# microsoft/aurora

Hardware: AMD Instinct MI355X
Metric: forecast-steps/sec (6h step) 0.25deg ERA5 721x1440x13 (higher is better)
Workload: dtype bf16; 1 GPU; AuroraPretrained(autocast=True) 1.3B, 0.25deg ERA5 721x1440, 13 levels, T=2, batch 1 per GPU, one forward step (BASELINE.json configs[1]); parallelism=1 GPU

## Files before the change

aurora_amd/csrc/gemm.hip:

```cpp
#include <stdlib.h>

#include <algorithm>

#include "gemm_tile.h"

namespace aurora {

namespace {

constexpr int BM = 128;
constexpr int BN = 128;
constexpr int ROW_BYTES = 128;
constexpr int TILE_BYTES = 128 * ROW_BYTES;
constexpr int THREADS = 256;
constexpr int A4_DEFAULT_MIN_K = 0;

template <typename T>
__global__ __launch_bounds__(THREADS, 2) void linear_kernel(const LinearArgs p_in) {
  const LinearArgs p = batch_problem(p_in);
  extern __shared__ __attribute__((aligned(16))) char smem[];
  auto lds_x = [&](int buf) { return smem + buf * 2 * TILE_BYTES; };
  auto lds_w = [&](int buf) { return smem + buf * 2 * TILE_BYTES + TILE_BYTES; };

  const int tid = threadIdx.x;
// ... 409 lines not shown
    }
  }
  if (p.C2 == nullptr && p.res == nullptr && p.vec_store) {
    if (p.act == AURORA_ACT_GELU) epilogue_256_bf16_coalesced<4>(p, acc, m0, n0, wm, wn, wave, lane, smem, &bias_pre);
    else epilogue_256_bf16_coalesced<2>(p, acc, m0, n0, wm, wn, wave, lane, smem, &bias_pre);
    return;
  }
  epilogue_256<bf16_t>(p, acc, m0, n0, wm, wn, i16, g);
}

}

}

using namespace aurora;

namespace {
int default_f32_mode() {
  static const int mode = [] {
    const char* e = getenv("AURORA_F32_GEMM");
    return !e ? 1 : (e[0] == 'n' || e[0] == '0') ? 0 : (e[0] == 'f' || e[0] == '2') ? 2 : 1;
  }();
  return mode;
}

int a4_min_k() {
  static const int v = [] {
    const char* e = getenv("AURORA_GEMM_A4_MIN_K");
    const int k = e ? atoi(e) : A4_DEFAULT_MIN_K;
    return k <= 0 ? 0x7fffffff : k;
  }();
  return v;
}

struct SplitWs { float* slabs; int64_t slab_bytes; int32_t* tickets; int n_tickets; int split; };

int choose_split(int64_t M, int N, int K, int64_t cus) {
  if (N % BN2 != 0 || M < 1024 || K % 32 != 0) return 1;
  const int64_t tiles = ((M + BM2 - 1) / BM2) * (N / BN2);
  const int kt = K / 32;
  int s = (int)std::min<int64_t>(std::min<int64_t>(8, cus / tiles), kt / 64);
  return s < 1 ? 1 : s;
}

struct LinearCall {
  const void* A; int64_t lda; const void* W; int64_t ldw; const float* bias; void* C; int64_t ldc;
  int64_t M; int N; int K; int dtype; void* stream;
  int act = AURORA_ACT_NONE;
  void* C2 = nullptr; int64_t ldc2 = 0; const float* residual = nullptr; int64_t ldr = 0;
  int f32_gemm = -1; const float* guard = nullptr; float guard_limit = 0.f;
  int batch = 1; int64_t stride_a = 0, stride_w = 0, stride_bias = 0, stride_c = 0;
  const SplitWs* ws = nullptr;
  int64_t plane_stride = 0; int plane_heads = 0;
  int pre = 0, mode = 0;
  int es() const { return dtype == AURORA_F32 ? 4 : 2; }
};

enum { K_TILE_128 = F32_KERNELS, K_RING, K_RING_MID, K_PP, K_PP_SPLITK, K_A4 };
struct LinearPlan {
  int kernel; bool twin;
  int bm, bn, rowb;
  int ksplit;
};

int check_call(LinearCall& c) {
  AURORA_CHECK_ARG(c.dtype == AURORA_F32 || c.dtype == AURORA_BF16, "linear: bad dtype %d", c.dtype);
  AURORA_CHECK_ARG(c.plane_stride == 0 || (c.dtype == AURORA_BF16 && c.plane_heads > 0 && c.N % (64 * c.plane_heads) == 0 &&
                                           c.N <= 192 * c.plane_heads && c.plane_stride >= c.M * 192 &&
                                           c.plane_stride % 8 == 0 && c.C2 == nullptr && c.residual == nullptr && c.batch == 1),
                   "linear: head planes need bf16, N = 64 heads x (1, 2 or 3), planes of >= M rows, one output, no residual");
  c.pre = c.f32_gemm < 0 ? 0 : c.f32_gemm & (AURORA_F32_A_SPLIT | AURORA_F32_W_SPLIT | AURORA_F32_C_SPLIT);
  if (c.pre) c.f32_gemm &= ~c.pre;
  AURORA_CHECK_ARG(c.f32_gemm >= -1 && c.f32_gemm <= 2, "linear: bad fp32 GEMM mode %d", c.f32_gemm);
  c.mode = c.f32_gemm < 0 ? default_f32_mode() : c.f32_gemm;
  AURORA_CHECK_ARG(!c.pre || (c.dtype == AURORA_F32 && c.mode == 2 && c.N % 128 == 0 && c.K % 32 == 0 && c.K >= 96),
                   "linear: fp16-pair operands need fp32, mode 2, N %% 128 == 0, K %% 32 == 0, K >= 96 (N=%d K=%d)", c.N, c.K);
  AURORA_CHECK_ARG(!(c.pre & AURORA_F32_A_SPLIT) || (c.pre & AURORA_F32_W_SPLIT),
                   "linear: a pre-split activation operand needs pre-split weights");
  AURORA_CHECK_ARG(!(c.pre & AURORA_F32_C_SPLIT) || (c.C2 == nullptr && c.ldc % 32 == 0 && ((uintptr_t)c.C % 16) == 0),
                   "linear: fp16-pair output needs ldc %% 32 == 0, 16-byte alignment and no second output");
  if (!(c.mode == 2 || (c.mode == 1 && c.dtype == AURORA_F32))) c.guard = nullptr;
  AURORA_CHECK_ARG(c.M > 0 && c.N > 0 && c.K > 0, "linear: empty problem M=%lld N=%d K=%d", (long long)c.M, c.N, c.K);
  const int es = c.es();
  AURORA_CHECK_ARG(((int64_t)c.K * es) % ROW_BYTES == 0,
                   "linear: K=%d must be a multiple of %d elements", c.K, ROW_BYTES / es);
  AURORA_CHECK_ARG((c.lda * es) % 16 == 0 && (c.ldw * es) % 16 == 0 && c.lda >= c.K && c.ldw >= c.K,
                   "linear: operand strides must be 16-byte multiples >= K");
  AURORA_CHECK_ARG(((uintptr_t)c.A % 16) == 0 && ((uintptr_t)c.W % 16) == 0, "linear: unaligned operand");
  AURORA_CHECK_ARG(c.act >= AURORA_ACT_NONE && c.act <= AURORA_ACT_SILU, "linear: bad activation %d", c.act);
  AURORA_CHECK_ARG(c.C != nullptr && c.ldc >= c.N && (!c.C2 || c.ldc2 >= c.N) && (!c.residual || c.ldr >= c.N || c.ldr == 0),
                   "linear: bad output strides");
  return AURORA_OK;
}

LinearPlan plan_linear(const LinearCall& c, int64_t cus) {
  const int64_t M = c.M;
  const int N = c.N, K = c.K, dtype = c.dtype, pre = c.pre, mode = c.mode;
  const bool split = dtype == AURORA_F32 && mode >= 1;
  const bool tall = pre != 0 && N % VN != 0;
  bool big = (M >= 1024 || split) && (N % BN2 == 0 || tall);
  bool mid = false;
  int ksplit = 1;
  if (big && dtype == AURORA_BF16 && c.batch == 1 && c.ws != nullptr) {
    ksplit = c.ws->split > 0 ? std::min(c.ws->split, K / 128) : choose_split(M, N, K, cus);
    const int64_t tiles = ((M + BM2 - 1) / BM2) * (N / BN2);
    if (ksplit > 1 && (tiles > c.ws->n_tickets || tiles * ksplit * (int64_t)(BM2 * BN2 * 4) > c.ws->slab_bytes)) ksplit = 1;
  }
  if (big && !split && ksplit <= 1) {
    const int64_t nb_big = ((M + BM2 - 1) / BM2) * (N / BN2), nb_small = ((M + BM - 1) / BM) * ((N + BN - 1) / BN);
    const int64_t nb_mid = ((M + BM2 - 1) / BM2) * (N / 128);
    if (dtype == AURORA_BF16) {
      auto cost = [&](int64_t nb, int64_t slots, double a, double b) {
        const int64_t full = nb / slots, rem = nb % slots;
        const double part = rem == 0 ? 0.0 : (slots > cus && rem <= cus) ? 0.65 : 1.0;
        return ((double)full + part) * (a + b * (double)K);
      };
      const double t_big = cost(nb_big, cus, 10.1, 0.0266), t_mid = cost(nb_mid, 2 * cus, 7.7, 0.0317),
                   t_small = cost(nb_small, 2 * cus, 7.6, 0.0153);
      if (t_mid < 0.97 * t_big && t_mid <= t_small) mid = true;
      else if (t_small < 0.97 * t_big) big = false;
    } else {
      auto fill = [&](int64_t nb, int64_t slots) { return (double)nb / (double)(((nb + slots - 1) / slots) * slots); };
      if (0.8 * fill(nb_small, 2 * cus) > fill(nb_big, cus)) big = false;
    }
  }
  LinearPlan plan{K_TILE_128, false, big ? BM2 : BM, mid ? 128 : big ? BN2 : BN, big ? ROW2 : ROW_BYTES, ksplit};
  const int k_tiles = (int)(((int64_t)K * c.es()) / plan.rowb);
  const bool f32pp = big && split && mode == 2 && K % 32 == 0 && K >= 96;
  const int pp = tall ? ((pre & AURORA_F32_A_SPLIT) ? F32_PP_AW_TALL : F32_PP_W_TALL)
                      : (pre & AURORA_F32_A_SPLIT) ? F32_PP_AW : (pre & AURORA_F32_W_SPLIT) ? F32_PP_W : F32_PP;
  if (mid) plan.kernel = K_RING_MID;
  else if (!big) plan.kernel = K_TILE_128;
  else if (pre) plan.kernel = pp;
  else if (split && mode == 1 && c.guard != nullptr) plan.kernel = F32_THREE;
  else if (split && mode == 2 && c.guard != nullptr) {
    plan.kernel = f32pp ? pp : F32_TWO;
    plan.twin = true;
  } else if (f32pp) plan.kernel = pp;
  else if (split && mode == 2) plan.kernel = F32_TWO;
  else if (split) plan.kernel = F32_THREE;
  else if (dtype == AURORA_F32) plan.kernel = K_RING;
  else if (ksplit > 1) plan.kernel = K_PP_SPLITK;
  else if (k_tiles >= 8 && k_tiles % 2 == 0 && K >= a4_min_k()) plan.kernel = K_A4;
  else if (k_tiles >= 4) plan.kernel = K_PP;
  else plan.kernel = K_RING;
  return plan;
}

constexpr LinearKernel KERNELS[K_A4 - K_TILE_128][2] = {
     {{linear_kernel<bf16_t>, THREADS, 4 * TILE_BYTES}, {linear_kernel<float>, THREADS, 4 * TILE_BYTES}},
     {{linear_kernel_256<bf16_t, 4, 4>, THREADS2, RING_LDS}, {linear_kernel_256<float, 4, 4>, THREADS2, RING_LDS}},
     {{linear_kernel_256<bf16_t, 2, 3>, 256, MID_LDS}, {}},
     {{linear_kernel_256pp<false>, THREADS2, PP_LDS}, {}},
     {{linear_kernel_256pp<true>, THREADS2, PP_LDS}, {}},
};

int vec_store_of(const LinearCall& c) {
  const int es = c.es(), es2 = es == 4 ? 2 : 4;
  if (c.plane_stride) return ((uintptr_t)c.C % 16) == 0 ? 1 : 0;
  bool vec = ((uintptr_t)c.C % 16) == 0 && (c.ldc * es) % 16 == 0;
  if (c.C2) vec = vec && ((uintptr_t)c.C2 % 16) == 0 && (c.ldc2 * es2) % 16 == 0;
  if (c.residual) vec = vec && ((uintptr_t)c.residual % 16) == 0 && (c.ldr * 4) % 16 == 0;
  return vec ? 1 : 0;
}

int launch_linear(const LinearCall& c, const LinearPlan& plan) {
  const int64_t M = c.M;
  const int N = c.N, K = c.K, es = c.es();
  const bool split = c.dtype == AURORA_F32 && c.mode >= 1, big = plan.bm == BM2;
  LinearArgs p;
  p.A = (const char*)c.A; p.lda_b = c.lda * es;
  p.W = (const char*)c.W; p.ldw_b = c.ldw * es;
  p.bias = c.bias;
  p.C = (char*)c.C; p.ldc = c.ldc; p.C2 = (char*)c.C2; p.ldc2 = c.ldc2;
  p.res = c.residual; p.ldr = c.ldr;
  p.M = M; p.N = N; p.k_tiles = (int)(((int64_t)K * es) / plan.rowb); p.act = c.act;
  p.tiles_n = (N + plan.bn - 1) / plan.bn;
  p.n_blocks = ((M + plan.bm - 1) / plan.bm) * p.tiles_n;
  p.vec_store = vec_store_of(c);
  if (split && big && c.act == AURORA_ACT_GELU) p.act = ACT_GELU_FAST;
  p.guard = split ? c.guard : nullptr;
  p.guard_limit = c.guard_limit;
  p.out_split = (c.pre & AURORA_F32_C_SPLIT) ? 1 : 0;
  AURORA_CHECK_ARG(p.n_blocks < (int64_t)1 << 31, "linear: too many tiles");

  p.bs_a = c.stride_a * es; p.bs_w = c.stride_w * es; p.bs_c = c.stride_c * es; p.bs_bias = c.stride_bias;
  p.split = plan.ksplit; p.slabs = plan.ksplit > 1 ? c.ws->slabs : nullptr; p.tickets = plan.ksplit > 1 ? c.ws->tickets : nullptr;
  p.plane_stride = c.plane_stride; p.plane_heads = c.plane_heads;
  once_per_device([] {
    for (const auto& row : KERNELS)
      for (const LinearKernel& k : row)
        if (k.fn) (void)hipFuncSetAttribute((const void*)k.fn, hipFuncAttributeMaxDynamicSharedMemorySize, k.lds_bytes);
  });
  if (plan.kernel < F32_KERNELS) {
    if (plan.kernel >= F32_PP) {
      const bool tall = plan.kernel >= F32_PP_W_TALL;
      LinearArgs q = p;
      q.k_tiles = K / 32;
      q.tiles_n = tall ? N / 128 : N / VN;
      q.n_blocks = tall ? ((M + 255) / 256) * q.tiles_n : ((M + VM - 1) / VM) * q.tiles_n;
      if (const int err = aurora_f32_launch(plan.kernel, &q, (unsigned)q.n_blocks, (unsigned)c.batch, c.stream)) return err;
    } else {
      if (const int err = aurora_f32_launch(plan.kernel, &p, (unsigned)p.n_blocks, (unsigned)c.batch, c.stream)) return err;
    }
    if (plan.twin) (void)aurora_f32_launch(F32_THREE, &p, (unsigned)p.n_blocks, (unsigned)c.batch, c.stream);
  } else if (plan.kernel == K_A4) {
    (void)aurora_a4_launch(&p, (unsigned)p.n_blocks, (unsigned)c.batch, c.stream);
  } else {
    const LinearKernel& k = KERNELS[plan.kernel - K_TILE_128][c.dtype == AURORA_F32];
    const int64_t slices = plan.kernel == K_PP_SPLITK ? plan.ksplit : 1;
    const dim3 grid((unsigned)(p.n_blocks * slices), (unsigned)c.batch);
    hipLaunchKernelGGL(k.fn, grid, dim3(k.threads), k.lds_bytes, as_stream(c.stream), p);
  }
  return check_launch("linear");
}

int linear_impl(LinearCall c) {
  if (const int err = check_call(c)) return err;
  return launch_linear(c, plan_linear(c, device_cus()));
}

static_assert(F32_THREE == AURORA_PLAN_F32_THREE && F32_TWO == AURORA_PLAN_F32_TWO && F32_PP == AURORA_PLAN_F32_PP &&
              F32_PP_W == AURORA_PLAN_F32_PP_W && F32_PP_AW == AURORA_PLAN_F32_PP_AW &&
              F32_PP_W_TALL == AURORA_PLAN_F32_PP_W_TALL && F32_PP_AW_TALL == AURORA_PLAN_F32_PP_AW_TALL &&
              K_TILE_128 == AURORA_PLAN_TILE128 && K_RING == AURORA_PLAN_RING && K_RING_MID == AURORA_PLAN_RING_MID &&
              K_PP == AURORA_PLAN_PP && K_PP_SPLITK == AURORA_PLAN_PP_SPLITK && K_A4 == AURORA_PLAN_A4,
              "include/aurora_hip.h: AURORA_PLAN_* out of step with the dispatcher's kernel ids");

LinearCall plain_call(const void* A, int64_t lda, const void* W, int64_t ldw, const float* bias, void* C, int64_t ldc, void* C2,
                      int64_t ldc2, const float* residual, int64_t ldr, int64_t M, int N, int K, int dtype, int act, void* stream) {
  LinearCall c{A, lda, W, ldw, bias, C, ldc, M, N, K, dtype, stream, act};
  c.C2 = C2; c.ldc2 = ldc2; c.residual = residual; c.ldr = ldr;
  return c;
}
}

extern "C" int aurora_hip_default_f32_gemm(void) { return default_f32_mode(); }

extern "C" int64_t aurora_hip_linear_workspace(int64_t M, int N, int K, int dtype) {
  if (dtype != AURORA_BF16 || M <= 0 || N <= 0 || K <= 0) return 0;
  const int s = choose_split(M, N, K, device_cus());
  return s <= 1 ? 0 : ((M + BM2 - 1) / BM2) * (N / BN2) * s * (int64_t)(BM2 * BN2 * 4);
}

extern "C" int aurora_hip_linear(const void* A, int64_t lda, const void* W, int64_t ldw,
                                 const float* bias, void* C, int64_t ldc, void* C2, int64_t ldc2,
                                 const float* residual, int64_t ldr, int64_t M, int N, int K,
                                 int dtype, int act, void* stream) {
  return aurora_hip_linear_ex(A, lda, W, ldw, bias, C, ldc, C2, ldc2, residual, ldr, M, N, K, dtype, act, -1, nullptr,
                              0.f, stream);
}

extern "C" int aurora_hip_linear_ex(const void* A, int64_t lda, const void* W, int64_t ldw,
                                    const float* bias, void* C, int64_t ldc, void* C2, int64_t ldc2,
                                    const float* residual, int64_t ldr, int64_t M, int N, int K,
                                    int dtype, int act, int f32_gemm, const float* guard, float guard_limit,
                                    void* stream) {
  LinearCall c = plain_call(A, lda, W, ldw, bias, C, ldc, C2, ldc2, residual, ldr, M, N, K, dtype, act, stream);
  c.f32_gemm = f32_gemm; c.guard = guard; c.guard_limit = guard_limit;
  return linear_impl(c);
}

extern "C" int aurora_hip_linear_planes(const void* A, int64_t lda, const void* W, int64_t ldw, const float* bias, void* C,
                                        int64_t plane_stride, int heads, int64_t M, int N, int K, int dtype, void* stream) {
  AURORA_CHECK_ARG(plane_stride > 0 && heads > 0, "linear_planes: plane_stride=%lld heads=%d", (long long)plane_stride, heads);
  LinearCall c = plain_call(A, lda, W, ldw, bias, C, N, nullptr, 0, nullptr, 0, M, N, K, dtype, AURORA_ACT_NONE, stream);
  c.plane_stride = plane_stride; c.plane_heads = heads;
  return linear_impl(c);
}

extern "C" int aurora_hip_linear_ws(const void* A, int64_t lda, const void* W, int64_t ldw, const float* bias, void* C,
                                    int64_t ldc, void* C2, int64_t ldc2, const float* residual, int64_t ldr, int64_t M, int N,
                                    int K, int dtype, int act, void* workspace, int64_t workspace_bytes, int32_t* tickets,
                                    int n_tickets, int split, void* stream) {
  AURORA_CHECK_ARG(workspace_bytes >= 0 && n_tickets >= 0 && split >= 0 && ((uintptr_t)workspace % 16) == 0,
                   "linear_ws: bad workspace arguments");
  const SplitWs ws{(float*)workspace, workspace ? workspace_bytes : 0, tickets, tickets ? n_tickets : 0, split};
  LinearCall c = plain_call(A, lda, W, ldw, bias, C, ldc, C2, ldc2, residual, ldr, M, N, K, dtype, act, stream);
  c.ws = &ws;
  return linear_impl(c);
}

extern "C" int aurora_hip_linear_batched(const void* A, int64_t lda, const void* W, int64_t ldw, const float* bias, void* C,
                                         int64_t ldc, int64_t M, int N, int K, int dtype, int act, int f32_gemm,
                                         const float* guard, float guard_limit, int batch, int64_t stride_a,
                                         int64_t stride_w, int64_t stride_bias, int64_t stride_c, void* stream) {
  AURORA_CHECK_ARG(batch >= 1 && batch <= 65535, "linear_batched: 1 <= batch <= 65535 (got %d)", batch);
  const int es = dtype == AURORA_F32 ? 4 : 2;
  AURORA_CHECK_ARG((stride_a * es) % 16 == 0 && (stride_w * es) % 16 == 0 && (stride_c * es) % 16 == 0 && stride_bias % 4 == 0,
                   "linear_batched: batch strides must keep every problem 16-byte aligned");
  LinearCall c = plain_call(A, lda, W, ldw, bias, C, ldc, nullptr, 0, nullptr, 0, M, N, K, dtype, act, stream);
  c.f32_gemm = f32_gemm; c.guard = guard; c.guard_limit = guard_limit;
  c.batch = batch; c.stride_a = stride_a; c.stride_w = stride_w; c.stride_bias = stride_bias; c.stride_c = stride_c;
  return linear_impl(c);
}

extern "C" int aurora_hip_linear_plan(int64_t M, int N, int K, int dtype, int f32_gemm, int has_guard, int batch, int64_t ldc,
                                      int64_t c_addr, int64_t ldc2, int64_t c2_addr, int64_t ldr, int64_t residual_addr,
                                      int64_t workspace_bytes, int n_tickets, int split, int64_t plane_stride, int plane_heads,
                                      int cus, int32_t* plan_out) {
  AURORA_CHECK_ARG(plan_out != nullptr && c_addr != 0 && cus >= 0 && batch >= 1, "linear_plan: bad query");
  static const float guard_word = 0.f;
  LinearCall c = plain_call((const void*)16, K, (const void*)16, K, nullptr, (void*)(uintptr_t)c_addr, ldc,
                            (void*)(uintptr_t)c2_addr, ldc2, (const float*)(uintptr_t)residual_addr, ldr, M, N, K, dtype,
                            AURORA_ACT_NONE, nullptr);
  c.f32_gemm = f32_gemm; c.guard = has_guard ? &guard_word : nullptr;
  c.batch = batch;
  const SplitWs ws{nullptr, workspace_bytes, nullptr, n_tickets, split};
  if (workspace_bytes >= 0) c.ws = &ws;
  c.plane_stride = plane_stride; c.plane_heads = plane_heads;
  if (const int err = check_call(c)) return err;
  const LinearPlan plan = plan_linear(c, cus > 0 ? cus : device_cus());
  const bool pp = plan.kernel >= F32_PP && plan.kernel < F32_KERNELS, tall = pp && plan.kernel >= F32_PP_W_TALL;
  plan_out[0] = plan.kernel;
  plan_out[1] = plan.twin ? 1 : 0;
  plan_out[2] = pp ? (tall ? 256 : VM) : plan.bm;
  plan_out[3] = pp ? (tall ? 128 : VN) : plan.bn;
  plan_out[4] = plan.ksplit;
  plan_out[5] = vec_store_of(c);
  return AURORA_OK;
}
```

aurora_amd/csrc/gemm_f32.hip:

```cpp
#include "gemm_tile.h"

#ifndef F32PP_PARTS
#define F32PP_PARTS 4
#endif

namespace aurora {

namespace {

typedef __bf16 bf16x8_t __attribute__((ext_vector_type(8)));

struct Split3 { u32x4 h, m, l; };

__device__ __forceinline__ void split_pair(uint32_t a0, uint32_t a1, uint32_t& h, uint32_t& m, uint32_t& l) {
  constexpr uint32_t SEL = 0x07060302u;
  h = __builtin_amdgcn_perm(a1, a0, SEL);
  const float r0 = __uint_as_float(a0) - __uint_as_float(a0 & 0xffff0000u);
  const float r1 = __uint_as_float(a1) - __uint_as_float(a1 & 0xffff0000u);
  const uint32_t q0 = __float_as_uint(r0), q1 = __float_as_uint(r1);
  m = __builtin_amdgcn_perm(q1, q0, SEL);
  const float s0 = r0 - __uint_as_float(q0 & 0xffff0000u);
  const float s1 = r1 - __uint_as_float(q1 & 0xffff0000u);
  l = __builtin_amdgcn_perm(__float_as_uint(s1), __float_as_uint(s0), SEL);
}
// ... 133 lines not shown
      Split2 w[4];
#pragma unroll
      for (int f = 0; f < 4; ++f)
        w[f] = split8_f16<true>(*reinterpret_cast<const u32x4*>(bufa + off_w[f]),
                                *reinterpret_cast<const u32x4*>(bufb + off_w[f]));
      u32x4 ra = *reinterpret_cast<const u32x4*>(bufa + off_x[0]);
      u32x4 rb = *reinterpret_cast<const u32x4*>(bufb + off_x[0]);
#pragma unroll
      for (int fm = 0; fm < 8; ++fm) {
        const Split2 x = split8_f16<false>(ra, rb);
        if (fm + 1 < 8) {
          ra = *reinterpret_cast<const u32x4*>(bufa + off_x[fm + 1]);
          rb = *reinterpret_cast<const u32x4*>(bufb + off_x[fm + 1]);
        }
#pragma unroll
        for (int fn = 0; fn < 4; ++fn) acc[fn][fm] = mma_f16(w[fn].l, x.h, acc[fn][fm]);
#pragma unroll
        for (int fn = 0; fn < 4; ++fn) acc[fn][fm] = mma_f16(w[fn].h, x.l, acc[fn][fm]);
#pragma unroll
        for (int fn = 0; fn < 4; ++fn) acc[fn][fm] = mma_f16(w[fn].h, x.h, acc[fn][fm]);
      }
  };
  for (int j = 0; j < np; ++j) {
    const char* bufa = smem + ((2 * j) & (NSTAGE2 - 1)) * STAGE2;
    const char* bufb = smem + ((2 * j + 1) & (NSTAGE2 - 1)) * STAGE2;
    if constexpr (TERMS == 3) pair3(bufa, bufb);
    else pair2(bufa, bufb);
    if (j + 1 < np) {
      asm volatile("s_waitcnt vmcnt(0)" ::: "memory");
      __builtin_amdgcn_s_barrier();
      asm volatile("" ::: "memory");
      if (j + 2 < np) {
        stage(2 * j + 4);
        stage(2 * j + 5);
      }
    }
  }
  if constexpr (use_two) {
#pragma unroll
    for (int a = 0; a < 4; ++a)
#pragma unroll
      for (int b = 0; b < 8; ++b) acc[a][b] *= 0.015625f;
  }
  if (p.C2 == nullptr && p.vec_store) {
    __syncthreads();
    epilogue_256_f32_coalesced(p, acc, m0, n0, wm, wn, wave, lane, smem);
    return;
  }
  epilogue_256<float>(p, acc, m0, n0, wm, wn, i16, g);
}


constexpr int VROW = 128, VTHREADS = 512, VNST = 3;
constexpr int VOPER_X = VM * VROW, VOPER_W = VN * VROW, VSTAGE = VOPER_X + VOPER_W;

template <bool A_PRE, bool W_PRE, bool TALL = false>
__global__ __launch_bounds__(VTHREADS, 2) void linear_kernel_f32pp(const LinearArgs p_in) {
  constexpr int TM = TALL ? 256 : VM, TN = TALL ? 128 : VN, OPX = TM * VROW, XP = TM / 64, WP = TN / 64;
  static_assert(OPX + TN * VROW == VSTAGE && XP + WP == 6, "stage size / DMA count the waitcnt immediates assume");
  const LinearArgs p = batch_problem(p_in);
  extern __shared__ __attribute__((aligned(16))) char smem[];
  if (p.guard != nullptr && !(*p.guard < p.guard_limit)) return;
  const int tid = threadIdx.x;
  const int lane = tid & 63;
  const int wave = __builtin_amdgcn_readfirstlane(tid >> 6);
  const int late = wave >> 2;
  const int wm = TALL ? wave >> 1 : wave >> 2, wn = TALL ? wave & 1 : wave & 3;

  uint32_t tile_m, tile_n;
  tile_of_block<2>(blockIdx.x, (uint32_t)p.n_blocks, (uint32_t)(p.n_blocks / p.tiles_n), (uint32_t)p.tiles_n, tile_m, tile_n);
  const int64_t m0 = (int64_t)tile_m * TM;
  const int n0 = (int)tile_n * TN;

  const char* src_x[XP];
  const char* src_w[WP];
#pragma unroll
  for (int r = 0; r < XP; ++r) {
    const int id = r * VTHREADS + tid;
    const int row = id >> 3, c = id & 7;
    int64_t gm = m0 + row;
    gm = gm < p.M ? gm : p.M - 1;
    src_x[r] = p.A + gm * p.lda_b + ((c ^ swz_x(row)) << 4);
  }
#pragma unroll
  for (int r = 0; r < WP; ++r) {
    const int id = r * VTHREADS + tid;
    const int row = id >> 3, c = id & 7;
    src_w[r] = p.W + (int64_t)(n0 + row) * p.ldw_b + ((c ^ swz_w(row)) << 4);
  }
  auto stage = [&](int kt) {
    const int64_t koff = (int64_t)kt * VROW;
    char* base = smem + (kt % VNST) * VSTAGE;
#pragma unroll
    for (int r = 0; r < XP; ++r)
      dma16(src_x[r] + koff, base + (r * VTHREADS + wave * 64) * 16);
#pragma unroll
    for (int r = 0; r < WP; ++r)
      dma16(src_w[r] + koff, base + OPX + (r * VTHREADS + wave * 64) * 16);
  };
  const int i16 = lane & 15, g = lane >> 4;
  int off_x[4][2], off_w[4][2];
#pragma unroll
  for (int f = 0; f < 4; ++f) {
    const int row_x = wm * 64 + 16 * f + i16;
    const int row_w = wn * 64 + 16 * (i16 >> 2) + 4 * f + (i16 & 3);
#pragma unroll
    for (int ks = 0; ks < 2; ++ks) {
      const int cx = A_PRE ? g + 4 * ks : 2 * g + ks, cw = W_PRE ? g + 4 * ks : 2 * g + ks;
      off_x[f][ks] = row_x * VROW + ((cx ^ swz_x(row_x)) << 4);
      off_w[f][ks] = OPX + row_w * VROW + ((cw ^ swz_w(row_w)) << 4);
    }
  }
  f32x4 acc[4][4];
  zero_acc(acc);

  const int nt = p.k_tiles;
  stage(0);
  stage(1);
  stage(2);
  asm volatile("s_waitcnt vmcnt(12)" ::: "memory");
  __builtin_amdgcn_s_barrier();
  asm volatile("" ::: "memory");
  if (late == 1) __builtin_amdgcn_s_barrier();

  for (int s = 0; s < nt; ++s) {
    const char* buf = smem + (s % VNST) * VSTAGE;
    u32x4 xa[4], xb[4];
    Split2 w[4];
#pragma unroll
    for (int f = 0; f < 4; ++f) {
      xa[f] = *reinterpret_cast<const u32x4*>(buf + off_x[f][0]);
      xb[f] = *reinterpret_cast<const u32x4*>(buf + off_x[f][1]);
    }
#pragma unroll
    for (int f = 0; f < 4; ++f)
      if constexpr (W_PRE)
        w[f] = Split2{*reinterpret_cast<const u32x4*>(buf + off_w[f][0]), *reinterpret_cast<const u32x4*>(buf + off_w[f][1])};
      else
        w[f] = split8_f16<true>(*reinterpret_cast<const u32x4*>(buf + off_w[f][0]), *reinterpret_cast<const u32x4*>(buf + off_w[f][1]));
    if (s >= 1 && s + 2 < nt) stage(s + 2);
    if (s + 2 < nt) asm volatile("s_waitcnt vmcnt(6)" ::: "memory");
    else asm volatile("s_waitcnt vmcnt(0)" ::: "memory");
    asm volatile("s_waitcnt lgkmcnt(0)" ::: "memory");
    __builtin_amdgcn_sched_barrier(0);
    __builtin_amdgcn_s_barrier();
    __builtin_amdgcn_sched_barrier(0);
    asm volatile("" ::: "memory");
#pragma unroll
    for (int fm = 0; fm < 4; ++fm) {
      Split2 x;
      if constexpr (A_PRE) x = Split2{xa[fm], xb[fm]};
      else x = split8_f16<false>(xa[fm], xb[fm]);
#pragma unroll
      for (int fn = 0; fn < 4; ++fn) acc[fn][fm] = mma_f16(w[fn].l, x.h, acc[fn][fm]);
#pragma unroll
      for (int fn = 0; fn < 4; ++fn) acc[fn][fm] = mma_f16(w[fn].h, x.l, acc[fn][fm]);
#pragma unroll
      for (int fn = 0; fn < 4; ++fn) acc[fn][fm] = mma_f16(w[fn].h, x.h, acc[fn][fm]);
    }
    __builtin_amdgcn_sched_barrier(0);
    __builtin_amdgcn_s_barrier();
    __builtin_amdgcn_sched_barrier(0);
    asm volatile("" ::: "memory");
  }
  if (late == 0) __builtin_amdgcn_s_barrier();
  asm volatile("" ::: "memory");

  const int nbase = n0 + wn * 64 + 16 * g;
  float bias_v[16];
#pragma unroll
  for (int t = 0; t < 16; ++t) bias_v[t] = p.bias ? p.bias[nbase + t] : 0.f;
  const bool vec = p.vec_store != 0;
  if (vec && p.C2 == nullptr && p.res == nullptr) {
    char* mine = smem + wave * 16384;
    const int rr = lane >> 4, cc = lane & 15;
    float* cbase = reinterpret_cast<float*>(p.C) + n0 + wn * 64 + cc * 4;
#pragma unroll
    for (int part = 0; part < F32PP_PARTS; ++part) {
#pragma unroll
    for (int fm = part * (4 / F32PP_PARTS); fm < (part + 1) * (4 / F32PP_PARTS); ++fm) {
      float v[16];
#pragma unroll
      for (int fn = 0; fn < 4; ++fn) {
        v[4 * fn + 0] = fmaf(acc[fn][fm].x, 0.015625f, bias_v[4 * fn + 0]);
        v[4 * fn + 1] = fmaf(acc[fn][fm].y, 0.015625f, bias_v[4 * fn + 1]);
        v[4 * fn + 2] = fmaf(acc[fn][fm].z, 0.015625f, bias_v[4 * fn + 2]);
        v[4 * fn + 3] = fmaf(acc[fn][fm].w, 0.015625f, bias_v[4 * fn + 3]);
      }
      if (p.act == AURORA_ACT_GELU || p.act == ACT_GELU_FAST) gelu_fast16x2(v);
      else if (p.act == AURORA_ACT_SILU) silu16(v);
      const int row = 16 * fm + i16, sw = row & 7;
      char* lrow = mine + row * 256;
      if (p.out_split) {
        uint32_t h[8], l[8];
#pragma unroll
        for (int t = 0; t < 8; ++t) split_pair_f16(v[2 * t], v[2 * t + 1], h[t], l[t]);
        const int pc = 8 * (g >> 1) + 2 * (g & 1);
        *reinterpret_cast<u32x4*>(lrow + (((pc + 0) ^ sw) << 4)) = u32x4{h[0], h[1], h[2], h[3]};
        *reinterpret_cast<u32x4*>(lrow + (((pc + 1) ^ sw) << 4)) = u32x4{h[4], h[5], h[6], h[7]};
        *reinterpret_cast<u32x4*>(lrow + (((pc + 4) ^ sw) << 4)) = u32x4{l[0], l[1], l[2], l[3]};
        *reinterpret_cast<u32x4*>(lrow + (((pc + 5) ^ sw) << 4)) = u32x4{l[4], l[5], l[6], l[7]};
      } else {
#pragma unroll
        for (int q = 0; q < 4; ++q)
// ... 29 lines not shown
      if (vec) {
#pragma unroll
        for (int q = 0; q < 4; ++q) {
          const f32x4 rv = reinterpret_cast<const f32x4*>(rp)[q];
          v[4 * q] += rv.x; v[4 * q + 1] += rv.y; v[4 * q + 2] += rv.z; v[4 * q + 3] += rv.w;
        }
      } else {
#pragma unroll
        for (int t = 0; t < 16; ++t) v[t] += rp[t];
      }
    }
    if (p.out_split) {
      uint32_t h[8], l[8];
#pragma unroll
      for (int t = 0; t < 8; ++t) split_pair_f16(v[2 * t], v[2 * t + 1], h[t], l[t]);
      char* dst = p.C + (m * p.ldc + (nbase & ~31)) * 4 + (nbase & 31) * 2;
      reinterpret_cast<u32x4*>(dst)[0] = u32x4{h[0], h[1], h[2], h[3]};
      reinterpret_cast<u32x4*>(dst)[1] = u32x4{h[4], h[5], h[6], h[7]};
      reinterpret_cast<u32x4*>(dst + 64)[0] = u32x4{l[0], l[1], l[2], l[3]};
      reinterpret_cast<u32x4*>(dst + 64)[1] = u32x4{l[4], l[5], l[6], l[7]};
      continue;
    }
    store16<float>(reinterpret_cast<float*>(p.C) + m * p.ldc + nbase, v, vec, 16);
    if (p.C2) store16<bf16_t>(reinterpret_cast<bf16_t*>(p.C2) + m * p.ldc2 + nbase, v, vec, 16);
  }
}

__global__ __launch_bounds__(256) void split_f16_kernel(const float* __restrict__ src, int64_t ld_src, char* __restrict__ dst,
                                                        int64_t ld_dst, int64_t rows, int K, float scale) {
  const int per_row = K >> 3;
  const int64_t id = (int64_t)blockIdx.x * 256 + threadIdx.x;
  if (id >= rows * per_row) return;
  const int64_t r = id / per_row;
  const int c = (int)(id - r * per_row) * 8;
  const f32x4 a = *reinterpret_cast<const f32x4*>(src + r * ld_src + c);
  const f32x4 b = *reinterpret_cast<const f32x4*>(src + r * ld_src + c + 4);
  uint32_t h[4], l[4];
  split_pair_f16(a.x * scale, a.y * scale, h[0], l[0]);
  split_pair_f16(a.z * scale, a.w * scale, h[1], l[1]);
  split_pair_f16(b.x * scale, b.y * scale, h[2], l[2]);
  split_pair_f16(b.z * scale, b.w * scale, h[3], l[3]);
  char* d = dst + (r * ld_dst + (c & ~31)) * 4 + (c & 31) * 2;
  *reinterpret_cast<u32x4*>(d) = u32x4{h[0], h[1], h[2], h[3]};
  *reinterpret_cast<u32x4*>(d + 64) = u32x4{l[0], l[1], l[2], l[3]};
}

}

}

using namespace aurora;

namespace {
constexpr LinearKernel F32_TABLE[F32_KERNELS] = {
     {linear_kernel_256_f32x3<3>, THREADS2, NSTAGE2 * STAGE2},
     {linear_kernel_256_f32x3<2>, THREADS2, NSTAGE2 * STAGE2},
     {linear_kernel_f32pp<false, false>, VTHREADS, VNST * VSTAGE},
     {linear_kernel_f32pp<false, true>, VTHREADS, VNST * VSTAGE},
     {linear_kernel_f32pp<true, true>, VTHREADS, VNST * VSTAGE},
     {linear_kernel_f32pp<false, true, true>, VTHREADS, VNST * VSTAGE},
     {linear_kernel_f32pp<true, true, true>, VTHREADS, VNST * VSTAGE},
};
}

extern "C" __attribute__((visibility("hidden"))) int aurora_f32_launch(int kernel, const void* linear_args, unsigned n_blocks,
                                                                      unsigned batch, void* stream) {
  const LinearArgs& p = *static_cast<const LinearArgs*>(linear_args);
  AURORA_CHECK_ARG(kernel >= 0 && kernel < F32_KERNELS, "linear: no fp32 kernel %d", kernel);
  once_per_device([] {
    for (const LinearKernel& k : F32_TABLE) (void)hipFuncSetAttribute((const void*)k.fn, hipFuncAttributeMaxDynamicSharedMemorySize, k.lds_bytes);
  });
  const LinearKernel& k = F32_TABLE[kernel];
  hipLaunchKernelGGL(k.fn, dim3(n_blocks, batch), dim3(k.threads), k.lds_bytes, as_stream(stream), p);
  return 0;
}

extern "C" int aurora_hip_split_f16(const float* src, int64_t ld_src, void* dst, int64_t ld_dst, int64_t rows, int K,
                                    float scale, void* stream) {
  AURORA_CHECK_ARG(src != nullptr && dst != nullptr && rows > 0 && K > 0 && K % 32 == 0, "split_f16: K=%d must be a positive multiple of 32", K);
  AURORA_CHECK_ARG(ld_src >= K && ld_dst >= K && ld_src % 4 == 0 && ld_dst % 32 == 0 && ((uintptr_t)src % 16) == 0 &&
                   ((uintptr_t)dst % 16) == 0, "split_f16: strides / alignment");
  const int64_t n = rows * (K >> 3);
  hipLaunchKernelGGL(split_f16_kernel, dim3((unsigned)((n + 255) / 256)), dim3(256), 0, as_stream(stream), src, ld_src,
                     (char*)dst, ld_dst, rows, K, scale);
  return check_launch("split_f16");
}
```

aurora_amd/csrc/gemm_tile.h:

```cpp
#pragma once

#include "common.h"

namespace aurora {

namespace {

constexpr int ACT_GELU_FAST = 4;

struct LinearArgs {
  const char* A; int64_t lda_b;
  const char* W; int64_t ldw_b;
  const float* bias;
  char* C; int64_t ldc;
  char* C2; int64_t ldc2;
  const float* res; int64_t ldr;
  int64_t M; int N; int k_tiles; int act;
  int tiles_n; int64_t n_blocks;
  int vec_store;
  const float* guard; float guard_limit;
  int out_split;
  int64_t bs_a, bs_w, bs_c, bs_bias;
  int split; float* slabs; int32_t* tickets;
  int64_t plane_stride; int plane_heads;
};

template <typename T>
__device__ __forceinline__ T* out_piece(const LinearArgs& p, int64_t m, int n) {
  T* const c = reinterpret_cast<T*>(p.C);
  if (!p.plane_stride) return c + m * p.ldc + n;
  const int blk = n >> 6, sel = blk / p.plane_heads, h = blk - sel * p.plane_heads;
  return c + (int64_t)h * p.plane_stride + m * 192 + sel * 64 + (n & 63);
}

__device__ __forceinline__ LinearArgs batch_problem(const LinearArgs& in) {
  LinearArgs p = in;
  const int64_t g = blockIdx.y;
  p.A += g * in.bs_a;
  p.W += g * in.bs_w;
  p.C += g * in.bs_c;
  if (in.bias) p.bias += g * in.bs_bias;
  return p;
}

typedef __attribute__((address_space(3))) void* lds_ptr_t;

__device__ __forceinline__ int swz_x(int row) { return row & 7; }
__device__ __forceinline__ int swz_w(int row) { return (((row >> 4) & 3) << 1) | ((row >> 1) & 1); }

template <typename T> struct Mma;
template <> struct Mma<bf16_t> {
  typedef __bf16 bf16x8 __attribute__((ext_vector_type(8)));
  __device__ static __forceinline__ f32x4 run(u32x4 a, u32x4 b, f32x4 c) {
    return __builtin_amdgcn_mfma_f32_16x16x32_bf16(__builtin_bit_cast(bf16x8, a),
                                                   __builtin_bit_cast(bf16x8, b), c, 0, 0, 0);
  }
};
template <> struct Mma<float> {
  __device__ static __forceinline__ f32x4 run(u32x4 a, u32x4 b, f32x4 c) {
    c = __builtin_amdgcn_mfma_f32_16x16x4f32(__uint_as_float(a.x), __uint_as_float(b.x), c, 0, 0, 0);
    c = __builtin_amdgcn_mfma_f32_16x16x4f32(__uint_as_float(a.y), __uint_as_float(b.y), c, 0, 0, 0);
    c = __builtin_amdgcn_mfma_f32_16x16x4f32(__uint_as_float(a.z), __uint_as_float(b.z), c, 0, 0, 0);
    c = __builtin_amdgcn_mfma_f32_16x16x4f32(__uint_as_float(a.w), __uint_as_float(b.w), c, 0, 0, 0);
    return c;
  }
};

template <typename T>
__device__ __forceinline__ void store16(T* dst, const float (&v)[16], bool vec, int n_left);

template <>
__device__ __forceinline__ void store16<float>(float* dst, const float (&v)[16], bool vec, int n_left) {
  if (vec && n_left >= 16) {
#pragma unroll
    for (int q = 0; q < 4; ++q)
      reinterpret_cast<f32x4*>(dst)[q] = f32x4{v[4 * q], v[4 * q + 1], v[4 * q + 2], v[4 * q + 3]};
  } else {
// ... 191 lines not shown
  float bias_v[16];
#pragma unroll
  for (int t = 0; t < 16; ++t) bias_v[t] = p.bias ? p.bias[nbase + t] : 0.f;
  const int rr = lane >> 4, cc = lane & 15;
  float* cbase = reinterpret_cast<float*>(p.C) + n0 + wn * 64 + cc * 4;
#pragma unroll
  for (int half = 0; half < 2; ++half) {
#pragma unroll
    for (int f = 0; f < 4; ++f) {
      const int fm = 4 * half + f;
      float v[16];
      biased16(acc, fm, bias_v, v);
      if (p.act == AURORA_ACT_GELU) {
#pragma unroll
        for (int t = 0; t < 16; ++t) v[t] = gelu_for<float>(v[t]);
      } else if (p.act == ACT_GELU_FAST) {
#pragma unroll
        for (int t = 0; t < 16; t += 2) {
          const f32x2_hw r = gelu_erf_fast2(f32x2_hw{v[t], v[t + 1]});
          v[t] = r.x;
          v[t + 1] = r.y;
        }
      } else if (p.act == AURORA_ACT_SILU) {
        silu16(v);
      }
      if (p.res) {
        const int64_t m = m0 + wm * 128 + 16 * fm + i16;
        const float* rp = p.res + (m < p.M ? m : p.M - 1) * p.ldr + nbase;
#pragma unroll
        for (int q = 0; q < 4; ++q) {
          const f32x4 rv = reinterpret_cast<const f32x4*>(rp)[q];
          v[4 * q] += rv.x; v[4 * q + 1] += rv.y; v[4 * q + 2] += rv.z; v[4 * q + 3] += rv.w;
        }
      }
      const int row = 16 * f + i16, sw = row & 7;
#pragma unroll
      for (int q = 0; q < 4; ++q)
        *reinterpret_cast<f32x4*>(mine + row * 256 + (((4 * g + q) ^ sw) << 4)) =
            f32x4{v[4 * q], v[4 * q + 1], v[4 * q + 2], v[4 * q + 3]};
    }
#pragma unroll
    for (int it = 0; it < 16; ++it) {
      const int row = it * 4 + rr;
      const f32x4 d = *reinterpret_cast<const f32x4*>(mine + row * 256 + ((cc ^ (row & 7)) << 4));
      const int64_t m = m0 + wm * 128 + 64 * half + row;
      if (m < p.M) __builtin_nontemporal_store(d, reinterpret_cast<f32x4*>(cbase + m * p.ldc));
    }
  }
}

struct LinearKernel { void (*fn)(LinearArgs); unsigned threads; int lds_bytes; };

enum F32Kernel { F32_THREE, F32_TWO, F32_PP, F32_PP_W, F32_PP_AW, F32_PP_W_TALL, F32_PP_AW_TALL, F32_KERNELS };

}

}

extern "C" __attribute__((visibility("hidden"))) int aurora_a4_launch(const void* linear_args, unsigned n_blocks, unsigned batch,
                                                                     void* stream);
extern "C" __attribute__((visibility("hidden"))) int aurora_f32_launch(int kernel, const void* linear_args, unsigned n_blocks,
                                                                      unsigned batch, void* stream);
```

aurora_amd/csrc/model.h:

```cpp
#pragma once

#include <math.h>
#include <stdlib.h>
#include <string.h>

#include <algorithm>
#include <array>
#include <exception>
#include <map>
#include <memory>
#include <stdexcept>
#include <string>
#include <vector>

#include "band.h"
#include "common.h"

namespace aurora {

struct Fail {
  int code;
};
#define REQUIRE(cond, ...)               \
  do {                                   \
// ... 137 lines not shown
  std::vector<std::string> sep_perceiver, mod_heads, pos_surf, pos_atmos, surf_inputs, density_vars, angle_vars;
  std::map<std::string, int> diff_index;
  std::vector<aurora::Channel> surf_channels, atmos_channels;
  std::vector<std::string> surf_heads, surf_out;
  std::vector<std::string> atmos_heads;

  std::map<std::string, aurora::Tensor> w;
  std::map<std::string, aurora::Tensor> w16;
  bool finalized = false;
  std::vector<aurora::Block> blocks;
  aurora::DevBuf mod, lead_emb, enc_q0;
  std::vector<aurora::DevBuf> keep;
  std::map<int, aurora::AttnSet> attn_sets;
  struct Merge { const void* w; const float *ln_w, *ln_b; };
  struct Split { const void *w1, *w2; const float *ln_w, *ln_b; };
  std::vector<Merge> merges;
  std::vector<Split> splits;
  aurora::Resampler enc_rs, dec_rs, dec_rs_alt;
  bool has_alt = false;

  bool have_grid = false;
  int n_lat = 0, n_lon = 0, Hp = 0, Wp = 0, n_levels = 0;
  int full_Hp = 0;
  std::vector<double> levels;
  aurora::DevBuf pos_scale, enc_bias, dec_queries, dec_q, dec_q_alt, stats;
  std::vector<size_t> surf_stat_off, static_stat_off, atmos_stat_off;
  size_t one_stat_off = 0;
  std::vector<size_t> static_lvl_stat_off;
  std::vector<double> static_loc;
  std::map<std::array<int64_t, 3>, aurora::EmbedPack> embed_packs;
  float enc_bias_max = 0.f;
  aurora::DevBuf surf_w0_s, surf_w2_s;
  float surf_l1_0 = 0.f, surf_b0 = 0.f, surf_c = 0.f;
  bool surf_chain = false;
  aurora::HeadGroup head_surf, head_main, head_alt;
  float dec_out_bound = 0.f, dec_out_bound_alt = 0.f;
  std::map<std::pair<int, int>, aurora::DevTables> tables;
  std::vector<aurora::Res> stage_res;
  std::vector<std::array<int, 2>> merge_pad;

  aurora_hip_band band{0, 1, nullptr, nullptr, nullptr};
  std::vector<std::vector<std::array<int, 2>>> rows;
  std::map<std::pair<int, int>, aurora::DevPlan> plans;
  void* stage_send = nullptr;
  void* stage_recv = nullptr;
  int64_t staging_bytes = 0, staging_need = 0;
  bool sharded() const { return band.world > 1; }
  int fuse_ln = 1;
  bool split_attention = false;
  bool qkv_planes = true;
  bool reassoc_out = true;
  bool compose_front = true;
  bool front_composed = false;
  bool score_weights = true;

  aurora::DevBuf abs_enc, dyn_planes, ctx_max;
  float guard_limit_min[4] = {INFINITY, INFINITY, INFINITY, INFINITY};
  int guard_launches[4] = {0, 0, 0, 0};
  void note_guard(const float* word, float limit) {
    const ptrdiff_t i = word - ctx_max.f();
    if (dry || word == nullptr || i < 0 || i >= 4) return;
    guard_limit_min[i] = std::min(guard_limit_min[i], limit);
    ++guard_launches[i];
  }
  aurora::DevBuf tickets;
  bool split_k = true;
  int abs_B = 0;
  struct Pinned { float* host = nullptr; size_t bytes = 0; hipEvent_t done = nullptr; };
  Pinned pinned[4];
  int pinned_next = 0;
  ~aurora_hip_model() {
    for (auto& t : timed) { (void)hipEventDestroy(t.e0); (void)hipEventDestroy(t.e1); }
    for (auto& e : event_pool) (void)hipEventDestroy(e);
    for (auto& s : pinned) {
      if (s.host) (void)hipHostFree(s.host);
      if (s.done) (void)hipEventDestroy(s.done);
    }
  }
  aurora::Arena arena;
  bool dry = false;
  int64_t generation = 0;

  struct Timed { int kind; double work; hipEvent_t e0, e1; };
  uint32_t profile_mask = 0;
  std::vector<Timed> timed;
  std::vector<hipEvent_t> event_pool;

  const float* W(const std::string& name) const {
    auto it = w.find(name);
    REQUIRE(it != w.end(), "missing weight '%s'", name.c_str());
    return it->second.f();
  }
  const aurora::Tensor& T_(const std::string& name) const {
    auto it = w.find(name);
    REQUIRE(it != w.end(), "missing weight '%s'", name.c_str());
    return it->second;
  }
  bool has(const std::string& name) const { return w.count(name) != 0; }
  int bb() const { return autocast ? AURORA_BF16 : AURORA_F32; }
  size_t bbs() const { return autocast ? 2 : 4; }
  int stage_dim(int s) const { return D << s; }
};

namespace aurora {

typedef aurora_hip_model Model;

enum Kind { K_LINEAR_BF16, K_LINEAR_F32, K_WINDOW_ATTENTION, K_LAYERNORM, K_MERGE_LN, K_SPLIT_LN, K_PATCHIFY,
            K_PERCEIVER_ATTENTION, K_ASSEMBLE, K_UNPATCHIFY, K_COPY2D, K_ABSMAX, K_LINEAR_LN, K_GATHER, K_PERCEIVER_OUT, K_COUNT };

hipEvent_t take_event(Model& m);

template <typename F>
void timed(Model& m, void* stream, int kind, double work, F&& fn) {
  if (m.dry) return;
  const bool on = (m.profile_mask >> kind) & 1u;
  hipEvent_t e0 = nullptr, e1 = nullptr;
  if (on) {
    e0 = take_event(m);
    e1 = take_event(m);
    hip_ok(hipEventRecord(e0, (hipStream_t)stream), "hipEventRecord");
  }
  ok(fn());
  if (on) {
    hip_ok(hipEventRecord(e1, (hipStream_t)stream), "hipEventRecord");
    m.timed.push_back({kind, work, e0, e1});
  }
}

constexpr int SPLIT_TICKETS = 4096;

struct LinearOp {
  const void *A, *W;
  const float* bias;
  void* C;
  int64_t lda, ldw, ldc, M;
  int N, K, dtype, act = AURORA_ACT_NONE, f32_gemm = -1, batch = 1;
  void* C2 = nullptr;
  const float *res = nullptr, *guard = nullptr;
  int64_t ldc2 = 0, ldr = 0, sa = 0, sw = 0, sbias = 0, sc = 0;
  float limit = 0.f;
  LinearOp(const void* A_, int64_t lda_, const void* W_, int64_t ldw_, const float* bias_, void* C_, int64_t ldc_, int64_t M_, int N_,
           int K_, int dtype_)
      : A(A_), W(W_), bias(bias_), C(C_), lda(lda_), ldw(ldw_), ldc(ldc_), M(M_), N(N_), K(K_), dtype(dtype_) {}
  LinearOp& activation(int a) { act = a; return *this; }
  LinearOp& second_output(void* c2, int64_t ld) { C2 = c2; ldc2 = ld; return *this; }
  LinearOp& residual(const float* r, int64_t ld) { res = r; ldr = ld; return *this; }
  LinearOp& f32_mode(int mode) { f32_gemm = mode; return *this; }
  LinearOp& guarded_by(const float* word, float lim) { guard = word; limit = lim; return *this; }
  LinearOp& batched(int n, int64_t a, int64_t w, int64_t b, int64_t c) { batch = n; sa = a; sw = w; sbias = b; sc = c; return *this; }
};

struct PerceiverCols {
  int B;
  int64_t cols, kv_bstride, kv_lstride;
  int Lq, Lk, heads;
  int64_t n_cols() const { return (int64_t)B * cols; }
  int64_t n_rows() const { return n_cols() * Lq; }
};

struct Launcher {
  Model& m;
  void* stream;
  void linear(const LinearOp& o) {
    void* ws = nullptr;
    int64_t ws_bytes = 0;
    const size_t mark = m.arena.top;
    m.note_guard(o.guard, o.limit);
    if (m.split_k && o.dtype == AURORA_BF16 && o.batch == 1 && o.f32_gemm == -1 &&
        (ws_bytes = aurora_hip_linear_workspace(o.M, o.N, o.K, o.dtype)) > 0)
      ws = m.arena.take((size_t)ws_bytes);
    timed(m, stream, o.dtype == AURORA_BF16 ? K_LINEAR_BF16 : K_LINEAR_F32, 2.0 * (double)o.M * o.N * o.K * o.batch, [&] {
      if (ws)
        return aurora_hip_linear_ws(o.A, o.lda, o.W, o.ldw, o.bias, o.C, o.ldc, o.C2, o.ldc2, o.res, o.ldr, o.M, o.N, o.K, o.dtype,
                                    o.act, ws, ws_bytes, (int32_t*)m.tickets.p, SPLIT_TICKETS, 0, stream);
      if (o.batch > 1)
        return aurora_hip_linear_batched(o.A, o.lda, o.W, o.ldw, o.bias, o.C, o.ldc, o.M, o.N, o.K, o.dtype, o.act, o.f32_gemm,
                                         o.guard, o.limit, o.batch, o.sa, o.sw, o.sbias, o.sc, stream);
      return aurora_hip_linear_ex(o.A, o.lda, o.W, o.ldw, o.bias, o.C, o.ldc, o.C2, o.ldc2, o.res, o.ldr, o.M, o.N, o.K, o.dtype,
                                  o.act, o.f32_gemm, o.guard, o.limit, stream);
    });
    m.arena.top = mark;
  }
  void guarded_pair(LinearOp op, const void* Ws, int splits, const float* word, float limit) {
    const void* Wf = op.W;
    op.W = Ws;
    linear(op.f32_mode(2 | AURORA_F32_W_SPLIT | splits).guarded_by(word, limit));
    op.W = Wf;
    linear(op.f32_mode(1));
  }
  void guarded_linear(LinearOp op, const void* Ws, int splits, int mode, const float* word, float limit) {
    if (Ws) guarded_pair(op, Ws, splits, word, limit);
    else if (mode == 2) linear(op.f32_mode(2).guarded_by(word, limit));
    else linear(op.f32_mode(mode));
  }
  void linear_planes(const void* A, int64_t lda, const void* Wt, int64_t ldw, const float* bias, void* C, int64_t plane_stride,
                     int heads, int64_t M, int N, int K) {
    timed(m, stream, K_LINEAR_BF16, 2.0 * (double)M * N * K, [&] {
      return aurora_hip_linear_planes(A, lda, Wt, ldw, bias, C, plane_stride, heads, M, N, K, AURORA_BF16, stream);
    });
  }
  void layernorm(const void* y, int64_t ldy, const float* gain, const float* shift, const float* res, int64_t ldr,
                 int64_t res_mod, float* out_f32, int64_t ldo, void* out_t, int64_t ldt, int64_t M, int D, float eps,
                 int dtype) {
    timed(m, stream, K_LAYERNORM, 0.0, [&] {
      return aurora_hip_layernorm(y, ldy, gain, shift, res, ldr, res_mod, out_f32, ldo, out_t, ldt, M, D, eps, dtype, stream);
    });
  }
  void layernorm_split(const float* y, int64_t ldy, const float* gain, const float* shift, const void* res, int64_t ldr,
                       int64_t res_mod, int res_is_split, float* out_f32, int64_t ldo, void* out_split, int64_t ld_split,
                       int64_t M, int D, float eps) {
    timed(m, stream, K_LAYERNORM, 0.0, [&] {
      return aurora_hip_layernorm_split(y, ldy, gain, shift, res, ldr, res_mod, res_is_split, out_f32, ldo, out_split, ld_split, M, D,
                                        eps, stream);
    });
  }
  void perceiver_attention(const PerceiverCols& g, int head_dim, const float* q, int64_t q_stride, const float* kv, float* att,
                           const float* pair_word, float pair_limit, const float* skip_word, float skip_limit) {
    timed(m, stream, K_PERCEIVER_ATTENTION, 0.0, [&] {
      if (skip_word)
        return aurora_hip_perceiver_attention_unless(q, q_stride, kv, att, g.B, g.cols, g.kv_bstride, g.kv_lstride, g.Lq, g.Lk, g.heads,
                                                     head_dim, AURORA_F32, pair_word, pair_limit, skip_word, skip_limit, stream);
      return aurora_hip_perceiver_attention_ex(q, q_stride, kv, att, g.B, g.cols, g.kv_bstride, g.kv_lstride, g.Lq, g.Lk, g.heads,
                                               head_dim, AURORA_F32, pair_word, pair_limit, stream);
    });
  }
  void perceiver_attention_scores(const PerceiverCols& g, int head_dim, const float* vs, int64_t ld_vs, int s_off, float* att,
                                  const float* pair_word, float pair_limit, const float* skip_word, float skip_limit) {
    timed(m, stream, K_PERCEIVER_ATTENTION, 0.0, [&] {
      return aurora_hip_perceiver_attention_scores(vs, ld_vs, s_off, att, g.B, g.cols, g.kv_bstride, g.kv_lstride, g.Lq, g.Lk, g.heads,
                                                   head_dim, pair_word, pair_limit, skip_word, skip_limit, stream);
    });
  }
  void perceiver_probs(const PerceiverCols& g, int head_dim, const float* q, const float* kv, int64_t ld_vs, int s_off, float* P,
                       void* Vp, const float* word, float limit) {
    timed(m, stream, K_PERCEIVER_ATTENTION, 0.0, [&] {
      if (q)
        return aurora_hip_perceiver_probs(q, kv, P, Vp, g.B, g.cols, g.kv_bstride, g.kv_lstride, g.Lq, g.Lk, g.heads, head_dim, word,
                                          limit, stream);
      return aurora_hip_perceiver_probs_scores(kv, ld_vs, s_off, P, Vp, g.B, g.cols, g.kv_bstride, g.kv_lstride, g.Lq, g.Lk, g.heads,
                                               head_dim, word, limit, stream);
    });
  }
  void perceiver_out(const PerceiverCols& g, int head_dim, const void* Vp, const void* W_pairs, int inner, const float* P, float* out,
                     int N, const float* word, float limit) {
    timed(m, stream, K_PERCEIVER_OUT, 2.0 * (double)g.n_cols() * g.Lk * N * inner + 2.0 * (double)g.n_rows() * N * g.heads * g.Lk, [&] {
      return aurora_hip_perceiver_out(Vp, W_pairs, inner, P, nullptr, out, N, g.n_cols(), g.Lq, g.Lk, g.heads, head_dim, N, word, limit,
                                      stream);
    });
  }
};

inline void upload(void* dst, const void* src, size_t bytes) {
  hip_ok(hipMemcpy(dst, src, bytes, hipMemcpyHostToDevice), "upload");
}
inline DevBuf to_device(const std::vector<float>& v) {
  DevBuf b(v.size() * sizeof(float));
  upload(b.p, v.data(), v.size() * sizeof(float));
  return b;
}
inline std::vector<float> to_host(const float* dev, size_t n) {
  std::vector<float> h(n);
  hip_ok(hipMemcpy(h.data(), dev, n * 4, hipMemcpyDeviceToHost), "download");
  return h;
}
inline std::vector<float> to_host(const Tensor& t) { return to_host(t.f(), (size_t)t.numel); }
inline bool contains(const std::vector<std::string>& v, const std::string& s) { return std::find(v.begin(), v.end(), s) != v.end(); }

// ... 36 lines not shown
```

aurora_amd/csrc/model.hip:

```cpp
#include "model.h"

namespace aurora {

hipEvent_t take_event(Model& m) {
  if (!m.event_pool.empty()) {
    hipEvent_t e = m.event_pool.back();
    m.event_pool.pop_back();
    return e;
  }
  hipEvent_t e;
  hip_ok(hipEventCreate(&e), "hipEventCreate");
  return e;
}

int bounded_mode() {
  static const int mode = getenv("AURORA_F32_GEMM") ? -1 : 2;
  return mode;
}

std::string level_to_str(double level) {
  const double value = round(level * 1000.0) / 1000.0;
  char buf[64];
  if (value == (double)(long long)value) snprintf(buf, sizeof buf, "%lld", (long long)value);
  else {
// ... 124 lines not shown
      m->enc_heads[i] = c->encoder_heads[i]; m->dec_heads[i] = c->decoder_heads[i];
      se += c->encoder_depths[i]; sd += c->decoder_depths[i];
    }
    REQUIRE(se == sd, "Encoder and decoder must have the same total depth.");
    for (int a = 0; a < 3; ++a) m->window[a] = c->window[a];
    REQUIRE(m->window[0] * m->window[1] * m->window[2] <= 144, "windows of more than 144 tokens are not supported");
    REQUIRE(m->Cl % m->window[0] == 0, "latent levels must be divisible by the window's level extent");
    m->enc_depth = c->enc_depth; m->dec_depth = c->dec_depth; m->max_history = c->max_history;
    m->ln_eps = c->perceiver_ln_eps; m->timestep_hours = c->timestep_hours;
    m->stabilise = c->stabilise_level_agg != 0; m->use_lora = c->use_lora != 0;
    m->lora_steps = c->lora_steps; m->lora_mode = c->lora_mode; m->autocast = c->autocast != 0;
    REQUIRE(m->lora_mode >= 0 && m->lora_mode <= 2, "create: lora_mode must be 0 (single), 1 (from_second) or 2 (all)");
    auto names = [](const char* const* p, int n, std::vector<std::string>& dst) {
      for (int i = 0; i < n; ++i) dst.push_back(p[i]);
    };
    names(c->surf_vars, c->n_surf, m->surf_vars);
    names(c->static_vars, c->n_static, m->static_vars);
    names(c->atmos_vars, c->n_atmos, m->atmos_vars);
    REQUIRE(!m->surf_vars.empty() && !m->atmos_vars.empty(), "create: variable lists must not be empty");
    m->variant = c->variant;
    REQUIRE(m->variant >= 0 && m->variant <= 2, "create: variant must be 0 (base), 1 (air pollution) or 2 (ocean wave)");
    for (int i = 0; i < c->n_level_condition; ++i) m->level_condition.push_back(c->level_condition[i]);
    m->dynamic_vars = c->dynamic_vars != 0; m->atmos_static_vars = c->atmos_static_vars != 0;
    m->clamp_first = c->clamp_at_first_step != 0; m->index_bug = c->simulate_indexing_bug != 0;
    names(c->separate_perceiver, c->n_separate_perceiver, m->sep_perceiver);
    names(c->modulation_heads, c->n_modulation_heads, m->mod_heads);
    names(c->positive_surf_vars, c->n_positive_surf, m->pos_surf);
    names(c->positive_atmos_vars, c->n_positive_atmos, m->pos_atmos);
    names(c->surf_inputs, c->n_surf_inputs, m->surf_inputs);
    names(c->density_channel_surf_vars, c->n_density, m->density_vars);
    names(c->angle_surf_vars, c->n_angle, m->angle_vars);
    if (m->surf_inputs.empty()) m->surf_inputs = m->surf_vars;
    REQUIRE(m->variant == 2 || m->surf_inputs == m->surf_vars, "create: surf_inputs are for the ocean-wave variant");
    if (c->difference_history)
      for (int i = 0; i < c->n_modulation_heads; ++i)
        if (c->difference_history[i] >= 0) m->diff_index[m->mod_heads[i]] = c->difference_history[i];
    REQUIRE(m->static_vars.size() <= 60 && m->surf_inputs.size() <= 60 && m->atmos_vars.size() <= 60, "create: too many variables");
    build_blocks(*m);
    build_channels(*m);
    m->ctx_max = DevBuf(16);
    const auto& tu = c->tuning;
    REQUIRE(tu.fuse_ln >= 0 && tu.fuse_ln <= 3, "create: tuning.fuse_ln = %d (0 default, 1 never, 2 by the fill rule, 3 always)", tu.fuse_ln);
    auto sw = [](int32_t v, bool dflt, const char* what) {
      REQUIRE(v >= 0 && v <= 2, "create: tuning.%s = %d (0 default, 1 off, 2 on)", what, v);
      return v == 0 ? dflt : v == 2;
    };
    m->fuse_ln = tu.fuse_ln == 0 ? 1 : tu.fuse_ln - 1;
    m->split_attention = sw(tu.band_split_attention, false, "band_split_attention");
    m->qkv_planes = sw(tu.qkv_planes, true, "qkv_planes");
    m->split_k = sw(tu.split_k, true, "split_k");
    m->reassoc_out = sw(tu.perceiver_reassoc, true, "perceiver_reassoc");
    m->score_weights = sw(tu.score_weights, true, "score_weights");
    m->compose_front = sw(tu.compose_front, true, "compose_front");
    m->tickets = DevBuf(SPLIT_TICKETS * sizeof(int32_t));
    hip_ok(hipMemset(m->tickets.p, 0, SPLIT_TICKETS * sizeof(int32_t)), "hipMemset");
    *out = m.release();
  })
}

extern "C" void aurora_hip_destroy(aurora_hip_model* m) { delete m; }

extern "C" int aurora_hip_set_band(aurora_hip_model* mp, const aurora_hip_band* band) {
  GUARDED({
    REQUIRE(mp != nullptr, "set_band: null model");
    Model& m = *mp;
    if (band == nullptr || band->world <= 1) {
      m.band = aurora_hip_band{0, 1, nullptr, nullptr, nullptr};
    } else {
      REQUIRE(band->rank >= 0 && band->rank < band->world, "set_band: rank %d of %d", band->rank, band->world);
      REQUIRE(band->post && band->wait, "set_band: the halo transport callbacks are required");
      m.band = *band;
    }
    m.have_grid = false;
    m.plans.clear(); m.rows.clear();
    m.stage_send = m.stage_recv = nullptr;
    m.staging_bytes = m.staging_need = 0;
  })
}

extern "C" int aurora_hip_band_rows(const aurora_hip_model* m, int32_t* row0, int32_t* row1) {
  GUARDED({
    REQUIRE(m && row0 && row1 && m->have_grid, "band_rows: precompute the grid first");
    const int h0 = m->sharded() ? m->rows[0][m->band.rank][0] : 0;
    *row0 = h0 * m->P;
    *row1 = (h0 + m->Hp) * m->P;
  })
}

extern "C" int64_t aurora_hip_band_staging_bytes(const aurora_hip_model* m) { return m ? m->staging_need : 0; }

extern "C" int aurora_hip_set_band_staging(aurora_hip_model* m, void* send, void* recv, int64_t staging_bytes) {
  GUARDED({
    REQUIRE(m != nullptr, "set_band_staging: null model");
    REQUIRE(staging_bytes >= m->staging_need, "set_band_staging: %lld bytes per buffer, %lld needed", (long long)staging_bytes,
            (long long)m->staging_need);
    REQUIRE(m->staging_need == 0 || (send && recv && (uintptr_t)send % 16 == 0 && (uintptr_t)recv % 16 == 0),
            "set_band_staging: two 16-byte aligned device buffers are required");
    m->stage_send = send;
    m->stage_recv = recv;
    m->staging_bytes = staging_bytes;
  })
}

extern "C" int aurora_hip_output_vars(const aurora_hip_model* m, const char** names, int capacity) {
  if (!m) return 0;
  if (names)
// ... 130 lines not shown
```

aurora_amd/csrc/model_weights.hip:

```cpp
#include "model.h"

namespace aurora {

constexpr int LORA_RANK = 8;

float absmax(const std::vector<float>& h) {
  float mx = 0.f;
  for (float v : h) mx = std::max(mx, fabsf(v));
  return mx;
}
float absmax(const float* dev, size_t n) { return absmax(to_host(dev, n)); }
float max_row_l1(const std::vector<float>& h, int64_t rows, int64_t K, float floor) {
  float best = floor;
  for (int64_t r = 0; r < rows; ++r) {
    float sum = 0.f;
    for (int64_t k = 0; k < K; ++k) sum += fabsf(h[(size_t)r * K + k]);
    best = std::max(best, sum);
  }
  return best;
}

bool presplit_shape(int64_t rows, int64_t K, int row_multiple) { return rows % row_multiple == 0 && K % 32 == 0 && K >= 96; }
DevBuf presplit(const float* w, int64_t rows, int64_t K, int64_t ld, int row_multiple, int groups) {
  if (!presplit_shape(rows, K, row_multiple)) return DevBuf();
// ... 393 lines not shown
}

}

using namespace aurora;

extern "C" int aurora_hip_compose_weight(const float* w_ctx, int N, int D, const float* w_e, int K, int groups, float* out) {
  GUARDED({
    REQUIRE(w_ctx && w_e && out && N > 0 && D > 0 && K > 0 && groups > 0, "compose_weight: bad argument");
    std::vector<double> acc((size_t)K);
    for (int g = 0; g < groups; ++g)
      for (int n = 0; n < N; ++n) {
        std::fill(acc.begin(), acc.end(), 0.0);
        for (int d = 0; d < D; ++d) {
          const double a = w_ctx[(size_t)n * D + d];
          const float* row = w_e + ((size_t)g * D + d) * K;
          for (int k = 0; k < K; ++k) acc[k] += a * row[k];
        }
        float* dst = out + ((size_t)g * N + n) * K;
        for (int k = 0; k < K; ++k) dst[k] = (float)acc[k];
      }
  })
}

extern "C" int aurora_hip_compose_bias(const float* w_ctx, int N, int D, const float* bias, int C, float* out) {
  GUARDED({
    REQUIRE(w_ctx && bias && out && N > 0 && D > 0 && C > 0, "compose_bias: bad argument");
    for (int c = 0; c < C; ++c)
      for (int n = 0; n < N; ++n) {
        double acc = 0.0;
        for (int d = 0; d < D; ++d) acc += (double)w_ctx[(size_t)n * D + d] * bias[(size_t)c * D + d];
        out[(size_t)c * N + n] = (float)acc;
      }
  })
}

extern "C" int aurora_hip_compose_front_rule(int Kpad, int D, const int32_t* N, int n_layers) {
  return compose_front_rule(Kpad, D, N, n_layers) ? 1 : 0;
}

extern "C" int aurora_hip_composed_value_bound(float v_l1, float embed_l1, float embed_bias_max, float composed_v_l1,
                                               float composed_vb_max, float out[6]) {
  GUARDED({
    REQUIRE(out && v_l1 > 0.f && embed_l1 > 0.f && composed_v_l1 > 0.f && embed_bias_max >= 0.f && composed_vb_max >= 0.f,
            "composed_value_bound: bad argument");
    const ValueBound staged{v_l1 * embed_l1, v_l1 * embed_bias_max}, folded = composed_value_bound(v_l1, embed_l1, embed_bias_max,
                                                                                              composed_v_l1, composed_vb_max);
    out[0] = staged.a; out[1] = staged.c; out[2] = (F16_SAFE / v_l1 - embed_bias_max) / embed_l1;
    out[3] = folded.a; out[4] = folded.c; out[5] = folded.word_limit();
  })
}

extern "C" int aurora_hip_front_composed(const aurora_hip_model* m) { return m != nullptr && m->front_composed ? 1 : 0; }

extern "C" int aurora_hip_pack_weights(aurora_hip_model* m, const char* name, const void* data, const int64_t* shape, int ndim,
                                       int dtype, int on_device) {
  GUARDED({
    REQUIRE(m && name && data && ndim >= 0 && ndim <= 8, "pack_weights: bad argument");
    REQUIRE(dtype == AURORA_F32, "pack_weights: parameters must be float32 (the engine keeps fp32 masters)");
    Tensor t;
    t.numel = 1;
    for (int i = 0; i < ndim; ++i) { t.shape.push_back(shape[i]); t.numel *= shape[i]; }
    t.buf = DevBuf((size_t)t.numel * 4);
    hip_ok(hipMemcpy(t.buf.p, data, (size_t)t.numel * 4, on_device ? hipMemcpyDeviceToDevice : hipMemcpyHostToDevice),
           "pack_weights copy");
    m->w[name] = std::move(t);
    m->finalized = false;
  })
}

namespace {
const char PACK_MAGIC[] = "AURORAHIP1";

bool backbone_matrix(const Model& m, const std::string& name) {
  if (name.rfind("backbone.", 0) != 0 || name.size() < 7 || name.compare(name.size() - 7, 7, ".weight") != 0) return false;
  for (const char* tag : {".mlp.fc1.", ".mlp.fc2.", ".downsample.reduction.", ".upsample.lin1.", ".upsample.lin2."})
    if (name.find(tag) != std::string::npos) return true;
  if (!m.use_lora && (name.find(".attn.qkv.") != std::string::npos || name.find(".attn.proj.") != std::string::npos)) return true;
  return false;
}
}

extern "C" int aurora_hip_save_packed(aurora_hip_model* mp, const char* path, void* stream) {
  GUARDED({
    REQUIRE(mp && path, "save_packed: null argument");
    Model& m = *mp;
    FILE* f = fopen(path, "wb");
    REQUIRE(f != nullptr, "save_packed: cannot open '%s' for writing", path);
    struct Closer { FILE* f; ~Closer() { fclose(f); } } closer{f};
    auto put = [&](const void* p, size_t n) { REQUIRE(fwrite(p, 1, n, f) == n, "save_packed: short write"); };
    put(PACK_MAGIC, sizeof(PACK_MAGIC));
    const uint32_t n_entries = (uint32_t)(m.w.size() + m.w16.size());
    put(&n_entries, 4);
    std::vector<char> host;
    auto entry = [&](const std::string& name, const Tensor& t, uint32_t dtype, const void* dev, size_t bytes) {
      const uint32_t len = (uint32_t)name.size(), nd = (uint32_t)t.shape.size();
      put(&len, 4); put(name.data(), len); put(&dtype, 4); put(&nd, 4);
      for (int64_t d : t.shape) put(&d, 8);
      const uint64_t nb = bytes;
      put(&nb, 8);
      host.resize(bytes);
      hip_ok(hipMemcpy(host.data(), dev, bytes, hipMemcpyDeviceToHost), "save_packed download");
      put(host.data(), bytes);
    };
    for (const auto& kv : m.w) {
      if (m.autocast && backbone_matrix(m, kv.first)) {
// ... 73 lines not shown
```

aurora_amd/csrc/norm.hip:

```cpp
#include <stdlib.h>

#include "common.h"

namespace aurora {
namespace {

constexpr int ROWS_PER_BLOCK = 4;

template <int MAXC>
__device__ __forceinline__ void row_stats(const float (&v)[MAXC][8], int lane, int n_pieces, float inv_d, float eps,
                                          float& mean, float& rstd) {
  float s = 0.f;
#pragma unroll
  for (int i = 0; i < MAXC; ++i)
    if (lane + 64 * i < n_pieces) {
#pragma unroll
      for (int j = 0; j < 8; ++j) s += v[i][j];
    }
  mean = wave_sum(s) * inv_d;
  float q = 0.f;
#pragma unroll
  for (int i = 0; i < MAXC; ++i)
    if (lane + 64 * i < n_pieces) {
#pragma unroll
      for (int j = 0; j < 8; ++j) {
        const float d = v[i][j] - mean;
        q = fmaf(d, d, q);
      }
    }
  rstd = rsqrtf(wave_sum(q) * inv_d + eps);
}

struct LnArgs {
  const void* y; int64_t ldy; const float* gain; const float* shift;
  const float* res; int64_t ldr; int64_t res_mod;
  float* out_f32; int64_t ldo; void* out_t; int64_t ldt;
  int64_t M; int D; float eps;
  int split_t;
  int split_res;
};

template <typename T, int NC, bool PRE = false>
__global__ __launch_bounds__(256) void layernorm_f32_kernel(const LnArgs p) {
  const int lane = threadIdx.x & 63;
  const int64_t row = (int64_t)blockIdx.x * ROWS_PER_BLOCK + (threadIdx.x >> 6);
  if (row >= p.M) return;
  const int n_pieces = p.D >> 2;
  const T* yr = reinterpret_cast<const T*>(p.y) + row * p.ldy;
  const float* rr = nullptr;
  if (p.res) rr = p.res + (p.res_mod > 0 ? (int64_t)(((p.M | p.res_mod) >> 32) == 0 ? (uint32_t)row % (uint32_t)p.res_mod : row % p.res_mod) : row) * p.ldr;
  const bool res_plain = PRE && rr != nullptr && !p.split_res;
  float v[NC][4], r4[PRE ? NC : 1][4];
#pragma unroll
  for (int i = 0; i < NC; ++i)
    if (lane + 64 * i < n_pieces) {
      load4(yr + (lane + 64 * i) * 4, v[i]);
      if constexpr (PRE) {
        if (res_plain) load4(rr + (lane + 64 * i) * 4, r4[i]);
      }
    }
  float s = 0.f;
#pragma unroll
  for (int i = 0; i < NC; ++i)
    if (lane + 64 * i < n_pieces) s += (v[i][0] + v[i][1]) + (v[i][2] + v[i][3]);
  const float inv_d = 1.0f / p.D;
  const float mean = wave_sum(s) * inv_d;
  float q = 0.f;
#pragma unroll
  for (int i = 0; i < NC; ++i)
    if (lane + 64 * i < n_pieces) {
#pragma unroll
      for (int j = 0; j < 4; ++j) {
        const float d = v[i][j] - mean;
        q = fmaf(d, d, q);
      }
    }
  const float rstd = rsqrtf(wave_sum(q) * inv_d + p.eps);
#pragma unroll
  for (int i = 0; i < NC; ++i) {
    const int e = (lane + 64 * i) * 4;
    if (lane + 64 * i < n_pieces) {
      float gn[4], sh[4], o[4];
      if (p.gain) load4(p.gain + e, gn);
      if (p.shift) load4(p.shift + e, sh);
#pragma unroll
      for (int j = 0; j < 4; ++j) {
        float t = (v[i][j] - mean) * rstd;
        if (p.gain) t *= gn[j];
        if (p.shift) t += sh[j];
        o[j] = t;
      }
      if (rr && p.split_res) {
        const char* s = reinterpret_cast<const char*>(rr) + (e & ~31) * 4 + (e & 31) * 2;
        const u32x2 h = *reinterpret_cast<const u32x2*>(s);
        const u32x2 l = *reinterpret_cast<const u32x2*>(s + 64);
        auto half = [](uint32_t w, int hi) { return (float)__builtin_bit_cast(_Float16, (uint16_t)(hi ? w >> 16 : w & 0xffffu)); };
        const uint32_t hw[2] = {h.x, h.y}, lw[2] = {l.x, l.y};
#pragma unroll
        for (int j = 0; j < 4; ++j) o[j] += half(hw[j >> 1], j & 1) + half(lw[j >> 1], j & 1);
      } else if (rr) {
        if constexpr (PRE) {
#pragma unroll
          for (int j = 0; j < 4; ++j) o[j] += r4[i][j];
        } else {
          float r[4];
          load4(rr + e, r);
#pragma unroll
          for (int j = 0; j < 4; ++j) o[j] += r[j];
        }
      }
      if (p.out_f32) store4(p.out_f32 + row * p.ldo + e, o);
      if (p.out_t && p.split_t) {
        uint32_t h0, h1, l0, l1;
        split_pair_f16(o[0], o[1], h0, l0);
        split_pair_f16(o[2], o[3], h1, l1);
        const bool odd = (lane & 1) != 0;
        auto swap1 = [](uint32_t x) { return (uint32_t)__builtin_amdgcn_update_dpp(0, (int)x, 0xB1, 0xf, 0xf, true); };
        const uint32_t r0 = swap1(odd ? h0 : l0), r1 = swap1(odd ? h1 : l1);
        const int e8 = e & ~7;
        char* d = reinterpret_cast<char*>(p.out_t) + (row * p.ldt + (e8 & ~31)) * 4 + (e8 & 31) * 2 + (odd ? 64 : 0);
        *reinterpret_cast<u32x4*>(d) = odd ? u32x4{r0, r1, l0, l1} : u32x4{h0, h1, r0, r1};
      } else if (p.out_t) {
        store4(reinterpret_cast<T*>(p.out_t) + row * p.ldt + e, o);
      }
    }
  }
}

struct MergeArgs {
  const float* x; const float* w; const float* b; void* out;
  int B, C, H, W, D, H2, W2; float eps;
};

template <typename T, int MAXC>
__global__ __launch_bounds__(256) void merge_ln_kernel(const MergeArgs p) {
  const int lane = threadIdx.x & 63;
  const int64_t row = (int64_t)blockIdx.x * ROWS_PER_BLOCK + (threadIdx.x >> 6);
  const int64_t rows = (int64_t)p.B * p.C * p.H2 * p.W2;
  if (row >= rows) return;
  const int w2 = (int)(row % p.W2);
  const int h2 = (int)((row / p.W2) % p.H2);
  const int64_t bc = row / ((int64_t)p.W2 * p.H2);
  const int D4 = 4 * p.D, n_pieces = D4 >> 3;
  float v[MAXC][8];
#pragma unroll
  for (int i = 0; i < MAXC; ++i) {
    const int e = (lane + 64 * i) * 8;
    if (lane + 64 * i < n_pieces) {
      const int seg = e / p.D, d = e - seg * p.D;
      const int hh = 2 * h2 + (seg >> 1), ww = 2 * w2 + (seg & 1);
      if (hh < p.H && ww < p.W) {
        load8(p.x + ((bc * p.H + hh) * p.W + ww) * p.D + d, v[i]);
      } else {
#pragma unroll
        for (int j = 0; j < 8; ++j) v[i][j] = 0.f;
      }
    }
  }
  float mean, rstd;
  row_stats<MAXC>(v, lane, n_pieces, 1.0f / D4, p.eps, mean, rstd);
  T* orow = reinterpret_cast<T*>(p.out) + row * D4;
#pragma unroll
  for (int i = 0; i < MAXC; ++i) {
    const int e = (lane + 64 * i) * 8;
    if (lane + 64 * i < n_pieces) {
      float gn[8], sh[8], o[8];
      load8(p.w + e, gn);
      load8(p.b + e, sh);
#pragma unroll
      for (int j = 0; j < 8; ++j) o[j] = (v[i][j] - mean) * rstd * gn[j] + sh[j];
      store8(orow + e, o);
    }
  }
}

struct SplitArgs {
  const void* y; const float* w; const float* b; void* out;
  int B, C, H, W, Dq, Ho, Wo; float eps;
};
// ... 62 lines not shown
                                          const void* res, int64_t ldr, int64_t res_mod, int res_is_split, float* out_f32,
                                          int64_t ldo, void* out_split, int64_t ld_split, int64_t M, int D, float eps,
                                          void* stream) {
  AURORA_CHECK_ARG(D % 32 == 0, "layernorm_split: D=%d must be a multiple of 32", D);
  AURORA_CHECK_ARG(out_split == nullptr || (ld_split % 32 == 0 && ld_split >= D),
                   "layernorm_split: the pair-layout output stride must be a multiple of 32, >= D");
  AURORA_CHECK_ARG(!res_is_split || (res != nullptr && ldr % 32 == 0 && ldr >= D),
                   "layernorm_split: the pair-layout residual stride must be a multiple of 32, >= D");
  return layernorm_impl(y, ldy, gain, shift, static_cast<const float*>(res), ldr, res_mod, out_f32, ldo, out_split, ld_split,
                        M, D, eps, AURORA_F32, out_split ? 1 : 0, res_is_split ? 1 : 0, stream);
}

static int layernorm_impl(const void* y, int64_t ldy, const float* gain, const float* shift, const float* res, int64_t ldr,
                          int64_t res_mod, float* out_f32, int64_t ldo, void* out_t, int64_t ldt, int64_t M, int D,
                          float eps, int dtype, int split_t, int split_res, void* stream) {
  AURORA_CHECK_ARG(dtype == AURORA_F32 || dtype == AURORA_BF16, "layernorm: bad dtype");
  AURORA_CHECK_ARG(D % 8 == 0 && D > 0 && D <= 4096, "layernorm: D=%d must be a multiple of 8, <= 4096", D);
  const int es = dtype == AURORA_F32 ? 4 : 2;
  AURORA_CHECK_ARG((ldy * es) % 16 == 0 && (uintptr_t)y % 16 == 0, "layernorm: unaligned input rows");
  AURORA_CHECK_ARG((!res || ((ldr * 4) % 16 == 0 && (uintptr_t)res % 16 == 0)) &&
                       (!out_f32 || ((ldo * 4) % 16 == 0 && (uintptr_t)out_f32 % 16 == 0)) &&
                       (!out_t || ((ldt * es) % 16 == 0 && (uintptr_t)out_t % 16 == 0)),
                   "layernorm: unaligned residual/output rows");
  AURORA_CHECK_ARG(out_f32 || out_t, "layernorm: no output");
  if (M <= 0) return AURORA_OK;
  LnArgs p{y, ldy, gain, shift, res, ldr, res_mod, out_f32, ldo, out_t, ldt, M, D, eps, split_t, split_res};
  if (dtype == AURORA_F32) {
    const dim3 grid(row_blocks(M)), block(256);
    if (D <= 256) hipLaunchKernelGGL((layernorm_f32_kernel<float, 1>), grid, block, 0, as_stream(stream), p);
    else if (D <= 512) hipLaunchKernelGGL((layernorm_f32_kernel<float, 2>), grid, block, 0, as_stream(stream), p);
    else if (D <= 1024) hipLaunchKernelGGL((layernorm_f32_kernel<float, 4>), grid, block, 0, as_stream(stream), p);
    else if (D <= 2048) hipLaunchKernelGGL((layernorm_f32_kernel<float, 8>), grid, block, 0, as_stream(stream), p);
    else hipLaunchKernelGGL((layernorm_f32_kernel<float, 16>), grid, block, 0, as_stream(stream), p);
  } else {
    const dim3 grid(row_blocks(M)), block(256);
    const bool pre = res != nullptr && M <= (int64_t)40 * device_cus();
    if (pre) {
      if (D <= 256) hipLaunchKernelGGL((layernorm_f32_kernel<bf16_t, 1, true>), grid, block, 0, as_stream(stream), p);
      else if (D <= 512) hipLaunchKernelGGL((layernorm_f32_kernel<bf16_t, 2, true>), grid, block, 0, as_stream(stream), p);
      else if (D <= 1024) hipLaunchKernelGGL((layernorm_f32_kernel<bf16_t, 4, true>), grid, block, 0, as_stream(stream), p);
      else if (D <= 2048) hipLaunchKernelGGL((layernorm_f32_kernel<bf16_t, 8, true>), grid, block, 0, as_stream(stream), p);
      else hipLaunchKernelGGL((layernorm_f32_kernel<bf16_t, 16>), grid, block, 0, as_stream(stream), p);
    } else {
      if (D <= 256) hipLaunchKernelGGL((layernorm_f32_kernel<bf16_t, 1>), grid, block, 0, as_stream(stream), p);
      else if (D <= 512) hipLaunchKernelGGL((layernorm_f32_kernel<bf16_t, 2>), grid, block, 0, as_stream(stream), p);
      else if (D <= 1024) hipLaunchKernelGGL((layernorm_f32_kernel<bf16_t, 4>), grid, block, 0, as_stream(stream), p);
      else if (D <= 2048) hipLaunchKernelGGL((layernorm_f32_kernel<bf16_t, 8>), grid, block, 0, as_stream(stream), p);
      else hipLaunchKernelGGL((layernorm_f32_kernel<bf16_t, 16>), grid, block, 0, as_stream(stream), p);
    }
  }
  return check_launch("layernorm");
}

extern "C" int aurora_hip_merge_ln(const float* x, const float* ln_w, const float* ln_b, void* out, int B, int C,
                                   int H, int W, int D, float eps, int dtype, void* stream) {
  AURORA_CHECK_ARG(dtype == AURORA_F32 || dtype == AURORA_BF16, "merge_ln: bad dtype");
  AURORA_CHECK_ARG(D % 8 == 0 && 4 * D <= 4096, "merge_ln: D=%d must be a multiple of 8 with 4D <= 4096", D);
  AURORA_CHECK_ARG(H >= 1 && W >= 1, "merge_ln: empty grid %dx%d", H, W);
  MergeArgs p{x, ln_w, ln_b, out, B, C, H, W, D, (H + 1) / 2, (W + 1) / 2, eps};
  const int64_t rows = (int64_t)B * C * p.H2 * p.W2;
  if (dtype == AURORA_F32)
    AURORA_DISPATCH_ROW(merge_ln_kernel, float, 4 * D, dim3(row_blocks(rows)), dim3(256), 0, as_stream(stream), p);
  else
    AURORA_DISPATCH_ROW(merge_ln_kernel, bf16_t, 4 * D, dim3(row_blocks(rows)), dim3(256), 0, as_stream(stream), p);
  return check_launch("merge_ln");
}

extern "C" int aurora_hip_split_ln(const void* y, const float* ln_w, const float* ln_b, void* out, int B, int C,
                                   int H, int W, int Dq, int crop_h, int crop_w, float eps, int dtype,
                                   void* stream) {
  AURORA_CHECK_ARG(dtype == AURORA_F32 || dtype == AURORA_BF16, "split_ln: bad dtype");
  AURORA_CHECK_ARG(Dq % 8 == 0 && Dq <= 4096, "split_ln: Dq=%d must be a multiple of 8, <= 4096", Dq);
  AURORA_CHECK_ARG(crop_h >= 0 && crop_h <= 1 && crop_w >= 0 && crop_w <= 1, "split_ln: crop must be 0 or 1");
  SplitArgs p{y, ln_w, ln_b, out, B, C, H, W, Dq, 2 * H - crop_h, 2 * W - crop_w, eps};
  const int64_t rows = (int64_t)B * C * p.Ho * p.Wo;
  if (dtype == AURORA_F32)
    AURORA_DISPATCH_ROW(split_ln_kernel, float, Dq, dim3(row_blocks(rows)), dim3(256), 0, as_stream(stream), p);
  else
    AURORA_DISPATCH_ROW(split_ln_kernel, bf16_t, Dq, dim3(row_blocks(rows)), dim3(256), 0, as_stream(stream), p);
  return check_launch("split_ln");
}
```

aurora_amd/csrc/step.hip:

```cpp
#include <algorithm>

#include "model.h"
#include "resampler_space.h"

namespace aurora {

namespace {

struct CtxGuard { float* word; float a, c, limit_kv; bool pairs, scan; };
struct ComposedFront { const ComposedCtx* layers; int levels, groups; int64_t rows; float embed_l1, embed_bias_max; };

struct ResamplerCall {
  const Resampler* rs;
  const float* ctx;
  int64_t ctx_rows;
  int ctx_dim;
  const float *q0, *latents0;
  PerceiverCols g;
  float eps;
  bool out_pairs;
  const ComposedFront* front;
  CtxGuard guard;
};

struct ResamplerLayer {
  const ResamplerCall& call;
  size_t i;
  const Resampler::Layer& ly;
  LayerSpace sp;
  const float* lat;
  const float* word;
  float lim_out;
  float *y, *lat1;
  char* S;
  size_t after_y;
  float *kv, *qb, *att, *P, *o;
  void* Vp;
  const float* q;
  int64_t q_stride;
};

ResamplerLayer resampler_layer(Model& m, const ResamplerCall& c, size_t i, const float* lat) {
  const Resampler& rs = *c.rs;
  const auto& ly = rs.layers[i];
  LayerShape sh{};
  sh.layer = i;
  sh.dim = ly.dim; sh.inner = ly.inner; sh.hidden = ly.hidden; sh.head_dim = ly.head_dim; sh.heads = c.g.heads;
  sh.n_vs = rs.n_vs; sh.vs_lq = rs.vs_lq;
  sh.ln_k = ly.ln_k_w != nullptr; sh.to_out_s = ly.to_out_s != nullptr; sh.fc1_s = ly.fc1_s != nullptr; sh.fc2_s = ly.fc2_s != nullptr;
  sh.f16_mode = ly.f16_mode;
  sh.reassoc_out = m.reassoc_out;
  sh.out_supported = aurora_hip_perceiver_out_supported(c.g.Lq, c.g.Lk, c.g.heads, ly.head_dim, ly.dim) != 0;
  sh.B = c.g.B; sh.cols = c.g.cols; sh.ctx_rows = c.ctx_rows; sh.Lq = c.g.Lq; sh.Lk = c.g.Lk;
  const LayerSpace sp = layer_space(sh);
  const CtxGuard& gd = c.guard;
  const float lim_out = c.front ? composed_value_bound(ly.v_l1, c.front->embed_l1, c.front->embed_bias_max, c.front->layers[i].v_l1,
                                                       c.front->layers[i].vb_max).word_limit()
                                : (F16_SAFE / ly.v_l1 - gd.c) / gd.a;
  ResamplerLayer r{c, i, ly, sp, lat, gd.word, lim_out};
  r.y = (float*)m.arena.take(sp.unit);
  r.after_y = m.arena.top;
  r.Vp = r.y;
  r.lat1 = (float*)m.arena.take(sp.unit);
  r.S = (char*)m.arena.take(sp.s_bytes);
  r.kv = r.o = (float*)r.S;
  r.qb = (float*)(r.S + round256(sp.kv_bytes));
  r.P = (float*)(r.S + sp.p_off);
  r.att = sp.att_in_y ? r.y : (float*)(r.S + sp.att_off);
  r.q = i > 0 ? r.qb : c.q0;
  r.q_stride = i > 0 ? c.g.Lq : 0;
  return r;
}

void project_context(Launcher& L, const ResamplerLayer& r) {
  const ResamplerCall& c = r.call;
// ... 34 lines not shown
}

void attend_plain(Launcher& L, const ResamplerLayer& r, bool skip) {
  const PerceiverCols& g = r.call.g;
  const auto& ly = r.ly;
  const int inner = ly.inner;
  const bool pairs = !skip && r.sp.att_pairs;
  const float* pair_word = pairs ? r.word : nullptr;
  const float pair_limit = skip ? 0.f : r.lim_out, skip_limit = skip ? r.lim_out : 0.f;
  const float* skip_word = skip ? r.word : nullptr;
  if (pairs) L.m.note_guard(r.word, r.lim_out);
  if (r.sp.scores) L.perceiver_attention_scores(g, ly.head_dim, r.kv, r.sp.kv_ld, inner, r.att, pair_word, pair_limit, skip_word, skip_limit);
  else L.perceiver_attention(g, ly.head_dim, r.q, r.q_stride, r.kv, r.att, pair_word, pair_limit, skip_word, skip_limit);
  LinearOp to_out(r.att, inner, ly.to_out, inner, nullptr, r.o, ly.dim, g.n_rows(), ly.dim, inner, AURORA_F32);
  if (skip) L.linear(to_out.f32_mode(1).guarded_by(r.word, r.lim_out));
  else L.guarded_linear(to_out, ly.to_out_s, pairs ? AURORA_F32_A_SPLIT : 0, ly.f16_mode, r.word, r.lim_out);
}

void attend_reassociated(Launcher& L, const ResamplerLayer& r) {
  const PerceiverCols& g = r.call.g;
  const auto& ly = r.ly;
  const LayerSpace& sp = r.sp;
  REQUIRE(sp.p_off >= sp.kv_bytes && sp.p_off >= sp.unit && sp.p_off + sp.p_bytes <= sp.s_bytes,
          "resampler: the softmax weights overlap k | v or to_out's result in the scratch region");
  for (int k = 0; k < 3; ++k) L.m.note_guard(r.word, r.lim_out);
  L.perceiver_probs(g, ly.head_dim, sp.scores ? nullptr : r.q, r.kv, sp.kv_ld, ly.inner, r.P, r.Vp, r.word, r.lim_out);
  L.perceiver_out(g, ly.head_dim, r.Vp, ly.to_out_s, ly.inner, r.P, r.o, ly.dim, r.word, r.lim_out);
  attend_plain(L, r, true);
}

void resampler_mlp(Launcher& L, const ResamplerLayer& r) {
  const ResamplerCall& c = r.call;
  const auto& ly = r.ly;
  const LayerSpace& sp = r.sp;
  const int Dd = ly.dim;
  const int64_t n_rows = c.g.n_rows();
  const float* res = r.i == 0 ? c.latents0 : r.lat;
  const int64_t res_mod = r.i == 0 ? c.g.Lq : 0;
  float *lat1 = r.lat1, *y = r.y;
  if (sp.pairs) L.layernorm_split(r.o, Dd, ly.ln1_w, ly.ln1_b, res, Dd, res_mod, 0, nullptr, 0, lat1, Dd, n_rows, Dd, c.eps);
  else L.layernorm(r.o, Dd, ly.ln1_w, ly.ln1_b, res, Dd, res_mod, lat1, Dd, nullptr, 0, n_rows, Dd, c.eps, AURORA_F32);
  float* hid = (float*)r.S;
  const int64_t chunk_rows = sp.chunk_rows;
  REQUIRE(chunk_rows >= 1 && (size_t)chunk_rows * sp.hid_row <= sp.s_bytes, "resampler: scratch region too small for the MLP");
  const int all = 2 | AURORA_F32_A_SPLIT | AURORA_F32_W_SPLIT;
  for (int64_t r0 = 0; r0 < n_rows; r0 += chunk_rows) {
    const int64_t nr = std::min(chunk_rows, n_rows - r0);
    LinearOp fc1(lat1 + (size_t)r0 * Dd, Dd, sp.pairs ? ly.fc1_s : ly.fc1_w, Dd, ly.fc1_b, hid, ly.hidden, nr, ly.hidden, Dd, AURORA_F32);
    LinearOp fc2(hid, ly.hidden, sp.pairs ? ly.fc2_s : ly.fc2_w, ly.hidden, ly.fc2_b, y + (size_t)r0 * Dd, Dd, nr, Dd, ly.hidden, AURORA_F32);
    L.linear(fc1.activation(AURORA_ACT_GELU).f32_mode(sp.pairs ? all | AURORA_F32_C_SPLIT : ly.f16_mode));
    L.linear(fc2.f32_mode(sp.pairs ? all : ly.f16_mode));
  }
  const bool y_pairs = c.out_pairs && sp.pairs && r.i + 1 == c.rs->layers.size();
  if (sp.pairs) L.layernorm_split(y, Dd, ly.ln2_w, ly.ln2_b, lat1, Dd, 0, 1, y_pairs ? nullptr : y, Dd, y_pairs ? y : nullptr, Dd, n_rows, Dd, c.eps);
  else L.layernorm(y, Dd, ly.ln2_w, ly.ln2_b, lat1, Dd, 0, y, Dd, nullptr, 0, n_rows, Dd, c.eps, AURORA_F32);
}

float* resampler(Model& m, Launcher& L, const ResamplerCall& c) {
  if (c.guard.scan)
    timed(m, L.stream, K_ABSMAX, 0.0, [&] { return aurora_hip_absmax_fold(c.ctx, c.ctx_rows * c.ctx_dim, c.guard.word, L.stream); });
  float* lat = nullptr;
  for (size_t i = 0; i < c.rs->layers.size(); ++i) {
    const ResamplerLayer r = resampler_layer(m, c, i, lat);
    project_context(L, r);
    norm_keys(L, r);
    project_queries(L, r);
    if (r.sp.reassoc) attend_reassociated(L, r);
    else attend_plain(L, r, false);
    resampler_mlp(L, r);
    m.arena.top = r.after_y;
    lat = r.y;
  }
  return lat;
}

inline int index_of(const std::vector<std::string>& v, const std::string& s) {
  const auto it = std::find(v.begin(), v.end(), s);
  return it == v.end() ? -1 : (int)(it - v.begin());
}

aurora_patch_var channel_desc(const Model& m, const aurora_hip_step_io& io, const Channel& ch, bool atmos_level, int C) {
  const float* st = m.stats.f();
  aurora_patch_var d{};
  d.transform = ch.transform; d.tw0 = ch.tw0; d.tw1 = ch.tw1; d.tb = ch.tb;
  switch (ch.kind) {
    case SRC_SURF:
      d.src = io.surf[ch.src];
      d.stride_b = io.surf_strides[0]; d.stride_t = io.surf_strides[1]; d.stride_h = io.surf_strides[2]; d.stride_w = io.surf_strides[3];
      d.loc = st + m.surf_stat_off[ch.src]; d.inv_scale = d.loc + 2;
      break;
    case SRC_STATIC:
      d.src = io.stat[ch.src];
      d.stride_h = io.static_strides[0]; d.stride_w = io.static_strides[1];
      if (atmos_level) { d.loc = st + m.static_lvl_stat_off[ch.src]; d.inv_scale = d.loc + 2 * C; }
      else { d.loc = st + m.static_stat_off[ch.src]; d.inv_scale = d.loc + 2; }
      break;
    case SRC_DYN:
      d.src = m.dyn_planes.f() + (size_t)ch.src * m.abs_B;
      d.stride_b = 1;
      d.loc = st + m.one_stat_off; d.inv_scale = d.loc + 2 * C;
      break;
    case SRC_ATMOS:
      d.src = io.atmos[ch.src];
      d.stride_b = io.atmos_strides[0]; d.stride_t = io.atmos_strides[1]; d.stride_c = io.atmos_strides[2];
      d.stride_h = io.atmos_strides[3]; d.stride_w = io.atmos_strides[4];
      d.loc = st + m.atmos_stat_off[ch.src]; d.inv_scale = d.loc + 2 * C;
      break;
  }
  return d;
}

bool channel_present(const aurora_hip_step_io& io, const Channel& ch) {
  switch (ch.kind) {
    case SRC_SURF: return io.surf[ch.src] != nullptr;
    case SRC_STATIC: return io.stat != nullptr && io.stat[ch.src] != nullptr;
    case SRC_ATMOS: return io.atmos[ch.src] != nullptr;
    default: return true;
  }
}

struct Step {
  Model& m;
  Launcher L;
// ... 399 lines not shown
  const std::string& name = hg.names[hi];
  aurora_unpatch_var d = plain_unpatch(s.io.out_atmos[v], m.stats.f() + m.atmos_stat_off[v], s.C,
                                       s.clamp_now && index_of(m.pos_atmos, name) >= 0, (int)hi * s.PP);
  diff_fields(s, d, name, hg.names, true, v, s.C);
  if (m.variant == 1 && m.use_lora && name == "so2")
    for (int c = 0; c < s.C; ++c)
      if (m.levels[c] >= 850) d.clamp_max1_levels |= 1u << c;
  return d;
}

void decode_surface(Step& s, const float* x_cat) {
  Model& m = s.m;
  const int B = s.B, D2 = 2 * s.D;
  const int64_t Lp = s.Lp;
  const HeadGroup& hs = m.head_surf;
  const int n_s = (int)hs.names.size() * s.PP, ld_s = round_up(n_s, 4);
  float* y_s = (float*)m.arena.take((size_t)B * Lp * ld_s * 4);
  for (int b = 0; b < B; ++b)
    s.L.linear(LinearOp(x_cat + (size_t)b * s.Cl * Lp * D2, D2, hs.w.f(), D2, hs.b.f(), y_s + (size_t)b * Lp * ld_s, ld_s, Lp, n_s, D2,
                        AURORA_F32));
  std::vector<aurora_unpatch_var> ud;
  for (size_t v = 0; v < m.surf_out.size(); ++v) {
    const int src = index_of(m.surf_inputs, m.surf_out[v]);
    REQUIRE(src >= 0, "surface output '%s' is not a surface input", m.surf_out[v].c_str());
    if (s.io.out_surf[v] == nullptr || s.io.surf[src] == nullptr) continue;
    ud.push_back(surf_unpatch(s, hs, v, src));
  }
  in_launches_of_32(s, K_UNPATCHIFY, ud, [&](const aurora_unpatch_var* d, int n, int) {
    return aurora_hip_unpatchify(y_s, ld_s, d, n, B, 1, s.Hp, s.Wp, s.P, s.L.stream);
  });
}

void decode_group(Step& s, const HeadGroup& hg, const Resampler& rs, const float* q, float out_bound, bool scan_ctx, const float* ctx) {
  Model& m = s.m;
  const int B = s.B, C = s.C, Cl = s.Cl, D2 = 2 * s.D;
  const int64_t Lp = s.Lp;
  const size_t gmark = m.arena.top;
  const auto& last_ly = rs.layers.back();
  const bool last_pairs = last_ly.fc1_s && last_ly.fc2_s && last_ly.dim % 32 == 0;
  const bool two_term = hg.n_pad > 0 && last_pairs && out_bound < F16_SAFE;
  ResamplerCall call{};
  call.rs = &rs;
  call.ctx = ctx;
  call.ctx_rows = (int64_t)B * (Cl - 1) * Lp;
  call.ctx_dim = D2;
  call.q0 = q;
  call.latents0 = m.dec_queries.f();
  call.g.B = B; call.g.cols = Lp; call.g.kv_bstride = (int64_t)(Cl - 1) * Lp; call.g.kv_lstride = Lp;
  call.g.Lq = C; call.g.Lk = Cl - 1; call.g.heads = m.perceiver_heads;
  call.eps = m.ln_eps;
  call.out_pairs = two_term;
  call.front = nullptr;
  call.guard = CtxGuard{m.ctx_max.f() + 3, 1.0f, 0.0f, F16_SAFE, false, scan_ctx};
  float* lat = resampler(m, s.L, call);
  const int n_a = two_term ? hg.n_pad : (int)hg.names.size() * s.PP, ld_a = round_up(n_a, 4);
  const float* hw = two_term ? (const float*)hg.ws.p : hg.w.f();
  const float* hb = two_term ? hg.bs.f() : hg.b.f();
  const int mode = two_term ? (2 | AURORA_F32_A_SPLIT | AURORA_F32_W_SPLIT) : -1;
  float* y_a = (float*)m.arena.take((size_t)B * Lp * C * ld_a * 4);
  if (hg.groups > 1)
    s.L.linear(LinearOp(lat, (int64_t)C * D2, hw, D2, hb, y_a, (int64_t)C * ld_a, (int64_t)B * Lp, n_a, D2, AURORA_F32)
                   .f32_mode(mode).batched(C, D2, (int64_t)n_a * D2, ld_a, ld_a));
  else
    s.L.linear(LinearOp(lat, D2, hw, D2, hb, y_a, ld_a, (int64_t)B * Lp * C, n_a, D2, AURORA_F32).f32_mode(mode));
  std::vector<aurora_unpatch_var> ad;
  for (size_t hi = 0; hi < hg.names.size(); ++hi) {
    const int v = index_of(m.atmos_vars, hg.names[hi]);
    if (v < 0) continue;
    if (s.io.out_atmos[v] == nullptr || s.io.atmos[v] == nullptr) continue;
    ad.push_back(atmos_unpatch(s, hg, hi, v));
  }
  in_launches_of_32(s, K_UNPATCHIFY, ad, [&](const aurora_unpatch_var* d, int n, int) {
    return aurora_hip_unpatchify(y_a, ld_a, d, n, B, C, s.Hp, s.Wp, s.P, s.L.stream);
  });
  m.arena.top = gmark;
}

void decode_levels(Step& s, const float* x_cat) {
  Model& m = s.m;
  const int B = s.B, Cl = s.Cl, D2 = 2 * s.D;
  const int64_t Lp = s.Lp;
  const float* ctx = x_cat + (size_t)Lp * D2;
  if (B > 1) {
    float* ctx_copy = (float*)m.arena.take((size_t)B * (Cl - 1) * Lp * D2 * 4);
    for (int b = 0; b < B; ++b)
      timed(m, s.L.stream, K_COPY2D, 0.0, [&] {
        return aurora_hip_copy2d(x_cat + ((size_t)b * Cl * Lp + Lp) * D2, D2, ctx_copy + (size_t)b * (Cl - 1) * Lp * D2, D2,
                                 (int64_t)(Cl - 1) * Lp, D2, AURORA_F32, s.L.stream);
      });
    ctx = ctx_copy;
  }
  if (!m.head_main.names.empty()) decode_group(s, m.head_main, m.dec_rs, m.dec_q.f(), m.dec_out_bound, true, ctx);
  if (m.has_alt && !m.head_alt.names.empty())
    decode_group(s, m.head_alt, m.dec_rs_alt, m.dec_q_alt.f(), m.dec_out_bound_alt, m.head_main.names.empty(), ctx);
}

}

void run_step(Model& m, const StepIO& sio, void* stream) {
  const aurora_hip_step_io& io = *sio.io;
  const int new_step = io.rollout_step + 1;
  Step s{m, Launcher{m, stream}, io, sio.B, sio.T, m.P, m.D, m.Hp, m.Wp, m.Cl, m.n_levels, m.P * m.P, (int64_t)m.Hp * m.Wp,
         m.sharded(), m.band.rank, m.band.world,
         m.clamp_first ? new_step >= 1 : new_step > 1,
         m.autocast, m.bb(), m.bbs()};
  Arena& A = m.arena;
  A.top = 0;
  const int B = s.B, D = s.D, n = m.n_stages;
  const int64_t L0 = (int64_t)s.Cl * s.Lp;
  if (!m.dry) ok(aurora_hip_zero_words(m.ctx_max.f(), 4, stream));
  if (!m.dry)
    for (int i = 0; i < 4; ++i) { m.guard_limit_min[i] = INFINITY; m.guard_launches[i] = 0; }

  float* xf = (float*)A.take((size_t)B * L0 * D * 4);
  void* xb = s.bf ? A.take((size_t)B * L0 * D * 2) : nullptr;
  const size_t after_x = A.top;
  const float* xs1 = encode_surface(s);
  const float* lat = encode_levels(s);
  assemble(s, xs1, lat, xf, xb);
  A.top = after_x;

  const AttnSet& aw = attn_weights(m, lora_key(m, io.rollout_step), stream);
  float* x_cat = (float*)A.take((size_t)B * L0 * 2 * D * 4);
  std::vector<float*> skips;
  size_t bi = 0;
  for (int i = 0; i < n; ++i) {
    for (int k = 0; k < m.enc_depths[i]; ++k, ++bi) block(s, m.blocks[bi], aw.qkv[bi], aw.proj[bi], i, xf, xb, nullptr, 0);
    skips.push_back(xf);
    if (i < n - 1) merge_stage(s, i, xf, xb);
  }
  for (int i = 0; i < n; ++i) {
    const bool last_layer = i == n - 1;
    for (int k = 0; k < m.dec_depths[i]; ++k, ++bi)
      block(s, m.blocks[bi], aw.qkv[bi], aw.proj[bi], n - 1 - i, xf, xb, last_layer && k == m.dec_depths[i] - 1 ? x_cat : nullptr, 2 * D);
    if (last_layer && m.dec_depths[i] == 0 && !m.dry) ok(aurora_hip_copy2d(xf, D, x_cat, 2 * D, (int64_t)B * L0, D, AURORA_F32, stream));
    if (i < n - 1) split_stage(s, i, skips, xf, xb);
  }
  timed(m, stream, K_COPY2D, 0.0, [&] { return aurora_hip_copy2d(skips[0], D, x_cat + D, 2 * D, (int64_t)B * L0, D, AURORA_F32, stream); });

  const size_t mark = A.top;
  decode_surface(s, x_cat);
  decode_levels(s, x_cat);
  A.top = mark;
}
// ... 3 lines not shown
```

aurora_amd/engine/lib.py:

```python

from __future__ import annotations

import ctypes
import os
import threading
from collections import namedtuple
from ctypes import c_float, c_int, c_int32, c_int64, c_void_p
from pathlib import Path
from typing import Optional

import numpy as np
import torch

from aurora_amd.engine.tables import DeviceTables, _upload

F32, BF16, F64 = 0, 1, 2
ACT_NONE, ACT_GELU, ACT_SILU = 0, 1, 2

_LIB_PATH = Path(__file__).resolve().parents[1] / "_lib" / "libaurora_hip.so"


class PatchVar(ctypes.Structure):
    _fields_ = [
        ("src", c_void_p), ("stride_b", c_int64), ("stride_t", c_int64), ("stride_c", c_int64),
        ("stride_h", c_int64), ("stride_w", c_int64), ("loc", c_void_p), ("inv_scale", c_void_p),
        ("transform", c_int32), ("tw0", c_float), ("tw1", c_float), ("tb", c_float),
    ]


class UnpatchVar(ctypes.Structure):
    _fields_ = [("dst", c_void_p), ("loc", c_void_p), ("scale", c_void_p),
                ("clamp_min0", c_int32), ("col0", c_int32), ("lvl_stride", c_int32), ("mod_col0", c_int32),
                ("prev", c_void_p), ("prev_sb", c_int64), ("prev_sc", c_int64), ("prev_sh", c_int64),
                ("inv_scale", c_void_p), ("clamp_max1_levels", ctypes.c_uint32),
                ("angle_col0", c_int32), ("dens_col0", c_int32), ("mask", c_void_p), ("mask_sh", c_int64),
                ("mask_thresh", c_float)]


def unpatch_var(dst: int, loc: int, scale: int, clamp_min0: int, col0: int) -> UnpatchVar:
    d = UnpatchVar(dst, loc, scale, clamp_min0, col0)
    d.mod_col0 = d.angle_col0 = d.dens_col0 = -1
    return d


_SIGNATURES = {
    "aurora_hip_version": (c_int, []),
    "aurora_hip_last_error": (ctypes.c_char_p, []),
    "aurora_hip_default_f32_gemm": (c_int, []),
    "aurora_hip_linear_ex": (c_int, [c_void_p, c_int64, c_void_p, c_int64, c_void_p, c_void_p, c_int64,
                                     c_void_p, c_int64, c_void_p, c_int64, c_int64, c_int, c_int, c_int,
                                     c_int, c_int, c_void_p, c_float, c_void_p]),
    "aurora_hip_linear_workspace": (c_int64, [c_int64, c_int, c_int, c_int]),
    "aurora_hip_linear_ws": (c_int, [c_void_p, c_int64, c_void_p, c_int64, c_void_p, c_void_p, c_int64, c_void_p, c_int64,
                                     c_void_p, c_int64, c_int64, c_int, c_int, c_int, c_int, c_void_p, c_int64, c_void_p,
                                     c_int, c_int, c_void_p]),
    "aurora_hip_linear_batched": (c_int, [c_void_p, c_int64, c_void_p, c_int64, c_void_p, c_void_p, c_int64, c_int64, c_int,
                                          c_int, c_int, c_int, c_int, c_void_p, c_float, c_int, c_int64, c_int64, c_int64,
                                          c_int64, c_void_p]),
    "aurora_hip_linear_plan": (c_int, [c_int64, c_int, c_int, c_int, c_int, c_int, c_int, c_int64, c_int64, c_int64, c_int64,
                                       c_int64, c_int64, c_int64, c_int, c_int, c_int64, c_int, c_int,
                                       ctypes.POINTER(c_int32)]),
    "aurora_hip_absmax": (c_int, [c_void_p, c_int64, c_void_p, c_void_p]),
    "aurora_hip_absmax_fold": (c_int, [c_void_p, c_int64, c_void_p, c_void_p]),
    "aurora_hip_zero_words": (c_int, [c_void_p, c_int, c_void_p]),
    "aurora_hip_linear_layernorm": (c_int, [c_void_p, c_int64, c_void_p, c_int64, c_void_p, c_void_p, c_void_p, c_void_p,
                                            c_int64, c_void_p, c_int64, c_void_p, c_int64, c_int64, c_int, c_int, c_float,
                                            c_void_p]),
    "aurora_hip_split_f16": (c_int, [c_void_p, c_int64, c_void_p, c_int64, c_int64, c_int, c_float, c_void_p]),
    "aurora_hip_layernorm_split": (c_int, [c_void_p, c_int64, c_void_p, c_void_p, c_void_p, c_int64, c_int64, c_int,
                                           c_void_p, c_int64, c_void_p, c_int64, c_int64, c_int, c_float, c_void_p]),
    "aurora_hip_linear": (c_int, [c_void_p, c_int64, c_void_p, c_int64, c_void_p, c_void_p, c_int64,
                                  c_void_p, c_int64, c_void_p, c_int64, c_int64, c_int, c_int, c_int,
                                  c_int, c_void_p]),
    "aurora_hip_window_attention": (c_int, [c_void_p, c_void_p, c_void_p, c_void_p, c_void_p, c_int,
                                            c_int64, c_int64, c_int, c_int, c_int, c_int, c_int, c_void_p]),
    "aurora_hip_window_attention_planes": (c_int, [c_void_p, c_int64, c_void_p, c_void_p, c_void_p, c_void_p, c_int,
                                                   c_int64, c_int64, c_int, c_int, c_int, c_int, c_int, c_void_p]),
    "aurora_hip_linear_planes": (c_int, [c_void_p, c_int64, c_void_p, c_int64, c_void_p, c_void_p, c_int64, c_int, c_int64,
                                         c_int, c_int, c_int, c_void_p]),
    "aurora_hip_gather_rows": (c_int, [c_void_p, c_int64, c_void_p, c_void_p, c_int64, c_int64, c_int64,
                                       c_void_p]),
    "aurora_hip_layernorm": (c_int, [c_void_p, c_int64, c_void_p, c_void_p, c_void_p, c_int64, c_int64,
                                     c_void_p, c_int64, c_void_p, c_int64, c_int64, c_int, c_float,
                                     c_int, c_void_p]),
    "aurora_hip_merge_ln": (c_int, [c_void_p, c_void_p, c_void_p, c_void_p, c_int, c_int, c_int, c_int,
                                    c_int, c_float, c_int, c_void_p]),
    "aurora_hip_split_ln": (c_int, [c_void_p, c_void_p, c_void_p, c_void_p, c_int, c_int, c_int, c_int,
                                    c_int, c_int, c_int, c_float, c_int, c_void_p]),
    "aurora_hip_patchify": (c_int, [ctypes.POINTER(PatchVar), c_int, c_void_p, c_int64, c_int, c_int,
                                    c_int, c_int, c_int, c_int, c_int, c_int, c_int, c_void_p]),
    "aurora_hip_patchify_absmax": (c_int, [ctypes.POINTER(PatchVar), c_int, c_void_p, c_int64, c_int, c_int,
                                           c_int, c_int, c_int, c_int, c_int, c_int, c_int, c_void_p, c_void_p]),
    "aurora_hip_perceiver_attention": (c_int, [c_void_p, c_int64, c_void_p, c_void_p, c_int, c_int64,
                                               c_int64, c_int64, c_int, c_int, c_int, c_int, c_int,
                                               c_void_p]),
    "aurora_hip_perceiver_attention_ex": (c_int, [c_void_p, c_int64, c_void_p, c_void_p, c_int, c_int64,
                                                  c_int64, c_int64, c_int, c_int, c_int, c_int, c_int,
                                                  c_void_p, c_float, c_void_p]),
    "aurora_hip_perceiver_attention_unless": (c_int, [c_void_p, c_int64, c_void_p, c_void_p, c_int, c_int64,
                                                      c_int64, c_int64, c_int, c_int, c_int, c_int, c_int,
                                                      c_void_p, c_float, c_void_p, c_float, c_void_p]),
    "aurora_hip_perceiver_out_supported": (c_int, [c_int, c_int, c_int, c_int, c_int]),
    "aurora_hip_perceiver_probs": (c_int, [c_void_p, c_void_p, c_void_p, c_void_p, c_int, c_int64, c_int64, c_int64,
                                           c_int, c_int, c_int, c_int, c_void_p, c_float, c_void_p]),
    "aurora_hip_perceiver_attention_scores": (c_int, [c_void_p, c_int64, c_int, c_void_p, c_int, c_int64, c_int64, c_int64,
                                                      c_int, c_int, c_int, c_int, c_void_p, c_float, c_void_p, c_float,
                                                      c_void_p]),
    "aurora_hip_perceiver_probs_scores": (c_int, [c_void_p, c_int64, c_int, c_void_p, c_void_p, c_int, c_int64, c_int64,
                                                  c_int64, c_int, c_int, c_int, c_int, c_void_p, c_float, c_void_p]),
    "aurora_hip_perceiver_out": (c_int, [c_void_p, c_void_p, c_int64, c_void_p, c_void_p, c_void_p, c_int64, c_int64,
                                         c_int, c_int, c_int, c_int, c_int, c_void_p, c_float, c_void_p]),
    "aurora_hip_assemble_tokens": (c_int, [c_void_p, c_void_p, c_void_p, c_void_p, c_void_p, c_void_p,
                                           c_int, c_int, c_int64, c_int, c_int, c_void_p]),
    "aurora_hip_unpatchify": (c_int, [c_void_p, c_int64, ctypes.POINTER(UnpatchVar), c_int, c_int,
                                      c_int, c_int, c_int, c_int, c_void_p]),
    "aurora_hip_copy2d": (c_int, [c_void_p, c_int64, c_void_p, c_int64, c_int64, c_int64, c_int,
                                  c_void_p]),
    "aurora_hip_convert": (c_int, [c_void_p, c_void_p, c_int64, c_int, c_void_p]),
    "aurora_hip_regrid_plan": (c_int, [c_void_p, c_int, c_void_p, c_int, c_void_p, c_int, c_void_p, c_int, c_void_p,
                                       c_void_p, c_void_p, c_void_p]),
    "aurora_hip_regrid": (c_int, [c_void_p, c_int, c_void_p, c_int, c_int, c_int, c_void_p, c_void_p, c_int, c_void_p,
                                  c_void_p, c_int, c_void_p]),
    "aurora_hip_conservative_regrid": (c_int, [c_void_p, c_int, c_void_p, c_int, c_int, c_int, c_int, c_int, c_void_p, c_void_p,
# ... 358 lines not shown
        with _Timed("window_attention_bf16", 4.0 * B * n_windows * n_tok * D * 2):
            _check(load().aurora_hip_window_attention_planes(_ptr(qkv), plane_stride, _ptr(qkv_bias), _ptr(out), _ptr(tok), _ptr(grp),
                                                             B, L, L_out, D, heads, n_windows, n_tok, dtype_code(qkv.dtype),
                                                             _stream()))
        return out
    assert qkv.is_contiguous() and out.is_contiguous() and qkv.numel() == B * L * 3 * D
    assert out.numel() == B * L_out * D and out.dtype == qkv.dtype
    assert tok.dtype == torch.int32 and tok.is_contiguous() and tok.dim() == 2
    assert grp is None or (grp.dtype == torch.uint8 and grp.shape == tok.shape and grp.is_contiguous())
    assert qkv_bias is None or (qkv_bias.dtype == torch.float32 and qkv_bias.numel() == 3 * D)
    n_windows, n_tok = tok.shape
    name = "window_attention_bf16" if qkv.dtype == torch.bfloat16 else "window_attention_f32"
    with _Timed(name, 4.0 * B * n_windows * n_tok * D * qkv.element_size()):
        _check(load().aurora_hip_window_attention(_ptr(qkv), _ptr(qkv_bias), _ptr(out), _ptr(tok), _ptr(grp),
                                                  B, L, L_out, D, heads, n_windows, n_tok,
                                                  dtype_code(qkv.dtype), _stream()))
    return out


def layernorm(y: torch.Tensor, gain: Optional[torch.Tensor], shift: Optional[torch.Tensor], *,
              res: Optional[torch.Tensor] = None, res_mod: int = 0,
              out_f32: Optional[torch.Tensor] = None, out_t: Optional[torch.Tensor] = None,
              eps: float = 1e-5, d: Optional[int] = None, split_t: bool = False, split_res: bool = False) -> None:
    ldy, dy = _rows(y)
    D = d if d is not None else dy
    M = y.shape[0]
    for v in (gain, shift):
        assert v is None or (v.dtype == torch.float32 and v.numel() >= D and v.is_contiguous())
    ldr = ldo = ldt = 0
    if res is not None:
        assert res.dtype == torch.float32
        ldr, _ = _rows(res)
    if out_f32 is not None:
        assert out_f32.dtype == torch.float32 and out_f32.shape[0] == M
        ldo, _ = _rows(out_f32)
    if out_t is not None:
        assert out_t.dtype == y.dtype and out_t.shape[0] == M
        ldt, _ = _rows(out_t)
    nbytes = M * D * (y.element_size() + (4 if res is not None else 0) + (4 if out_f32 is not None else 0)
                      + (y.element_size() if out_t is not None else 0))
    if split_t or split_res:
        assert y.dtype == torch.float32 and (out_t is not None) == split_t and (res is not None or not split_res)
        with _Timed("layernorm", float(nbytes)):
            _check(load().aurora_hip_layernorm_split(_ptr(y), ldy, _ptr(gain), _ptr(shift), _ptr(res), ldr, res_mod,
                                                     1 if split_res else 0, _ptr(out_f32), ldo, _ptr(out_t), ldt, M, D,
                                                     eps, _stream()))
        return
    with _Timed("layernorm", float(nbytes)):
        _check(load().aurora_hip_layernorm(_ptr(y), ldy, _ptr(gain), _ptr(shift), _ptr(res), ldr, res_mod,
                                           _ptr(out_f32), ldo, _ptr(out_t), ldt, M, D, eps,
                                           dtype_code(y.dtype), _stream()))


def merge_ln(x: torch.Tensor, ln_w: torch.Tensor, ln_b: torch.Tensor, out: torch.Tensor,
             B: int, C: int, H: int, W: int, D: int, eps: float = 1e-5) -> torch.Tensor:
    assert x.dtype == torch.float32 and x.is_contiguous() and x.numel() == B * C * H * W * D
    assert out.is_contiguous() and out.numel() == B * C * ((H + 1) // 2) * ((W + 1) // 2) * 4 * D
    with _Timed("merge_ln", 0.0):
        _check(load().aurora_hip_merge_ln(_ptr(x), _ptr(ln_w), _ptr(ln_b), _ptr(out), B, C, H, W, D, eps,
                                          dtype_code(out.dtype), _stream()))
    return out


def split_ln(y: torch.Tensor, ln_w: torch.Tensor, ln_b: torch.Tensor, out: torch.Tensor,
             B: int, C: int, H: int, W: int, Dq: int, crop_h: int, crop_w: int,
             eps: float = 1e-5) -> torch.Tensor:
    assert y.is_contiguous() and y.numel() == B * C * H * W * 4 * Dq and y.dtype == out.dtype
    assert out.is_contiguous() and out.numel() == B * C * (2 * H - crop_h) * (2 * W - crop_w) * Dq
    with _Timed("split_ln", 0.0):
        _check(load().aurora_hip_split_ln(_ptr(y), _ptr(ln_w), _ptr(ln_b), _ptr(out), B, C, H, W, Dq,
                                          crop_h, crop_w, eps, dtype_code(y.dtype), _stream()))
    return out


def patchify(desc: list[PatchVar], out: torch.Tensor, k_offset: int, k_total: int, B: int, T: int,
             n_lvl: int, Hp: int, Wp: int, P: int, absmax: Optional[torch.Tensor] = None) -> None:
    Kpad = out.shape[1]
    assert out.is_contiguous() and out.shape[0] == n_lvl * B * Hp * Wp
    assert absmax is None or (absmax.dtype == torch.float32 and absmax.numel() >= 1)
    arr = (PatchVar * len(desc))(*desc)
    with _Timed("patchify", 0.0):
        _check(load().aurora_hip_patchify_absmax(arr, len(desc), _ptr(out), Kpad, k_offset, k_total, B, T, n_lvl,
                                                 Hp, Wp, P, dtype_code(out.dtype), _ptr(absmax), _stream()))


def perceiver_attention(q: torch.Tensor, q_col_stride: int, kv: torch.Tensor, out: torch.Tensor,
                        B: int, cols_per_b: int, kv_bstride: int, kv_lstride: int, Lq: int, Lk: int,
                        heads: int, head_dim: int, pair_guard=None, skip_guard=None) -> torch.Tensor:
    assert q.is_contiguous() and kv.is_contiguous() and out.is_contiguous()
    assert q.dtype == kv.dtype == out.dtype
    word, limit = pair_guard if pair_guard is not None else (None, 0.0)
    sword, slimit = skip_guard if skip_guard is not None else (None, 0.0)
    with _Timed("perceiver_attention", 0.0):
        _check(load().aurora_hip_perceiver_attention_unless(_ptr(q), q_col_stride, _ptr(kv), _ptr(out), B,
                                                            cols_per_b, kv_bstride, kv_lstride, Lq, Lk, heads,
                                                            head_dim, dtype_code(q.dtype), _ptr(word), float(limit),
                                                            _ptr(sword), float(slimit), _stream()))
    return out


def perceiver_probs(q: torch.Tensor, kv: torch.Tensor, B: int, cols_per_b: int, kv_bstride: int, kv_lstride: int,
                    Lq: int, Lk: int, heads: int, head_dim: int, guard=None):
    assert q.is_contiguous() and kv.is_contiguous() and q.dtype == kv.dtype == torch.float32
    n_cols, inner = B * cols_per_b, heads * head_dim
    P = torch.zeros((n_cols, heads, 64), device=kv.device, dtype=torch.float32)
    Vp = torch.zeros((n_cols * Lk, inner), device=kv.device, dtype=torch.float32)
# ... 810 lines not shown
              ("tcwv", tcwv), ("ivtu", ivtu), ("ivtv", ivtv), ("ivt", ivt))
    tensors = [t for _, fs in groups if fs is not None for t in fs if t is not None]
    if not tensors:
        return
    dev = tensors[0].device
    assert all(t.device == dev for t in tensors), "diagnostics: every tensor must be on one device"
    if row_table is not None:
        _operand("diagnostics", "row_table", row_table, torch.float64, f"fp64 {(n_lat, 4)}", dev=dev, anchor="the fields", shape=(n_lat, 4))
    if level_w is not None:
        _operand("diagnostics", "level_w", level_w, torch.float64, "fp64 vector", dev=dev, anchor="the fields", dim=1)
    addr = {}
    for what, fs in groups:
        if fs is None:
            continue
        if what in ("vo", "div", "ws") and any(t is None for t in fs):
            assert u is not None and len(fs) == len(u), f"diagnostics: {what} with None entries must have an entry per u entry"
            addr[what] = [a for t, like in zip(fs, u) for a in
                          ([0] * (like.numel() // (n_lat * n_lon)) if t is None else _plane_addresses("diagnostics", [t], n_lat, n_lon, what))]
        else:
            addr[what] = _plane_addresses("diagnostics", fs, n_lat, n_lon, what)
    n_wind, n_cols = len(addr.get("u", ())), 0
    C = 0 if level_w is None else level_w.shape[0]
    for what in ("v", "vo", "div", "ws"):
        assert what not in addr or len(addr[what]) == n_wind, f"diagnostics: {what} holds {len(addr[what])} planes, u {n_wind}"
    if q is not None:
        assert C >= 1 and len(addr["q"]) % C == 0, f"diagnostics: q holds {len(addr['q'])} planes, which is no multiple of the {C} level weights"
        n_cols = len(addr["q"]) // C
        for what in ("col_u", "col_v"):
            assert what not in addr or len(addr[what]) == n_cols * C, f"diagnostics: {what} holds {len(addr[what])} planes, q {n_cols * C}"
        for what in ("tcwv", "ivtu", "ivtv", "ivt"):
            assert what not in addr or len(addr[what]) == n_cols, f"diagnostics: {what} holds {len(addr[what])} planes for {n_cols} columns"
    if n_wind == 0 and n_cols == 0:
        return
    planes = _planes("diagnostics", [], dev)
    for what, addresses in addr.items():
        planes.add(what, addresses)
    at = planes.upload()
    moved = 4.0 * n_lat * n_lon * (n_wind * (2 + sum(k in addr for k in ("vo", "div", "ws"))) +
                                   n_cols * (C * (1 + sum(k in addr for k in ("col_u", "col_v"))) +
                                             sum(k in addr for k in ("tcwv", "ivtu", "ivtv", "ivt"))))
    _launch(dev, "diagnostics", moved, "aurora_hip_diagnostics", at.get("u"), at.get("v"), at.get("vo"), at.get("div"), at.get("ws"), n_wind,
            _ptr(row_table), float(L), 1 if wrap else 0, at.get("q"), at.get("col_u"), at.get("col_v"), at.get("tcwv"), at.get("ivtu"),
            at.get("ivtv"), at.get("ivt"), n_cols, C, _ptr(level_w), n_lat, n_lon)


_PD = ctypes.POINTER(ctypes.c_double)
_PF = ctypes.POINTER(ctypes.c_float)
_PS = ctypes.POINTER(ctypes.c_char_p)


class HipTuning(ctypes.Structure):
    _fields_ = [("fuse_ln", c_int32), ("band_split_attention", c_int32), ("qkv_planes", c_int32), ("split_k", c_int32),
                ("perceiver_reassoc", c_int32), ("score_weights", c_int32), ("compose_front", c_int32),
                ("reserved", c_int32 * 1)]


def tuning_from_env() -> HipTuning:
    t = HipTuning()

    def value(var: str, allowed: tuple[int, ...]):
        raw = os.environ.get(var)
        if raw is None:
            return None
        try:
            v = int(raw.strip())
        except ValueError:
            v = None
        if v not in allowed:
            raise ValueError(f"{var}={raw!r}: expected one of {', '.join(map(str, allowed))}")
        return v

    v = value("AURORA_FUSE_LN", (0, 1, 2))
    if v is not None:
        t.fuse_ln = v + 1
    for field, var in (("band_split_attention", "AURORA_BAND_SPLIT_ATTENTION"), ("qkv_planes", "AURORA_QKV_PLANES"),
                       ("split_k", "AURORA_SPLIT_K"), ("perceiver_reassoc", "AURORA_PERCEIVER_REASSOC"),
                       ("score_weights", "AURORA_SCORE_WEIGHTS"), ("compose_front", "AURORA_COMPOSE_FRONT")):
        v = value(var, (0, 1))
        if v is not None:
            setattr(t, field, 2 if v else 1)
    return t


class HipConfig(ctypes.Structure):
    _fields_ = [("embed_dim", c_int32), ("patch_size", c_int32), ("latent_levels", c_int32), ("num_heads", c_int32),
                ("n_stages", c_int32), ("encoder_depths", c_int32 * 4), ("encoder_heads", c_int32 * 4),
                ("decoder_depths", c_int32 * 4), ("decoder_heads", c_int32 * 4), ("window", c_int32 * 3),
                ("enc_depth", c_int32), ("dec_depth", c_int32), ("perceiver_ln_eps", c_float),
                ("max_history", c_int32), ("timestep_hours", ctypes.c_double), ("stabilise_level_agg", c_int32),
                ("use_lora", c_int32), ("lora_steps", c_int32), ("lora_mode", c_int32), ("autocast", c_int32),
                ("n_surf", c_int32), ("n_static", c_int32), ("n_atmos", c_int32),
                ("surf_vars", _PS), ("static_vars", _PS), ("atmos_vars", _PS),
                ("variant", c_int32), ("n_level_condition", c_int32), ("level_condition", _PD),
                ("dynamic_vars", c_int32), ("atmos_static_vars", c_int32), ("clamp_at_first_step", c_int32),
                ("simulate_indexing_bug", c_int32),
                ("n_separate_perceiver", c_int32), ("separate_perceiver", _PS),
                ("n_modulation_heads", c_int32), ("modulation_heads", _PS),
                ("difference_history", ctypes.POINTER(c_int32)),
                ("n_positive_surf", c_int32), ("positive_surf_vars", _PS),
                ("n_positive_atmos", c_int32), ("positive_atmos_vars", _PS),
                ("n_surf_inputs", c_int32), ("surf_inputs", _PS),
                ("n_density", c_int32), ("density_channel_surf_vars", _PS),
                ("n_angle", c_int32), ("angle_surf_vars", _PS), ("tuning", HipTuning)]


class HipHaloMsg(ctypes.Structure):
    _fields_ = [("peer", c_int32), ("reserved", c_int32), ("offset", c_int64), ("bytes", c_int64)]


HALO_POST_FN = ctypes.CFUNCTYPE(c_int, c_void_p, ctypes.POINTER(HipHaloMsg), c_int32, ctypes.POINTER(HipHaloMsg), c_int32,
                                c_void_p)
HALO_WAIT_FN = ctypes.CFUNCTYPE(c_int, c_void_p, c_void_p)


class HipBand(ctypes.Structure):
    _fields_ = [("rank", c_int32), ("world", c_int32), ("post", HALO_POST_FN), ("wait", HALO_WAIT_FN), ("user", c_void_p)]


class HipGrid(ctypes.Structure):
    _fields_ = [("n_lat", c_int32), ("n_lon", c_int32), ("lat", _PD), ("lon", _PD), ("n_levels", c_int32),
                ("levels", _PD), ("levels_float32", c_int32), ("surf_loc", _PD), ("surf_scale", _PD),
                ("static_loc", _PD), ("static_scale", _PD), ("atmos_loc", _PD), ("atmos_scale", _PD),
                ("pos_encoding", _PF), ("scale_encoding", _PF)]


class HipStepIO(ctypes.Structure):
    _fields_ = [("B", c_int32), ("T", c_int32), ("surf", ctypes.POINTER(c_void_p)), ("surf_strides", c_int64 * 4),
                ("stat", ctypes.POINTER(c_void_p)), ("static_strides", c_int64 * 2),
                ("atmos", ctypes.POINTER(c_void_p)), ("atmos_strides", c_int64 * 5),
                ("out_surf", ctypes.POINTER(c_void_p)), ("out_atmos", ctypes.POINTER(c_void_p)),
                ("rollout_step", c_int32)]


class HipProfileEntry(ctypes.Structure):
    _fields_ = [("kernel", ctypes.c_char_p), ("launches", c_int64), ("ms", ctypes.c_double), ("work", ctypes.c_double)]


class HipPlanInfo(ctypes.Structure):
    _fields_ = [("n_windows", c_int32), ("win_tokens", c_int32), ("n_own", c_int32), ("n_halo", c_int32),
                ("n_interior", c_int32), ("recv_offset", c_int32 * 2), ("recv_count", c_int32 * 2),
                ("send_count", c_int32 * 2), ("has_groups", c_int32)]


PROFILE_KINDS = ("linear_bf16", "linear_f32", "window_attention_bf16", "layernorm", "merge_ln", "split_ln", "patchify",
                 "perceiver_attention", "assemble_tokens", "unpatchify", "copy2d", "absmax", "linear_layernorm_bf16",
                 "gather_rows", "perceiver_out")

_SIGNATURES.update({
    "aurora_hip_profile_begin": (c_int, [c_void_p, ctypes.c_uint32]),
    "aurora_hip_profile_end": (c_int, [c_void_p, ctypes.POINTER(HipProfileEntry), c_int, ctypes.POINTER(c_int)]),
    "aurora_hip_profile_end_list": (c_int, [c_void_p, ctypes.POINTER(HipProfileEntry), c_int, ctypes.POINTER(c_int)]),
    "aurora_hip_create": (c_int, [ctypes.POINTER(HipConfig), ctypes.POINTER(c_void_p)]),
    "aurora_hip_destroy": (None, [c_void_p]),
    "aurora_hip_pack_weights": (c_int, [c_void_p, ctypes.c_char_p, c_void_p, ctypes.POINTER(c_int64), c_int, c_int, c_int]),
    "aurora_hip_finalize": (c_int, [c_void_p, c_void_p]),
    "aurora_hip_save_packed": (c_int, [c_void_p, ctypes.c_char_p, c_void_p]),
    "aurora_hip_load_packed": (c_int, [c_void_p, ctypes.c_char_p]),
    "aurora_hip_precompute": (c_int, [c_void_p, ctypes.POINTER(HipGrid), c_void_p]),
    "aurora_hip_set_time": (c_int, [c_void_p, _PD, c_int, c_void_p]),
    "aurora_hip_step": (c_int, [c_void_p, ctypes.POINTER(HipStepIO), c_void_p]),
    "aurora_hip_workspace_bytes": (c_int64, [c_void_p]),
    "aurora_hip_guard_words": (c_int, [c_void_p, ctypes.POINTER(c_float), c_void_p]),
    "aurora_hip_guard_limits": (c_int, [c_void_p, ctypes.POINTER(c_float)]),
    "aurora_hip_abi_sizes": (c_int, [ctypes.POINTER(c_int32), c_int]),
    "aurora_hip_generation": (c_int64, [c_void_p]),
    "aurora_hip_compose_weight": (c_int, [_PF, c_int, c_int, _PF, c_int, c_int, _PF]),
    "aurora_hip_compose_bias": (c_int, [_PF, c_int, c_int, _PF, c_int, _PF]),
    "aurora_hip_compose_front_rule": (c_int, [c_int, c_int, ctypes.POINTER(c_int32), c_int]),
    "aurora_hip_composed_value_bound": (c_int, [c_float, c_float, c_float, c_float, c_float, _PF]),
    "aurora_hip_front_composed": (c_int, [c_void_p]),
    "aurora_hip_output_vars": (c_int, [c_void_p, _PS, c_int]),
    "aurora_hip_set_time_ex": (c_int, [c_void_p, _PD, ctypes.POINTER(c_int32), c_int, c_void_p]),
    "aurora_hip_set_band": (c_int, [c_void_p, ctypes.POINTER(HipBand)]),
    "aurora_hip_band_rows": (c_int, [c_void_p, ctypes.POINTER(c_int32), ctypes.POINTER(c_int32)]),
    "aurora_hip_band_staging_bytes": (c_int64, [c_void_p]),
    "aurora_hip_set_band_staging": (c_int, [c_void_p, c_void_p, c_void_p, c_int64]),
    "aurora_hip_pos_scale_encoding": (c_int, [_PD, _PD, c_int, c_int, c_int, c_int, _PF, _PF]),
    "aurora_hip_band_partition": (c_int, [c_int, ctypes.POINTER(c_int32), ctypes.POINTER(c_int32), c_int, c_int, c_int,
                                          ctypes.POINTER(c_int32), ctypes.POINTER(c_int32)]),
    "aurora_hip_band_plan": (c_int, [ctypes.POINTER(c_int32), ctypes.POINTER(c_int32), c_int, c_int, c_int,
                                     ctypes.POINTER(c_int32), ctypes.POINTER(HipPlanInfo), c_void_p, c_void_p, c_void_p,
                                     c_void_p]),
})
EXPORTED_SYMBOLS = tuple(_SIGNATURES)
```

aurora_amd/engine/native.py:

```python
from __future__ import annotations

import ctypes
from datetime import timedelta

import numpy as np
import torch

from aurora_amd import normalisation
from aurora_amd.batch import BandBatch, Batch, derive_metadata
from aurora_amd.engine import encodings, lib

_LORA_MODES = {"single": 0, "from_second": 1, "all": 2}
_VARIANTS = {"base": 0, "air_pollution": 1, "wave": 2}


def _version(t: torch.Tensor) -> int:
    try:
        return t._version
    except RuntimeError:
        return -1


def _strs(names):
    return (ctypes.c_char_p * max(len(names), 1))(*[n.encode() for n in names])
# ... 253 lines not shown
                need = L.aurora_hip_band_staging_bytes(self._h)
                if self.transport.send is None or self.transport.send.numel() < need:
                    self.transport.allocate(need)
                lib._check(L.aurora_hip_set_band_staging(self._h, self.transport.send.data_ptr(), self.transport.recv.data_ptr(),
                                                         self.transport.send.numel()))
            self._grid_key = key
        self._grid_ident = ident
        self._keep_coords = (lat, lon)

    def full_lat(self):
        return self._keep_coords[0] if getattr(self, "_keep_coords", None) is not None else None

    def profile_begin(self, only=None) -> None:
        mask = 0
        for i, k in enumerate(lib.PROFILE_KINDS):
            if only is None or k in only:
                mask |= 1 << i
        lib._check(lib.load().aurora_hip_profile_begin(self._h, mask))

    def profile_end(self) -> dict:
        out = (lib.HipProfileEntry * len(lib.PROFILE_KINDS))()
        n = ctypes.c_int(0)
        lib._check(lib.load().aurora_hip_profile_end(self._h, out, len(out), ctypes.byref(n)))
        return {e.kernel.decode(): {"launches": e.launches, "ms": e.ms, "work": e.work} for e in out[:n.value] if e.launches}

    def profile_end_list(self) -> list:
        n = ctypes.c_int(0)
        lib._check(lib.load().aurora_hip_profile_end_list(self._h, None, 0, ctypes.byref(n)))
        out = (lib.HipProfileEntry * max(n.value, 1))()
        lib._check(lib.load().aurora_hip_profile_end_list(self._h, out, n.value, ctypes.byref(n)))
        return [(e.kernel.decode(), e.ms, e.work) for e in out[:n.value]]

    def set_time(self, times) -> None:
        stamps = _dbl([t.timestamp() / 3600 for t in times])
        cal = _i32([x for t in times for x in (t.hour, t.weekday(), t.day)])
        lib._check(lib.load().aurora_hip_set_time_ex(self._h, stamps, cal, len(times), lib._stream()))

    def workspace_bytes(self) -> int:
        return int(lib.load().aurora_hip_workspace_bytes(self._h))

    def guard_words(self) -> tuple[float, float, float, float]:
        out = (ctypes.c_float * 4)()
        lib._check(lib.load().aurora_hip_guard_words(self._h, out, lib._stream()))
        return tuple(float(v) for v in out)

    def guard_limits(self) -> tuple[tuple[float, float, float, float], tuple[int, int, int, int]]:
        out = (ctypes.c_float * 8)()
        lib._check(lib.load().aurora_hip_guard_limits(self._h, out))
        return tuple(float(v) for v in out[:4]), tuple(int(v) for v in out[4:])

    def front_composed(self) -> bool:
        return bool(lib.load().aurora_hip_front_composed(self._h))

    def generation(self) -> int:
        return int(lib.load().aurora_hip_generation(self._h))

    @torch.no_grad()
    def step(self, batch: Batch, upload_time: bool = True, out=None) -> Batch:
        cfg = self.cfg
        md = batch.metadata
        levels = tuple(md.atmos_levels)
        H, W = batch.spatial_shape
        first = next(iter(batch.surf_vars.values()))
        B, T = first.shape[:2]
        dev = first.device
        assert md.lat.shape[0] == H and md.lon.shape[-1] == W
        assert md.lat.dtype in (torch.float32, torch.float64), f"Latitude num. unstable: {md.lat.dtype}."
        assert md.lon.dtype in (torch.float32, torch.float64), f"Longitude num. unstable: {md.lon.dtype}."
        if self.shard is None:
            self.precompute(md.lat, md.lon, levels)
        else:
            assert self.band_rows is not None and H == self.band_rows[1] - self.band_rows[0], "not this rank's latitude band"
        if upload_time:
            self.set_time(md.time)

        def unknown(d_, known, what):
            extra = [k for k in d_ if k not in known]
            if extra:
                raise KeyError(f"{what} variable(s) {extra} are not variables of this model")

        unknown(batch.surf_vars, self.surf_inputs, "surface-level")
        unknown(batch.static_vars, cfg.static_vars, "static")
        unknown(batch.atmos_vars, cfg.atmos_vars, "atmospheric")

        def same_strides(ts):
            ts = [None if t is None else (t if t.dtype == torch.float32 else t.float()) for t in ts]
            real = [t for t in ts if t is not None]
            if len({t.stride() for t in real}) > 1 or any(t.stride(-1) != 1 for t in real):
                ts = [None if t is None else t.contiguous() for t in ts]
            return ts

        surf = same_strides([batch.surf_vars.get(n) for n in self.surf_inputs])
        stat = same_strides([batch.static_vars.get(n) for n in cfg.static_vars])
        atmos = same_strides([batch.atmos_vars.get(n) for n in cfg.atmos_vars])

        def dest(kind, name, shape):
            t = None if out is None else out[kind].get(name)
            if (t is not None and tuple(t.shape) == shape and t.dtype == torch.float32 and t.is_contiguous()
                    and t.device == dev):
                return t
            return torch.empty(shape, dtype=torch.float32, device=dev)

        have_s, have_a = set(batch.surf_vars), set(batch.atmos_vars)
        out_s = [dest(0, n, (B, 1, H, W)) if n in have_s else None for n in self.surf_outputs]
        out_a = [dest(1, n, (B, 1, len(levels), H, W)) if n in have_a else None for n in cfg.atmos_vars]
        ptrs = lambda ts: (ctypes.c_void_p * max(len(ts), 1))(*[None if t is None else t.data_ptr() for t in ts])
# ... 32 lines not shown
```

include/aurora_hip.h:

```cpp
#ifndef AURORA_HIP_H
#define AURORA_HIP_H

#include <stddef.h>
#include <stdint.h>

#ifdef __cplusplus
extern "C" {
#endif

#define AURORA_F32 0
#define AURORA_BF16 1
#define AURORA_F64 2

#define AURORA_OK 0
#define AURORA_E_ARG (-1)
#define AURORA_E_LAUNCH (-2)

#define AURORA_ACT_NONE 0
#define AURORA_ACT_GELU 1
#define AURORA_ACT_SILU 2

const char* aurora_hip_last_error(void);
int aurora_hip_version(void);

int aurora_hip_linear(const void* A, int64_t lda, const void* W, int64_t ldw, const float* bias,
                      void* C, int64_t ldc, void* C2, int64_t ldc2,
                      const float* residual, int64_t ldr,
                      int64_t M, int N, int K, int dtype, int act, void* stream);

int aurora_hip_linear_ex(const void* A, int64_t lda, const void* W, int64_t ldw, const float* bias,
                         void* C, int64_t ldc, void* C2, int64_t ldc2,
                         const float* residual, int64_t ldr,
                         int64_t M, int N, int K, int dtype, int act,
                         int f32_gemm, const float* guard, float guard_limit, void* stream);
int aurora_hip_default_f32_gemm(void);
int aurora_hip_linear_batched(const void* A, int64_t lda, const void* W, int64_t ldw, const float* bias, void* C, int64_t ldc,
                              int64_t M, int N, int K, int dtype, int act, int f32_gemm, const float* guard,
                              float guard_limit, int batch, int64_t stride_a, int64_t stride_w, int64_t stride_bias,
                              int64_t stride_c, void* stream);

#define AURORA_PLAN_F32_THREE 0
#define AURORA_PLAN_F32_TWO 1
#define AURORA_PLAN_F32_PP 2
#define AURORA_PLAN_F32_PP_W 3
#define AURORA_PLAN_F32_PP_AW 4
#define AURORA_PLAN_F32_PP_W_TALL 5
#define AURORA_PLAN_F32_PP_AW_TALL 6
#define AURORA_PLAN_TILE128 7
#define AURORA_PLAN_RING 8
#define AURORA_PLAN_RING_MID 9
#define AURORA_PLAN_PP 10
#define AURORA_PLAN_PP_SPLITK 11
#define AURORA_PLAN_A4 12
int aurora_hip_linear_plan(int64_t M, int N, int K, int dtype, int f32_gemm, int has_guard, int batch, int64_t ldc,
                           int64_t c_addr, int64_t ldc2, int64_t c2_addr, int64_t ldr, int64_t residual_addr,
                           int64_t workspace_bytes, int n_tickets, int split, int64_t plane_stride, int plane_heads,
                           int cus, int32_t* plan_out);

int64_t aurora_hip_linear_workspace(int64_t M, int N, int K, int dtype);
int aurora_hip_linear_ws(const void* A, int64_t lda, const void* W, int64_t ldw, const float* bias, void* C, int64_t ldc,
                         void* C2, int64_t ldc2, const float* residual, int64_t ldr, int64_t M, int N, int K, int dtype,
                         int act, void* workspace, int64_t workspace_bytes, int32_t* tickets, int n_tickets, int split,
                         void* stream);

int aurora_hip_linear_planes(const void* A, int64_t lda, const void* W, int64_t ldw, const float* bias, void* C,
                             int64_t plane_stride, int heads, int64_t M, int N, int K, int dtype, void* stream);

#define AURORA_F32_A_SPLIT 4
#define AURORA_F32_W_SPLIT 8
#define AURORA_F32_C_SPLIT 16
int aurora_hip_split_f16(const float* src, int64_t ld_src, void* dst, int64_t ld_dst, int64_t rows, int K,
                         float scale, void* stream);

int aurora_hip_absmax(const float* x, int64_t n, float* out, void* stream);
int aurora_hip_absmax_fold(const float* x, int64_t n, float* out, void* stream);
int aurora_hip_zero_words(float* words, int n, void* stream);

int aurora_hip_window_attention(const void* qkv, const float* qkv_bias, void* out,
                                const int32_t* tok, const uint8_t* grp,
                                int B, int64_t L, int64_t L_out, int D, int heads, int n_windows,
                                int win_tokens, int dtype, void* stream);
int aurora_hip_window_attention_planes(const void* qkv, int64_t plane_stride, const float* qkv_bias, void* out,
                                       const int32_t* tok, const uint8_t* grp,
                                       int B, int64_t L, int64_t L_out, int D, int heads, int n_windows,
                                       int win_tokens, int dtype, void* stream);

int aurora_hip_layernorm(const void* y, int64_t ldy, const float* gain, const float* shift,
                         const float* res, int64_t ldr, int64_t res_mod,
                         float* out_f32, int64_t ldo, void* out_t, int64_t ldt,
                         int64_t M, int D, float eps, int dtype, void* stream);
int aurora_hip_linear_layernorm(const void* A, int64_t lda, const void* W, int64_t ldw, const float* bias,
                                const float* gain, const float* shift,
                                const float* x_in, int64_t ldx, float* x_out, int64_t ldo,
                                void* x_bf16, int64_t ldb, int64_t M, int N, int K, float eps, void* stream);

int aurora_hip_layernorm_split(const float* y, int64_t ldy, const float* gain, const float* shift,
                               const void* res, int64_t ldr, int64_t res_mod, int res_is_split,
                               float* out_f32, int64_t ldo, void* out_split, int64_t ld_split,
                               int64_t M, int D, float eps, void* stream);

int aurora_hip_merge_ln(const float* x, const float* ln_w, const float* ln_b, void* out,
                        int B, int C, int H, int W, int D, float eps, int dtype, void* stream);

int aurora_hip_split_ln(const void* y, const float* ln_w, const float* ln_b, void* out,
                        int B, int C, int H, int W, int Dq, int crop_h, int crop_w, float eps,
                        int dtype, void* stream);

typedef struct aurora_patch_var {
  const float* src;
  int64_t stride_b;
  int64_t stride_t;
  int64_t stride_c;
  int64_t stride_h;
  int64_t stride_w;
  const float* loc;
  const float* inv_scale;
  int32_t transform;
  float tw0, tw1, tb;
} aurora_patch_var;

int aurora_hip_patchify(const aurora_patch_var* desc, int n_vars, void* out, int64_t Kpad,
                        int k_offset, int K_total, int B, int T, int n_lvl, int Hp, int Wp, int P,
                        int dtype, void* stream);
int aurora_hip_patchify_absmax(const aurora_patch_var* desc, int n_vars, void* out, int64_t Kpad,
                               int k_offset, int K_total, int B, int T, int n_lvl, int Hp, int Wp, int P,
                               int dtype, float* absmax, void* stream);

int aurora_hip_perceiver_attention(const void* q, int64_t q_col_stride, const void* kv, void* out,
                                   int B, int64_t cols_per_b, int64_t kv_bstride, int64_t kv_lstride,
                                   int Lq, int Lk, int heads, int head_dim, int dtype, void* stream);
int aurora_hip_perceiver_attention_ex(const void* q, int64_t q_col_stride, const void* kv, void* out,
                                      int B, int64_t cols_per_b, int64_t kv_bstride, int64_t kv_lstride,
                                      int Lq, int Lk, int heads, int head_dim, int dtype,
                                      const float* pair_guard, float pair_limit, void* stream);
int aurora_hip_perceiver_attention_unless(const void* q, int64_t q_col_stride, const void* kv, void* out,
                                          int B, int64_t cols_per_b, int64_t kv_bstride, int64_t kv_lstride,
                                          int Lq, int Lk, int heads, int head_dim, int dtype,
                                          const float* pair_guard, float pair_limit, const float* skip_guard,
                                          float skip_limit, void* stream);

int aurora_hip_perceiver_out_supported(int Lq, int Lk, int heads, int head_dim, int N);
int aurora_hip_perceiver_probs(const float* q, const float* kv, float* P, void* Vp, int B, int64_t cols_per_b,
                               int64_t kv_bstride, int64_t kv_lstride, int Lq, int Lk, int heads, int head_dim,
                               const float* guard, float guard_limit, void* stream);
int aurora_hip_perceiver_attention_scores(const float* vs, int64_t ld_vs, int s_off, void* out, int B, int64_t cols_per_b,
                                          int64_t kv_bstride, int64_t kv_lstride, int Lq, int Lk, int heads, int head_dim,
                                          const float* pair_guard, float pair_limit, const float* skip_guard, float skip_limit,
                                          void* stream);
int aurora_hip_perceiver_probs_scores(const float* vs, int64_t ld_vs, int s_off, float* P, void* Vp, int B, int64_t cols_per_b,
                                      int64_t kv_bstride, int64_t kv_lstride, int Lq, int Lk, int heads, int head_dim,
                                      const float* guard, float guard_limit, void* stream);
int aurora_hip_perceiver_out(const void* Vp, const void* W_pairs, int64_t ldw, const float* P, const float* bias,
// ... 19 lines not shown
  int32_t angle_col0;
  int32_t dens_col0;
  const float* mask;
  int64_t mask_sh;
  float mask_thresh;
} aurora_unpatch_var;

int aurora_hip_unpatchify(const float* y, int64_t ldy, const aurora_unpatch_var* desc, int n_vars,
                          int B, int n_lvl, int Hp, int Wp, int P, void* stream);

int aurora_hip_copy2d(const void* src, int64_t lds_, void* dst, int64_t ldd, int64_t rows,
                      int64_t cols, int dtype, void* stream);
int aurora_hip_gather_rows(const void* src, int64_t src_pitch_bytes, const int32_t* idx, void* dst,
                           int64_t dst_pitch_bytes, int64_t n_rows, int64_t row_bytes, void* stream);
int aurora_hip_convert(const void* src, void* dst, int64_t n, int src_dtype, void* stream);

typedef struct aurora_hip_model aurora_hip_model;

typedef struct aurora_hip_config {
  int32_t embed_dim, patch_size, latent_levels, num_heads;
  int32_t n_stages;
  int32_t encoder_depths[4], encoder_heads[4], decoder_depths[4], decoder_heads[4];
  int32_t window[3];
  int32_t enc_depth, dec_depth;
  float perceiver_ln_eps;
  int32_t max_history;
  double timestep_hours;
  int32_t stabilise_level_agg, use_lora, lora_steps, lora_mode;
  int32_t autocast;
  int32_t n_surf, n_static, n_atmos;
  const char* const* surf_vars;
  const char* const* static_vars;
  const char* const* atmos_vars;
  int32_t variant;
  int32_t n_level_condition;
  const double* level_condition;
  int32_t dynamic_vars, atmos_static_vars, clamp_at_first_step, simulate_indexing_bug;
  int32_t n_separate_perceiver;  const char* const* separate_perceiver;
  int32_t n_modulation_heads;    const char* const* modulation_heads;
  const int32_t* difference_history;
  int32_t n_positive_surf;       const char* const* positive_surf_vars;
  int32_t n_positive_atmos;      const char* const* positive_atmos_vars;
  int32_t n_surf_inputs;         const char* const* surf_inputs;
  int32_t n_density;             const char* const* density_channel_surf_vars;
  int32_t n_angle;               const char* const* angle_surf_vars;
  struct aurora_hip_tuning {
    int32_t fuse_ln;
    int32_t band_split_attention;
    int32_t qkv_planes;
    int32_t split_k;
    int32_t perceiver_reassoc;
    int32_t score_weights;
    int32_t compose_front;
    int32_t reserved[1];
  } tuning;
} aurora_hip_config;

typedef struct aurora_hip_grid {
  int32_t n_lat, n_lon;
  const double* lat;
  const double* lon;
  int32_t n_levels;
  const double* levels;
  int32_t levels_float32;
  const double* surf_loc;
  const double* surf_scale;
  const double* static_loc;
  const double* static_scale;
  const double* atmos_loc;
  const double* atmos_scale;
  const float* pos_encoding;
  const float* scale_encoding;
} aurora_hip_grid;

typedef struct aurora_hip_step_io {
  int32_t B, T;
  const float* const* surf;
  int64_t surf_strides[4];
  const float* const* stat;
  int64_t static_strides[2];
  const float* const* atmos;
  int64_t atmos_strides[5];
  float* const* out_surf;
  float* const* out_atmos;
  int32_t rollout_step;
} aurora_hip_step_io;

int aurora_hip_create(const aurora_hip_config* config, aurora_hip_model** out);
void aurora_hip_destroy(aurora_hip_model* model);
int aurora_hip_pack_weights(aurora_hip_model* model, const char* name, const void* data, const int64_t* shape, int ndim,
                            int dtype, int on_device);
int aurora_hip_finalize(aurora_hip_model* model, void* stream);
int aurora_hip_save_packed(aurora_hip_model* model, const char* path, void* stream);
int aurora_hip_load_packed(aurora_hip_model* model, const char* path);
int aurora_hip_precompute(aurora_hip_model* model, const aurora_hip_grid* grid, void* stream);
int aurora_hip_pos_scale_encoding(const double* lat, const double* lon, int n_lat, int n_lon, int patch_size,
                                  int embed_dim, float* pos_out, float* scale_out);
int aurora_hip_set_time(aurora_hip_model* model, const double* time_hours, int B, void* stream);
int aurora_hip_step(aurora_hip_model* model, const aurora_hip_step_io* io, void* stream);
int64_t aurora_hip_workspace_bytes(const aurora_hip_model* model);
#define AURORA_F16_SAFE_RANGE 16384.0f
int aurora_hip_guard_words(const aurora_hip_model* model, float out[4], void* stream);
int aurora_hip_guard_limits(const aurora_hip_model* model, float out[8]);
int aurora_hip_compose_weight(const float* w_ctx, int N, int D, const float* w_e, int K, int groups, float* out);
int aurora_hip_compose_bias(const float* w_ctx, int N, int D, const float* bias, int C, float* out);
int aurora_hip_compose_front_rule(int Kpad, int D, const int32_t* N, int n_layers);
int aurora_hip_composed_value_bound(float v_l1, float embed_l1, float embed_bias_max, float composed_v_l1,
                                    float composed_vb_max, float out[6]);
int aurora_hip_front_composed(const aurora_hip_model* model);
int64_t aurora_hip_generation(const aurora_hip_model* model);
int aurora_hip_abi_sizes(int32_t* out, int capacity);
int aurora_hip_output_vars(const aurora_hip_model* model, const char** names, int capacity);
int aurora_hip_set_time_ex(aurora_hip_model* model, const double* time_hours, const int32_t* calendar, int B, void* stream);

typedef struct aurora_hip_halo_msg {
  int32_t peer;
  int32_t reserved;
  int64_t offset;
  int64_t bytes;
} aurora_hip_halo_msg;
typedef int (*aurora_hip_halo_post_fn)(void* user, const aurora_hip_halo_msg* sends, int32_t n_sends,
                                       const aurora_hip_halo_msg* recvs, int32_t n_recvs, void* stream);
typedef int (*aurora_hip_halo_wait_fn)(void* user, void* stream);
typedef struct aurora_hip_band {
  int32_t rank, world;
  aurora_hip_halo_post_fn post;
  aurora_hip_halo_wait_fn wait;
  void* user;
} aurora_hip_band;
int aurora_hip_set_band(aurora_hip_model* model, const aurora_hip_band* band);
int aurora_hip_band_rows(const aurora_hip_model* model, int32_t* row0, int32_t* row1);
int64_t aurora_hip_band_staging_bytes(const aurora_hip_model* model);
int aurora_hip_set_band_staging(aurora_hip_model* model, void* send, void* recv, int64_t staging_bytes);
typedef struct aurora_hip_plan_info {
  int32_t n_windows, win_tokens, n_own, n_halo, n_interior;
  int32_t recv_offset[2], recv_count[2], send_count[2];
  int32_t has_groups;
} aurora_hip_plan_info;
int aurora_hip_band_partition(int n_stages, const int32_t res0[3], const int32_t window[3], int world, int rank, int stage,
                              int32_t* h0, int32_t* h1);
int aurora_hip_band_plan(const int32_t res[3], const int32_t window[3], int shifted, int world, int rank,
                         const int32_t* rows, aurora_hip_plan_info* info, int32_t* tok, uint8_t* grp,
                         int32_t* send_idx_prev, int32_t* send_idx_next);

typedef struct aurora_hip_profile_entry {
  const char* kernel;
  int64_t launches;
  double ms;
  double work;
} aurora_hip_profile_entry;
int aurora_hip_profile_begin(aurora_hip_model* model, uint32_t kind_mask);
int aurora_hip_profile_end(aurora_hip_model* model, aurora_hip_profile_entry* out, int capacity, int* n_out);
int aurora_hip_profile_end_list(aurora_hip_model* model, aurora_hip_profile_entry* out, int capacity, int* n_out);

int aurora_hip_regrid_plan(const double* lat, int n_lat, const double* lon, int n_lon, const double* lat_new, int n_lat_new,
                           const double* lon_new, int n_lon_new, int32_t* rows, double* row_w, int32_t* cols,
                           double* col_w);
int aurora_hip_regrid(const void* const* src_planes, int src_dtype, float* const* dst_planes, int n_planes, int n_lat,
                      int n_lon, const int32_t* rows, const double* row_w, int n_rows_out, const int32_t* cols,
                      const double* col_w, int n_cols_out, void* stream);

int aurora_hip_conservative_regrid(const void* const* src_planes, int src_dtype, float* const* dst_planes, int n_planes,
// ... 100 lines not shown
```

Measured before the change: 7.976 forecast-steps/s.

## Fuse decoder tail LayerNorm and residual into the fp32 head GEMM A-side load

Adds an A-side LayerNorm variant of the fp32 fp16-pair GEMM that normalises raw fp32 rows with precomputed row statistics, applies gain, shift and a pair-layout residual, and splits to fp16 pairs in registers. The decoder heads now compute only row statistics and feed the raw latent into this kernel, instead of first writing a normalised, split activation. This is meant to remove a full LayerNorm-and-split pass over the decoder latent, at the cost of a shallower two-stage pipeline with full vmcnt(0) waits and extra per-tile ALU and residual loads. It is enabled by default through a new tuning flag.

```diff
diff --git a/aurora_amd/csrc/gemm.hip b/aurora_amd/csrc/gemm.hip
--- a/aurora_amd/csrc/gemm.hip
+++ b/aurora_amd/csrc/gemm.hip
@@ -485,6 +485,7 @@
   int batch = 1; int64_t stride_a = 0, stride_w = 0, stride_bias = 0, stride_c = 0;
   const SplitWs* ws = nullptr;
   int64_t plane_stride = 0; int plane_heads = 0;
+  const float *ln_stats = nullptr, *ln_gain = nullptr, *ln_shift = nullptr; const void* ln_res = nullptr; int64_t ln_ldr = 0;
   int pre = 0, mode = 0;
   int es() const { return dtype == AURORA_F32 ? 4 : 2; }
 };
@@ -512,6 +513,13 @@
                    "linear: a pre-split activation operand needs pre-split weights");
   AURORA_CHECK_ARG(!(c.pre & AURORA_F32_C_SPLIT) || (c.C2 == nullptr && c.ldc % 32 == 0 && ((uintptr_t)c.C % 16) == 0),
                    "linear: fp16-pair output needs ldc %% 32 == 0, 16-byte alignment and no second output");
+  AURORA_CHECK_ARG(c.ln_stats == nullptr ||
+                       (c.pre == AURORA_F32_W_SPLIT && c.K <= 2048 && c.ln_gain && c.ln_shift && c.ln_res && c.ln_ldr >= c.K &&
+                        c.ln_ldr % 32 == 0 && c.ln_ldr < (1 << 22) && ((uintptr_t)c.ln_res % 16) == 0 && ((uintptr_t)c.ln_stats % 8) == 0 &&
+                        ((uintptr_t)c.ln_gain % 16) == 0 && ((uintptr_t)c.ln_shift % 16) == 0 && c.batch == 1 &&
+                        c.C2 == nullptr && c.residual == nullptr && c.guard == nullptr),
+                   "linear: the A-side LayerNorm needs pre-split weights only (fp32 rows), K <= 2048, gain, shift and a pair-layout "
+                   "residual (stride %% 32 == 0, >= K), one problem, one output, no guard (K=%d)", c.K);
   if (!(c.mode == 2 || (c.mode == 1 && c.dtype == AURORA_F32))) c.guard = nullptr;
   AURORA_CHECK_ARG(c.M > 0 && c.N > 0 && c.K > 0, "linear: empty problem M=%lld N=%d K=%d", (long long)c.M, c.N, c.K);
   const int es = c.es();
@@ -530,7 +538,7 @@
   const int64_t M = c.M;
   const int N = c.N, K = c.K, dtype = c.dtype, pre = c.pre, mode = c.mode;
   const bool split = dtype == AURORA_F32 && mode >= 1;
-  const bool tall = pre != 0 && N % VN != 0;
+  const bool tall = pre != 0 && (N % VN != 0 || c.ln_stats != nullptr);
   bool big = (M >= 1024 || split) && (N % BN2 == 0 || tall);
   bool mid = false;
   int ksplit = 1;
@@ -564,6 +572,7 @@
                       : (pre & AURORA_F32_A_SPLIT) ? F32_PP_AW : (pre & AURORA_F32_W_SPLIT) ? F32_PP_W : F32_PP;
   if (mid) plan.kernel = K_RING_MID;
   else if (!big) plan.kernel = K_TILE_128;
+  else if (c.ln_stats) plan.kernel = F32_PP_LN_TALL;
   else if (pre) plan.kernel = pp;
   else if (split && mode == 1 && c.guard != nullptr) plan.kernel = F32_THREE;
   else if (split && mode == 2 && c.guard != nullptr) {
@@ -620,12 +629,13 @@
   p.bs_a = c.stride_a * es; p.bs_w = c.stride_w * es; p.bs_c = c.stride_c * es; p.bs_bias = c.stride_bias;
   p.split = plan.ksplit; p.slabs = plan.ksplit > 1 ? c.ws->slabs : nullptr; p.tickets = plan.ksplit > 1 ? c.ws->tickets : nullptr;
   p.plane_stride = c.plane_stride; p.plane_heads = c.plane_heads;
+  p.ln_stats = c.ln_stats; p.ln_gain = c.ln_gain; p.ln_shift = c.ln_shift; p.ln_res = (const char*)c.ln_res; p.ln_ldr_b = c.ln_ldr * 4;
   once_per_device([] {
     for (const auto& row : KERNELS)
       for (const LinearKernel& k : row)
         if (k.fn) (void)hipFuncSetAttribute((const void*)k.fn, hipFuncAttributeMaxDynamicSharedMemorySize, k.lds_bytes);
   });
-  if (plan.kernel < F32_KERNELS) {
+  if (plan.kernel < F32_KERNELS || plan.kernel == F32_PP_LN_TALL) {
     if (plan.kernel >= F32_PP) {
       const bool tall = plan.kernel >= F32_PP_W_TALL;
       LinearArgs q = p;
@@ -725,6 +735,16 @@
   LinearCall c = plain_call(A, lda, W, ldw, bias, C, ldc, nullptr, 0, nullptr, 0, M, N, K, dtype, act, stream);
   c.f32_gemm = f32_gemm; c.guard = guard; c.guard_limit = guard_limit;
   c.batch = batch; c.stride_a = stride_a; c.stride_w = stride_w; c.stride_bias = stride_bias; c.stride_c = stride_c;
+  return linear_impl(c);
+}
+
+extern "C" int aurora_hip_linear_a_layernorm(const float* y, int64_t ldy, const float* stats, const float* gain, const float* shift,
+                                             const void* res_pairs, int64_t ldr, const void* W_pairs, int64_t ldw,
+                                             const float* bias, float* C, int64_t ldc, int64_t M, int N, int K, void* stream) {
+  AURORA_CHECK_ARG(stats != nullptr, "linear_a_layernorm: no row statistics");
+  LinearCall c = plain_call(y, ldy, W_pairs, ldw, bias, C, ldc, nullptr, 0, nullptr, 0, M, N, K, AURORA_F32, AURORA_ACT_NONE, stream);
+  c.f32_gemm = 2 | AURORA_F32_W_SPLIT;
+  c.ln_stats = stats; c.ln_gain = gain; c.ln_shift = shift; c.ln_res = res_pairs; c.ln_ldr = ldr;
   return linear_impl(c);
 }
 
diff --git a/aurora_amd/csrc/gemm_f32.hip b/aurora_amd/csrc/gemm_f32.hip
--- a/aurora_amd/csrc/gemm_f32.hip
+++ b/aurora_amd/csrc/gemm_f32.hip
@@ -209,12 +209,38 @@
 
 
 constexpr int VROW = 128, VTHREADS = 512, VNST = 3;
+constexpr int VLN_LDS = 16384;
+
+__device__ __forceinline__ Split2 ln_split8(u32x4 a, u32x4 b, float mean, float rstd, const f32x4 (&gn)[2], const f32x4 (&sh)[2],
+                                            u32x4 rh, u32x4 rl) {
+#pragma clang fp contract(off)
+  const float y[8] = {__uint_as_float(a.x), __uint_as_float(a.y), __uint_as_float(a.z), __uint_as_float(a.w),
+                      __uint_as_float(b.x), __uint_as_float(b.y), __uint_as_float(b.z), __uint_as_float(b.w)};
+  const float gv[8] = {gn[0].x, gn[0].y, gn[0].z, gn[0].w, gn[1].x, gn[1].y, gn[1].z, gn[1].w};
+  const float sv[8] = {sh[0].x, sh[0].y, sh[0].z, sh[0].w, sh[1].x, sh[1].y, sh[1].z, sh[1].w};
+  const uint32_t hw[4] = {rh.x, rh.y, rh.z, rh.w}, lw[4] = {rl.x, rl.y, rl.z, rl.w};
+  auto half = [](uint32_t w, int hi) { return (float)__builtin_bit_cast(_Float16, (uint16_t)(hi ? w >> 16 : w & 0xffffu)); };
+  float o[8];
+#pragma unroll
+  for (int j = 0; j < 8; ++j) {
+    float t = (y[j] - mean) * rstd;
+    t = t * gv[j];
+    t = t + sv[j];
+    const float r = half(hw[j >> 1], j & 1) + half(lw[j >> 1], j & 1);
+    o[j] = t + r;
+  }
+  uint32_t h[4], l[4];
+#pragma unroll
+  for (int q = 0; q < 4; ++q) split_pair_f16(o[2 * q], o[2 * q + 1], h[q], l[q]);
+  return Split2{u32x4{h[0], h[1], h[2], h[3]}, u32x4{l[0], l[1], l[2], l[3]}};
+}
 constexpr int VOPER_X = VM * VROW, VOPER_W = VN * VROW, VSTAGE = VOPER_X + VOPER_W;
 
-template <bool A_PRE, bool W_PRE, bool TALL = false>
+template <bool A_PRE, bool W_PRE, bool TALL = false, bool A_LN = false>
 __global__ __launch_bounds__(VTHREADS, 2) void linear_kernel_f32pp(const LinearArgs p_in) {
   constexpr int TM = TALL ? 256 : VM, TN = TALL ? 128 : VN, OPX = TM * VROW, XP = TM / 64, WP = TN / 64;
   static_assert(OPX + TN * VROW == VSTAGE && XP + WP == 6, "stage size / DMA count the waitcnt immediates assume");
+  static_assert(!A_LN || (!A_PRE && W_PRE && TALL), "the A-side LayerNorm form: fp32 rows, pre-split weights, 256 x 128 tiles");
   const LinearArgs p = batch_problem(p_in);
   extern __shared__ __attribute__((aligned(16))) char smem[];
   if (p.guard != nullptr && !(*p.guard < p.guard_limit)) return;
@@ -272,10 +298,49 @@
   zero_acc(acc);
 
   const int nt = p.k_tiles;
-  stage(0);
-  stage(1);
-  stage(2);
-  asm volatile("s_waitcnt vmcnt(12)" ::: "memory");
+  const char* res_tile = A_LN ? p.ln_res + m0 * p.ln_ldr_b : nullptr;
+  uint32_t res_x[A_LN ? 4 : 1];
+  f32x2_t st[A_LN ? 4 : 1];
+  u32x4 rh[A_LN ? 4 : 1], rl[A_LN ? 4 : 1];
+  const float* gs_lds = reinterpret_cast<const float*>(smem + VNST * VSTAGE);
+  const int K = nt * 32;
+  auto residual = [&](int kt) {
+#pragma unroll
+    for (int f = 0; f < 4; ++f) {
+      rh[f] = *reinterpret_cast<const u32x4*>(res_tile + (int64_t)kt * VROW + res_x[f]);
+      rl[f] = *reinterpret_cast<const u32x4*>(res_tile + (int64_t)kt * VROW + res_x[f] + 64);
+    }
+  };
+  if constexpr (A_LN) {
+    stage(0);
+    stage(1);
+    f32x4 gsv[2];
+#pragma unroll
+    for (int u = 0; u < 2; ++u) {
+      const int i = u * VTHREADS + tid;
+      if (4 * i < 2 * K) gsv[u] = *reinterpret_cast<const f32x4*>((4 * i < K ? p.ln_gain : p.ln_shift - K) + 4 * i);
+    }
+#pragma unroll
+    for (int f = 0; f < 4; ++f) {
+      int64_t gm = m0 + wm * 64 + 16 * f + i16;
+      gm = gm < p.M ? gm : p.M - 1;
+      res_x[f] = (uint32_t)(gm - m0) * (uint32_t)p.ln_ldr_b + (g << 4);
+      st[f] = reinterpret_cast<const f32x2_t*>(p.ln_stats)[gm];
+    }
+    residual(0);
+#pragma unroll
+    for (int u = 0; u < 2; ++u) {
+      const int i = u * VTHREADS + tid;
+      if (4 * i < 2 * K) *reinterpret_cast<f32x4*>(smem + VNST * VSTAGE + 16 * i) = gsv[u];
+    }
+    asm volatile("s_waitcnt vmcnt(0)" ::: "memory");
+    asm volatile("s_waitcnt lgkmcnt(0)" ::: "memory");
+  } else {
+    stage(0);
+    stage(1);
+    stage(2);
+    asm volatile("s_waitcnt vmcnt(12)" ::: "memory");
+  }
   __builtin_amdgcn_s_barrier();
   asm volatile("" ::: "memory");
   if (late == 1) __builtin_amdgcn_s_barrier();
@@ -289,24 +354,48 @@
       xa[f] = *reinterpret_cast<const u32x4*>(buf + off_x[f][0]);
       xb[f] = *reinterpret_cast<const u32x4*>(buf + off_x[f][1]);
     }
-#pragma unroll
-    for (int f = 0; f < 4; ++f)
-      if constexpr (W_PRE)
-        w[f] = Split2{*reinterpret_cast<const u32x4*>(buf + off_w[f][0]), *reinterpret_cast<const u32x4*>(buf + off_w[f][1])};
-      else
-        w[f] = split8_f16<true>(*reinterpret_cast<const u32x4*>(buf + off_w[f][0]), *reinterpret_cast<const u32x4*>(buf + off_w[f][1]));
-    if (s >= 1 && s + 2 < nt) stage(s + 2);
-    if (s + 2 < nt) asm volatile("s_waitcnt vmcnt(6)" ::: "memory");
-    else asm volatile("s_waitcnt vmcnt(0)" ::: "memory");
+    auto read_w = [&] {
+#pragma unroll
+      for (int f = 0; f < 4; ++f)
+        if constexpr (W_PRE)
+          w[f] = Split2{*reinterpret_cast<const u32x4*>(buf + off_w[f][0]), *reinterpret_cast<const u32x4*>(buf + off_w[f][1])};
+        else
+          w[f] = split8_f16<true>(*reinterpret_cast<const u32x4*>(buf + off_w[f][0]), *reinterpret_cast<const u32x4*>(buf + off_w[f][1]));
+    };
+    if constexpr (!A_LN) read_w();
+    f32x4 gn[A_LN ? 2 : 1], sh[A_LN ? 2 : 1];
+    if constexpr (A_LN) {
+#pragma unroll
+      for (int h = 0; h < 2; ++h) {
+        gn[h] = *reinterpret_cast<const f32x4*>(gs_lds + s * 32 + 8 * g + 4 * h);
+        sh[h] = *reinterpret_cast<const f32x4*>(gs_lds + K + s * 32 + 8 * g + 4 * h);
+      }
+      asm volatile("s_waitcnt vmcnt(0)" ::: "memory");
+    } else {
+      if (s >= 1 && s + 2 < nt) stage(s + 2);
+      if (s + 2 < nt) asm volatile("s_waitcnt vmcnt(6)" ::: "memory");
+      else asm volatile("s_waitcnt vmcnt(0)" ::: "memory");
+    }
     asm volatile("s_waitcnt lgkmcnt(0)" ::: "memory");
     __builtin_amdgcn_sched_barrier(0);
     __builtin_amdgcn_s_barrier();
     __builtin_amdgcn_sched_barrier(0);
     asm volatile("" ::: "memory");
+    if constexpr (A_LN) {
+#pragma unroll
+      for (int fm = 0; fm < 4; ++fm) {
+        const Split2 x = ln_split8(xa[fm], xb[fm], st[fm].x, st[fm].y, gn, sh, rh[fm], rl[fm]);
+        xa[fm] = x.h;
+        xb[fm] = x.l;
+      }
+      if (s + 1 < nt) residual(s + 1);
+      if (s + 2 < nt) stage(s + 2);
+      read_w();
+    }
 #pragma unroll
     for (int fm = 0; fm < 4; ++fm) {
       Split2 x;
-      if constexpr (A_PRE) x = Split2{xa[fm], xb[fm]};
+      if constexpr (A_PRE || A_LN) x = Split2{xa[fm], xb[fm]};
       else x = split8_f16<false>(xa[fm], xb[fm]);
 #pragma unroll
       for (int fn = 0; fn < 4; ++fn) acc[fn][fm] = mma_f16(w[fn].l, x.h, acc[fn][fm]);
@@ -442,7 +531,7 @@
 using namespace aurora;
 
 namespace {
-constexpr LinearKernel F32_TABLE[F32_KERNELS] = {
+constexpr LinearKernel F32_TABLE[F32_KERNELS + 1] = {
      {linear_kernel_256_f32x3<3>, THREADS2, NSTAGE2 * STAGE2},
      {linear_kernel_256_f32x3<2>, THREADS2, NSTAGE2 * STAGE2},
      {linear_kernel_f32pp<false, false>, VTHREADS, VNST * VSTAGE},
@@ -450,17 +539,18 @@
      {linear_kernel_f32pp<true, true>, VTHREADS, VNST * VSTAGE},
      {linear_kernel_f32pp<false, true, true>, VTHREADS, VNST * VSTAGE},
      {linear_kernel_f32pp<true, true, true>, VTHREADS, VNST * VSTAGE},
+     {linear_kernel_f32pp<false, true, true, true>, VTHREADS, VNST * VSTAGE + VLN_LDS},
 };
 }
 
 extern "C" __attribute__((visibility("hidden"))) int aurora_f32_launch(int kernel, const void* linear_args, unsigned n_blocks,
                                                                       unsigned batch, void* stream) {
   const LinearArgs& p = *static_cast<const LinearArgs*>(linear_args);
-  AURORA_CHECK_ARG(kernel >= 0 && kernel < F32_KERNELS, "linear: no fp32 kernel %d", kernel);
+  AURORA_CHECK_ARG((kernel >= 0 && kernel < F32_KERNELS) || kernel == F32_PP_LN_TALL, "linear: no fp32 kernel %d", kernel);
   once_per_device([] {
     for (const LinearKernel& k : F32_TABLE) (void)hipFuncSetAttribute((const void*)k.fn, hipFuncAttributeMaxDynamicSharedMemorySize, k.lds_bytes);
   });
-  const LinearKernel& k = F32_TABLE[kernel];
+  const LinearKernel& k = F32_TABLE[kernel == F32_PP_LN_TALL ? F32_KERNELS : kernel];
   hipLaunchKernelGGL(k.fn, dim3(n_blocks, batch), dim3(k.threads), k.lds_bytes, as_stream(stream), p);
   return 0;
 }
diff --git a/aurora_amd/csrc/gemm_tile.h b/aurora_amd/csrc/gemm_tile.h
--- a/aurora_amd/csrc/gemm_tile.h
+++ b/aurora_amd/csrc/gemm_tile.h
@@ -23,6 +23,7 @@
   int64_t bs_a, bs_w, bs_c, bs_bias;
   int split; float* slabs; int32_t* tickets;
   int64_t plane_stride; int plane_heads;
+  const float* ln_stats; const float* ln_gain; const float* ln_shift; const char* ln_res; int64_t ln_ldr_b;
 };
 
 template <typename T>
@@ -320,6 +321,7 @@
 struct LinearKernel { void (*fn)(LinearArgs); unsigned threads; int lds_bytes; };
 
 enum F32Kernel { F32_THREE, F32_TWO, F32_PP, F32_PP_W, F32_PP_AW, F32_PP_W_TALL, F32_PP_AW_TALL, F32_KERNELS };
+constexpr int F32_PP_LN_TALL = 64;
 
 }
 
diff --git a/aurora_amd/csrc/model.h b/aurora_amd/csrc/model.h
--- a/aurora_amd/csrc/model.h
+++ b/aurora_amd/csrc/model.h
@@ -213,6 +213,8 @@
   bool reassoc_out = true;
   bool compose_front = true;
   bool front_composed = false;
+  int ln_in_heads_used = 0;
+  bool ln_in_heads = true;
   bool score_weights = true;
 
   aurora::DevBuf abs_enc, dyn_planes, ctx_max;
@@ -301,6 +303,9 @@
   const float *res = nullptr, *guard = nullptr;
   int64_t ldc2 = 0, ldr = 0, sa = 0, sw = 0, sbias = 0, sc = 0;
   float limit = 0.f;
+  const float *ln_stats = nullptr, *ln_gain = nullptr, *ln_shift = nullptr;
+  const void* ln_res = nullptr;
+  int64_t ln_ldr = 0;
   LinearOp(const void* A_, int64_t lda_, const void* W_, int64_t ldw_, const float* bias_, void* C_, int64_t ldc_, int64_t M_, int N_,
            int K_, int dtype_)
       : A(A_), W(W_), bias(bias_), C(C_), lda(lda_), ldw(ldw_), ldc(ldc_), M(M_), N(N_), K(K_), dtype(dtype_) {}
@@ -310,6 +315,9 @@
   LinearOp& f32_mode(int mode) { f32_gemm = mode; return *this; }
   LinearOp& guarded_by(const float* word, float lim) { guard = word; limit = lim; return *this; }
   LinearOp& batched(int n, int64_t a, int64_t w, int64_t b, int64_t c) { batch = n; sa = a; sw = w; sbias = b; sc = c; return *this; }
+  LinearOp& a_layernorm(const float* stats, const float* gain, const float* shift, const void* res_pairs, int64_t ld) {
+    ln_stats = stats; ln_gain = gain; ln_shift = shift; ln_res = res_pairs; ln_ldr = ld; return *this;
+  }
 };
 
 struct PerceiverCols {
@@ -335,6 +343,9 @@
       if (ws)
         return aurora_hip_linear_ws(o.A, o.lda, o.W, o.ldw, o.bias, o.C, o.ldc, o.C2, o.ldc2, o.res, o.ldr, o.M, o.N, o.K, o.dtype,
                                     o.act, ws, ws_bytes, (int32_t*)m.tickets.p, SPLIT_TICKETS, 0, stream);
+      if (o.ln_stats)
+        return aurora_hip_linear_a_layernorm((const float*)o.A, o.lda, o.ln_stats, o.ln_gain, o.ln_shift, o.ln_res, o.ln_ldr, o.W, o.ldw,
+                                             o.bias, (float*)o.C, o.ldc, o.M, o.N, o.K, stream);
       if (o.batch > 1)
         return aurora_hip_linear_batched(o.A, o.lda, o.W, o.ldw, o.bias, o.C, o.ldc, o.M, o.N, o.K, o.dtype, o.act, o.f32_gemm,
                                          o.guard, o.limit, o.batch, o.sa, o.sw, o.sbias, o.sc, stream);
@@ -375,6 +386,9 @@
       return aurora_hip_layernorm_split(y, ldy, gain, shift, res, ldr, res_mod, res_is_split, out_f32, ldo, out_split, ld_split, M, D,
                                         eps, stream);
     });
+  }
+  void layernorm_stats(const float* y, int64_t ldy, int64_t M, int D, float eps, float* stats) {
+    timed(m, stream, K_LAYERNORM, 0.0, [&] { return aurora_hip_layernorm_stats(y, ldy, M, D, eps, stats, stream); });
   }
   void perceiver_attention(const PerceiverCols& g, int head_dim, const float* q, int64_t q_stride, const float* kv, float* att,
                            const float* pair_word, float pair_limit, const float* skip_word, float skip_limit) {
diff --git a/aurora_amd/csrc/model.hip b/aurora_amd/csrc/model.hip
--- a/aurora_amd/csrc/model.hip
+++ b/aurora_amd/csrc/model.hip
@@ -200,6 +200,7 @@
     m->reassoc_out = sw(tu.perceiver_reassoc, true, "perceiver_reassoc");
     m->score_weights = sw(tu.score_weights, true, "score_weights");
     m->compose_front = sw(tu.compose_front, true, "compose_front");
+    m->ln_in_heads = sw(tu.ln_in_heads, true, "ln_in_heads");
     m->tickets = DevBuf(SPLIT_TICKETS * sizeof(int32_t));
     hip_ok(hipMemset(m->tickets.p, 0, SPLIT_TICKETS * sizeof(int32_t)), "hipMemset");
     *out = m.release();
diff --git a/aurora_amd/csrc/model_weights.hip b/aurora_amd/csrc/model_weights.hip
--- a/aurora_amd/csrc/model_weights.hip
+++ b/aurora_amd/csrc/model_weights.hip
@@ -469,6 +469,7 @@
 }
 
 extern "C" int aurora_hip_front_composed(const aurora_hip_model* m) { return m != nullptr && m->front_composed ? 1 : 0; }
+extern "C" int aurora_hip_ln_in_heads_used(const aurora_hip_model* m) { return m != nullptr ? m->ln_in_heads_used : 0; }
 
 extern "C" int aurora_hip_pack_weights(aurora_hip_model* m, const char* name, const void* data, const int64_t* shape, int ndim,
                                        int dtype, int on_device) {
diff --git a/aurora_amd/csrc/norm.hip b/aurora_amd/csrc/norm.hip
--- a/aurora_amd/csrc/norm.hip
+++ b/aurora_amd/csrc/norm.hip
@@ -24,6 +24,28 @@
     if (lane + 64 * i < n_pieces) {
 #pragma unroll
       for (int j = 0; j < 8; ++j) {
+        const float d = v[i][j] - mean;
+        q = fmaf(d, d, q);
+      }
+    }
+  rstd = rsqrtf(wave_sum(q) * inv_d + eps);
+}
+
+template <int NC>
+__device__ __forceinline__ void row4_stats(const float (&v)[NC][4], int lane, int n_pieces, int D, float eps, float& mean,
+                                           float& rstd) {
+  float s = 0.f;
+#pragma unroll
+  for (int i = 0; i < NC; ++i)
+    if (lane + 64 * i < n_pieces) s += (v[i][0] + v[i][1]) + (v[i][2] + v[i][3]);
+  const float inv_d = 1.0f / D;
+  mean = wave_sum(s) * inv_d;
+  float q = 0.f;
+#pragma unroll
+  for (int i = 0; i < NC; ++i)
+    if (lane + 64 * i < n_pieces) {
+#pragma unroll
+      for (int j = 0; j < 4; ++j) {
         const float d = v[i][j] - mean;
         q = fmaf(d, d, q);
       }
@@ -59,23 +81,8 @@
         if (res_plain) load4(rr + (lane + 64 * i) * 4, r4[i]);
       }
     }
-  float s = 0.f;
-#pragma unroll
-  for (int i = 0; i < NC; ++i)
-    if (lane + 64 * i < n_pieces) s += (v[i][0] + v[i][1]) + (v[i][2] + v[i][3]);
-  const float inv_d = 1.0f / p.D;
-  const float mean = wave_sum(s) * inv_d;
-  float q = 0.f;
-#pragma unroll
-  for (int i = 0; i < NC; ++i)
-    if (lane + 64 * i < n_pieces) {
-#pragma unroll
-      for (int j = 0; j < 4; ++j) {
-        const float d = v[i][j] - mean;
-        q = fmaf(d, d, q);
-      }
-    }
-  const float rstd = rsqrtf(wave_sum(q) * inv_d + p.eps);
+  float mean, rstd;
+  row4_stats<NC>(v, lane, n_pieces, p.D, p.eps, mean, rstd);
 #pragma unroll
   for (int i = 0; i < NC; ++i) {
     const int e = (lane + 64 * i) * 4;
@@ -125,6 +132,23 @@
       }
     }
   }
+}
+
+template <int NC>
+__global__ __launch_bounds__(256) void layernorm_stats_kernel(const float* __restrict__ y, int64_t ldy, int64_t M, int D, float eps,
+                                                              f32x2_t* __restrict__ stats) {
+  const int lane = threadIdx.x & 63;
+  const int64_t row = (int64_t)blockIdx.x * ROWS_PER_BLOCK + (threadIdx.x >> 6);
+  if (row >= M) return;
+  const int n_pieces = D >> 2;
+  const float* yr = y + row * ldy;
+  float v[NC][4];
+#pragma unroll
+  for (int i = 0; i < NC; ++i)
+    if (lane + 64 * i < n_pieces) load4(yr + (lane + 64 * i) * 4, v[i]);
+  float mean, rstd;
+  row4_stats<NC>(v, lane, n_pieces, D, eps, mean, rstd);
+  if (lane == 0) stats[row] = f32x2_t{mean, rstd};
 }
 
 struct MergeArgs {
@@ -293,6 +317,23 @@
   return check_launch("layernorm");
 }
 
+extern "C" int aurora_hip_layernorm_stats(const float* y, int64_t ldy, int64_t M, int D, float eps, float* stats_out,
+                                          void* stream) {
+  AURORA_CHECK_ARG(y != nullptr && stats_out != nullptr, "layernorm_stats: null rows or statistics");
+  AURORA_CHECK_ARG(D % 8 == 0 && D > 0 && D <= 4096, "layernorm_stats: D=%d must be a multiple of 8, <= 4096", D);
+  AURORA_CHECK_ARG(ldy >= D && (ldy * 4) % 16 == 0 && (uintptr_t)y % 16 == 0 && (uintptr_t)stats_out % 8 == 0,
+                   "layernorm_stats: unaligned rows or statistics");
+  if (M <= 0) return AURORA_OK;
+  const dim3 grid(row_blocks(M)), block(256);
+  f32x2_t* st = reinterpret_cast<f32x2_t*>(stats_out);
+  if (D <= 256) hipLaunchKernelGGL((layernorm_stats_kernel<1>), grid, block, 0, as_stream(stream), y, ldy, M, D, eps, st);
+  else if (D <= 512) hipLaunchKernelGGL((layernorm_stats_kernel<2>), grid, block, 0, as_stream(stream), y, ldy, M, D, eps, st);
+  else if (D <= 1024) hipLaunchKernelGGL((layernorm_stats_kernel<4>), grid, block, 0, as_stream(stream), y, ldy, M, D, eps, st);
+  else if (D <= 2048) hipLaunchKernelGGL((layernorm_stats_kernel<8>), grid, block, 0, as_stream(stream), y, ldy, M, D, eps, st);
+  else hipLaunchKernelGGL((layernorm_stats_kernel<16>), grid, block, 0, as_stream(stream), y, ldy, M, D, eps, st);
+  return check_launch("layernorm_stats");
+}
+
 extern "C" int aurora_hip_merge_ln(const float* x, const float* ln_w, const float* ln_b, void* out, int B, int C,
                                    int H, int W, int D, float eps, int dtype, void* stream) {
   AURORA_CHECK_ARG(dtype == AURORA_F32 || dtype == AURORA_BF16, "merge_ln: bad dtype");
diff --git a/aurora_amd/csrc/step.hip b/aurora_amd/csrc/step.hip
--- a/aurora_amd/csrc/step.hip
+++ b/aurora_amd/csrc/step.hip
@@ -10,6 +10,7 @@
 struct CtxGuard { float* word; float a, c, limit_kv; bool pairs, scan; };
 struct ComposedFront { const ComposedCtx* layers; int levels, groups; int64_t rows; float embed_l1, embed_bias_max; };
 
+struct ResamplerTail { const float* stats; const float* lat1; const float *gain, *shift; bool deferred; };
 struct ResamplerCall {
   const Resampler* rs;
   const float* ctx;
@@ -21,6 +22,7 @@
   bool out_pairs;
   const ComposedFront* front;
   CtxGuard guard;
+  ResamplerTail* tail;
 };
 
 struct ResamplerLayer {
@@ -161,6 +163,13 @@
     L.linear(fc2.f32_mode(sp.pairs ? all : ly.f16_mode));
   }
   const bool y_pairs = c.out_pairs && sp.pairs && r.i + 1 == c.rs->layers.size();
+  if (y_pairs && c.tail && ly.ln2_w && ly.ln2_b && Dd <= 2048) {
+    REQUIRE((size_t)n_rows * 8 <= sp.s_bytes, "resampler: scratch region too small for the row statistics");
+    float* stats = (float*)r.S;
+    L.layernorm_stats(y, Dd, n_rows, Dd, c.eps, stats);
+    *c.tail = ResamplerTail{stats, lat1, ly.ln2_w, ly.ln2_b, true};
+    return;
+  }
   if (sp.pairs) L.layernorm_split(y, Dd, ly.ln2_w, ly.ln2_b, lat1, Dd, 0, 1, y_pairs ? nullptr : y, Dd, y_pairs ? y : nullptr, Dd, n_rows, Dd, c.eps);
   else L.layernorm(y, Dd, ly.ln2_w, ly.ln2_b, lat1, Dd, 0, y, Dd, nullptr, 0, n_rows, Dd, c.eps, AURORA_F32);
 }
@@ -178,6 +187,8 @@
     else attend_plain(L, r, false);
     resampler_mlp(L, r);
     m.arena.top = r.after_y;
+    if (c.tail && c.tail->deferred)
+      m.arena.top = (size_t)((const char*)c.tail->stats - m.arena.base) + (size_t)c.g.n_rows() * 8;
     lat = r.y;
   }
   return lat;
@@ -683,6 +694,8 @@
   call.out_pairs = two_term;
   call.front = nullptr;
   call.guard = CtxGuard{m.ctx_max.f() + 3, 1.0f, 0.0f, F16_SAFE, false, scan_ctx};
+  ResamplerTail tail{};
+  call.tail = m.ln_in_heads && two_term && hg.groups <= 1 ? &tail : nullptr;
   float* lat = resampler(m, s.L, call);
   const int n_a = two_term ? hg.n_pad : (int)hg.names.size() * s.PP, ld_a = round_up(n_a, 4);
   const float* hw = two_term ? (const float*)hg.ws.p : hg.w.f();
@@ -692,7 +705,15 @@
   if (hg.groups > 1)
     s.L.linear(LinearOp(lat, (int64_t)C * D2, hw, D2, hb, y_a, (int64_t)C * ld_a, (int64_t)B * Lp, n_a, D2, AURORA_F32)
                    .f32_mode(mode).batched(C, D2, (int64_t)n_a * D2, ld_a, ld_a));
-  else
+  else if (tail.deferred) {
+    const size_t rows = (size_t)B * Lp * C;
+    REQUIRE((const char*)tail.lat1 >= (const char*)lat + rows * D2 * 4 && (const char*)tail.stats >= (const char*)tail.lat1 + rows * D2 * 4 &&
+                (const char*)y_a >= (const char*)tail.stats + rows * 8,
+            "decoder: the heads' result overlaps the LayerNorm operands they read (result, residual, statistics)");
+    s.L.linear(LinearOp(lat, D2, hw, D2, hb, y_a, ld_a, (int64_t)rows, n_a, D2, AURORA_F32)
+                   .a_layernorm(tail.stats, tail.gain, tail.shift, tail.lat1, D2));
+    ++m.ln_in_heads_used;
+  } else
     s.L.linear(LinearOp(lat, D2, hw, D2, hb, y_a, ld_a, (int64_t)B * Lp * C, n_a, D2, AURORA_F32).f32_mode(mode));
   std::vector<aurora_unpatch_var> ad;
   for (size_t hi = 0; hi < hg.names.size(); ++hi) {
@@ -721,6 +742,7 @@
       });
     ctx = ctx_copy;
   }
+  m.ln_in_heads_used = 0;
   if (!m.head_main.names.empty()) decode_group(s, m.head_main, m.dec_rs, m.dec_q.f(), m.dec_out_bound, true, ctx);
   if (m.has_alt && !m.head_alt.names.empty())
     decode_group(s, m.head_alt, m.dec_rs_alt, m.dec_q_alt.f(), m.dec_out_bound_alt, m.head_main.names.empty(), ctx);
diff --git a/aurora_amd/engine/lib.py b/aurora_amd/engine/lib.py
--- a/aurora_amd/engine/lib.py
+++ b/aurora_amd/engine/lib.py
@@ -69,6 +69,9 @@
     "aurora_hip_split_f16": (c_int, [c_void_p, c_int64, c_void_p, c_int64, c_int64, c_int, c_float, c_void_p]),
     "aurora_hip_layernorm_split": (c_int, [c_void_p, c_int64, c_void_p, c_void_p, c_void_p, c_int64, c_int64, c_int,
                                            c_void_p, c_int64, c_void_p, c_int64, c_int64, c_int, c_float, c_void_p]),
+    "aurora_hip_layernorm_stats": (c_int, [c_void_p, c_int64, c_int64, c_int, c_float, c_void_p, c_void_p]),
+    "aurora_hip_linear_a_layernorm": (c_int, [c_void_p, c_int64, c_void_p, c_void_p, c_void_p, c_void_p, c_int64, c_void_p,
+                                              c_int64, c_void_p, c_void_p, c_int64, c_int64, c_int, c_int, c_void_p]),
     "aurora_hip_linear": (c_int, [c_void_p, c_int64, c_void_p, c_int64, c_void_p, c_void_p, c_int64,
                                   c_void_p, c_int64, c_void_p, c_int64, c_int64, c_int, c_int, c_int,
                                   c_int, c_void_p]),
@@ -533,6 +536,36 @@
                                            dtype_code(y.dtype), _stream()))
 
 
+def layernorm_stats(y: torch.Tensor, eps: float = 1e-5, d: Optional[int] = None) -> torch.Tensor:
+    ldy, dy = _rows(y)
+    D = d if d is not None else dy
+    M = y.shape[0]
+    assert y.dtype == torch.float32
+    stats = torch.empty(M, 2, dtype=torch.float32, device=y.device)
+    with _Timed("layernorm", float(M * D * 4)):
+        _check(load().aurora_hip_layernorm_stats(_ptr(y), ldy, M, D, eps, _ptr(stats), _stream()))
+    return stats
+
+
+def linear_a_layernorm(y: torch.Tensor, stats: torch.Tensor, gain: torch.Tensor, shift: torch.Tensor, res_pairs: torch.Tensor,
+                       w_pairs: torch.Tensor, bias: Optional[torch.Tensor], out: torch.Tensor) -> torch.Tensor:
+    ldy, K = _rows(y)
+    ldr, _ = _rows(res_pairs)
+    ldw, kw = _rows(w_pairs)
+    ldc, _ = _rows(out)
+    M, N = y.shape[0], w_pairs.shape[0]
+    assert y.dtype == res_pairs.dtype == w_pairs.dtype == out.dtype == torch.float32 and kw == K
+    assert stats.dtype == torch.float32 and stats.is_contiguous() and stats.shape == (M, 2) and res_pairs.shape[0] == M
+    for v in (gain, shift):
+        assert v.dtype == torch.float32 and v.numel() >= K and v.is_contiguous()
+    assert bias is None or (bias.dtype == torch.float32 and bias.numel() >= N and bias.is_contiguous())
+    assert out.shape[0] == M and out.shape[1] >= N
+    with _Timed("linear_f32", 2.0 * M * N * K):
+        _check(load().aurora_hip_linear_a_layernorm(_ptr(y), ldy, _ptr(stats), _ptr(gain), _ptr(shift), _ptr(res_pairs), ldr,
+                                                    _ptr(w_pairs), ldw, _ptr(bias), _ptr(out), ldc, M, N, K, _stream()))
+    return out
+
+
 def merge_ln(x: torch.Tensor, ln_w: torch.Tensor, ln_b: torch.Tensor, out: torch.Tensor,
              B: int, C: int, H: int, W: int, D: int, eps: float = 1e-5) -> torch.Tensor:
     assert x.dtype == torch.float32 and x.is_contiguous() and x.numel() == B * C * H * W * D
@@ -1449,7 +1482,7 @@
 class HipTuning(ctypes.Structure):
     _fields_ = [("fuse_ln", c_int32), ("band_split_attention", c_int32), ("qkv_planes", c_int32), ("split_k", c_int32),
                 ("perceiver_reassoc", c_int32), ("score_weights", c_int32), ("compose_front", c_int32),
-                ("reserved", c_int32 * 1)]
+                ("ln_in_heads", c_int32)]
 
 
 def tuning_from_env() -> HipTuning:
@@ -1472,7 +1505,8 @@
         t.fuse_ln = v + 1
     for field, var in (("band_split_attention", "AURORA_BAND_SPLIT_ATTENTION"), ("qkv_planes", "AURORA_QKV_PLANES"),
                        ("split_k", "AURORA_SPLIT_K"), ("perceiver_reassoc", "AURORA_PERCEIVER_REASSOC"),
-                       ("score_weights", "AURORA_SCORE_WEIGHTS"), ("compose_front", "AURORA_COMPOSE_FRONT")):
+                       ("score_weights", "AURORA_SCORE_WEIGHTS"), ("compose_front", "AURORA_COMPOSE_FRONT"),
+                       ("ln_in_heads", "AURORA_LN_IN_HEADS")):
         v = value(var, (0, 1))
         if v is not None:
             setattr(t, field, 2 if v else 1)
@@ -1566,6 +1600,7 @@
     "aurora_hip_compose_front_rule": (c_int, [c_int, c_int, ctypes.POINTER(c_int32), c_int]),
     "aurora_hip_composed_value_bound": (c_int, [c_float, c_float, c_float, c_float, c_float, _PF]),
     "aurora_hip_front_composed": (c_int, [c_void_p]),
+    "aurora_hip_ln_in_heads_used": (c_int, [c_void_p]),
     "aurora_hip_output_vars": (c_int, [c_void_p, _PS, c_int]),
     "aurora_hip_set_time_ex": (c_int, [c_void_p, _PD, ctypes.POINTER(c_int32), c_int, c_void_p]),
     "aurora_hip_set_band": (c_int, [c_void_p, ctypes.POINTER(HipBand)]),
diff --git a/aurora_amd/engine/native.py b/aurora_amd/engine/native.py
--- a/aurora_amd/engine/native.py
+++ b/aurora_amd/engine/native.py
@@ -329,6 +329,9 @@
     def front_composed(self) -> bool:
         return bool(lib.load().aurora_hip_front_composed(self._h))
 
+    def ln_in_heads_used(self) -> int:
+        return int(lib.load().aurora_hip_ln_in_heads_used(self._h))
+
     def generation(self) -> int:
         return int(lib.load().aurora_hip_generation(self._h))
 
diff --git a/include/aurora_hip.h b/include/aurora_hip.h
--- a/include/aurora_hip.h
+++ b/include/aurora_hip.h
@@ -72,6 +72,10 @@
 int aurora_hip_split_f16(const float* src, int64_t ld_src, void* dst, int64_t ld_dst, int64_t rows, int K,
                          float scale, void* stream);
 
+int aurora_hip_linear_a_layernorm(const float* y, int64_t ldy, const float* stats, const float* gain, const float* shift,
+                                  const void* res_pairs, int64_t ldr, const void* W_pairs, int64_t ldw, const float* bias,
+                                  float* C, int64_t ldc, int64_t M, int N, int K, void* stream);
+
 int aurora_hip_absmax(const float* x, int64_t n, float* out, void* stream);
 int aurora_hip_absmax_fold(const float* x, int64_t n, float* out, void* stream);
 int aurora_hip_zero_words(float* words, int n, void* stream);
@@ -98,6 +102,8 @@
                                const void* res, int64_t ldr, int64_t res_mod, int res_is_split,
                                float* out_f32, int64_t ldo, void* out_split, int64_t ld_split,
                                int64_t M, int D, float eps, void* stream);
+
+int aurora_hip_layernorm_stats(const float* y, int64_t ldy, int64_t M, int D, float eps, float* stats_out, void* stream);
 
 int aurora_hip_merge_ln(const float* x, const float* ln_w, const float* ln_b, void* out,
                         int B, int C, int H, int W, int D, float eps, int dtype, void* stream);
@@ -223,7 +229,7 @@
     int32_t perceiver_reassoc;
     int32_t score_weights;
     int32_t compose_front;
-    int32_t reserved[1];
+    int32_t ln_in_heads;
   } tuning;
 } aurora_hip_config;
 
@@ -279,6 +285,7 @@
 int aurora_hip_composed_value_bound(float v_l1, float embed_l1, float embed_bias_max, float composed_v_l1,
                                     float composed_vb_max, float out[6]);
 int aurora_hip_front_composed(const aurora_hip_model* model);
+int aurora_hip_ln_in_heads_used(const aurora_hip_model* model);
 int64_t aurora_hip_generation(const aurora_hip_model* model);
 int aurora_hip_abi_sizes(int32_t* out, int capacity);
 int aurora_hip_output_vars(const aurora_hip_model* model, const char** names, int capacity);
```

Result: no change. 8.013 forecast-steps/s (median of 6 runs) (+0.5%).
